# sepsamavi/safe-interactive-crowdnav

Hardware: AMD Instinct MI355X
Metric: sampled trajectories/sec (N x K, 50 denoise steps) (higher is better)
Workload: dtype fp16 activations x split-fp16 weights (weight-lo term as one bf8 MFMA per k64), fp32 accumulate; 1 GPU; cfg3: 256 episodes/GPU x N=5 x K=20 x H=12, 50 DDIM steps, JMID; episodes_per_gpu=256, total_episodes=256, humans=5, samples=20, horizon=12, denoise_steps=50, net=jmid, precision=f16mx, class_default_precision=f16mx, lanes=2

## Files before the change

### include/jmid_hip.h

```cpp
#ifndef JMID_HIP_H
#define JMID_HIP_H

#include <stddef.h>
#include <stdint.h>

#ifdef __cplusplus
extern "C" {
#endif
typedef struct jmid_ctx* jmid_handle_t;

#pragma GCC visibility push(default)

enum { JMID_NET_IMID = 0, JMID_NET_JMID = 1 };
enum { JMID_MEM_HOST = 0, JMID_MEM_DEVICE = 1 };
enum { JMID_PREC_F32 = 0, JMID_PREC_F16X3 = 1, JMID_PREC_F16 = 2, JMID_PREC_F16X2 = 3, JMID_PREC_F16MX = 4 };

enum {
    JMID_OK = 0,
    JMID_EINVAL = -1,
    JMID_ENOWEIGHT = -2,
    JMID_EHIP = -3,
    JMID_ENOMEM = -4,
    JMID_ERANGE = -5,
    JMID_ETIMEOUT = -6,
// ... 47 lines not shown

int jmid_wall_statistics(jmid_handle_t h, int E, int A, int K, int T, const float* pos, const float* p0, int L, const double* walls,
                         double radius, float* dist_out, uint8_t* agent_out, float* sample_out, float* scene_out, int mem);

int jmid_topk(jmid_handle_t h, int E, int A, int K, int T, int k, const float* pos, const float* bw, float* sel, float* logw,
              int mem);

int jmid_predict(jmid_handle_t h, int E, int A, int K, int T, int k, const float* x_st, const float* nbr_sum, const float* edge_mask,
                 const float* x_T, const float* p0, float dt, int precision, const float* bw, float* sel, float* logw, float* pos_out);

int jmid_net_eval_padded(jmid_handle_t h, int E, int A, int K, int T, const int32_t* n_agents, int step_idx, const float* x, const float* ctx,
                         int precision, float* e_out, int mem);
int jmid_denoise_padded(jmid_handle_t h, int E, int A, int K, int T, const int32_t* n_agents, const float* x_T, const float* ctx, const float* p0,
                        float dt, int precision, float* vel_out, float* pos_out, int mem);
int jmid_topk_padded(jmid_handle_t h, int E, int A, int K, int T, int k, const int32_t* n_agents, const float* pos, const float* bw, float* sel,
                     float* logw, int mem);
int jmid_predict_padded(jmid_handle_t h, int E, int A, int K, int T, int k, const int32_t* n_agents, const float* x_st, const float* nbr_sum,
                        const float* edge_mask, const float* x_T, const float* p0, float dt, int precision, const float* bw, float* sel,
                        float* logw, float* pos_out);

int jmid_collision_statistics_padded(jmid_handle_t h, int E, int A, int K, int T, const int32_t* n_agents, const float* pos, double threshold,
                                     float* pair_out, uint8_t* agent_out, float* sample_out, float* scene_out, int mem);
int jmid_wall_statistics_padded(jmid_handle_t h, int E, int A, int K, int T, const int32_t* n_agents, const float* pos, const float* p0, int L,
                                const double* walls, double radius, float* dist_out, uint8_t* agent_out, float* sample_out, float* scene_out,
                                int mem);

int jmid_build_scene(jmid_handle_t h, int E, int N, int F, const double* human_xy, const double* robot_xy, double time_step, int horizon,
                     int force_all_in_cluster, uint8_t* in_cluster_out, uint8_t* robot_in_cluster_out, int* n_in_out, double* cv_out, int mem);

int jmid_scene_get(jmid_handle_t h, float* x, float* x_st, float* nbr_sum, float* edge_mask, float* p0, int mem);

int jmid_build_scene_var(jmid_handle_t h, int E, int N, int F, const double* human_xy, const double* robot_xy, const int32_t* first_frame,
                         double time_step, int horizon, int force_all_in_cluster, uint8_t* in_cluster_out, uint8_t* robot_in_cluster_out,
                         int* n_in_out, double* cv_out, int mem);

int jmid_build_scene_absent(jmid_handle_t h, int E, int N, int F, const double* human_xy, const double* robot_xy, const int32_t* first_frame,
                            double time_step, int horizon, int force_all_in_cluster, uint8_t* in_cluster_out, uint8_t* robot_in_cluster_out,
                            int* n_in_out, double* cv_out, int mem);

int jmid_scene_get_first_index(jmid_handle_t h, int32_t* out, int mem);

int jmid_predict_scene(jmid_handle_t h, int E, int A, int K, int T, int k, const float* x_T, float dt, int precision, const float* bw,
                       float* sel, float* logw, float* pos_out);

int jmid_build_scene_stamped(jmid_handle_t h, int E, int N, int R, const double* stamps, const double* human_xy, const double* robot_xy,
                             const int* n_frames, double time_step, int horizon, int force_all_in_cluster, uint8_t* in_cluster_out,
                             uint8_t* robot_in_cluster_out, int* n_in_out, int* n_grid_out, double* cv_out, int mem);

int jmid_build_scene_stamped_var(jmid_handle_t h, int E, int N, int R, const double* stamps, const double* human_xy, const double* robot_xy,
                                 const int* n_frames, double time_step, int horizon, int force_all_in_cluster, uint8_t* in_cluster_out,
                                 uint8_t* robot_in_cluster_out, int* n_in_out, int* n_grid_out, double* cv_out, int32_t* first_frame_out,
                                 int mem);

int jmid_build_scene_stamped_coast(jmid_handle_t h, int E, int N, int R, const double* stamps, const double* human_xy, const double* robot_xy,
                                   const int* n_frames, double time_step, int horizon, int force_all_in_cluster, uint8_t* in_cluster_out,
                                   uint8_t* robot_in_cluster_out, int* n_in_out, int* n_grid_out, double* cv_out, int32_t* first_frame_out,
                                   int max_coast, int32_t* coast_out, int mem);

int jmid_scene_get_frames(jmid_handle_t h, double* human_xy_out, double* robot_xy_out, double* pose_now_out, int mem);

int jmid_forecast_scene(jmid_handle_t h, int E, int A, int K, int T, int k, const float* x_T, float dt, int precision, const float* bw,
                        double* forecasts_out, double* logw_out);

int jmid_noise_fill(jmid_handle_t h, uint64_t seed, int E, int rows, int T, const uint32_t* episode_ids, int draw, float* out, int mem);

int jmid_denoise_seeded(jmid_handle_t h, int E, int A, int K, int T, uint64_t seed, const uint32_t* episode_ids, const float* ctx,
                        const float* p0, float dt, int precision, float* vel_out, float* pos_out, int mem);

int jmid_denoise_reject_seeded(jmid_handle_t h, int E, int A, int K, int T, uint64_t seed, const uint32_t* episode_ids, int draw0,
                               const float* ctx, const float* p0, float dt, int precision, double threshold, int max_rounds,
                               float* vel_out, float* pos_out, int32_t* slot_out, int32_t* episode_out, int mem);

int jmid_denoise_reject_walls_seeded(jmid_handle_t h, int E, int A, int K, int T, uint64_t seed, const uint32_t* episode_ids, int draw0,
                                     const float* ctx, const float* p0, float dt, int precision, double threshold, int max_rounds, int L,
                                     const double* walls, double radius, float* vel_out, float* pos_out, int32_t* slot_out,
                                     int32_t* episode_out, int32_t* cause_out, int mem);

int jmid_predict_scene_seeded(jmid_handle_t h, int E, int A, int K, int T, int k, uint64_t seed, const uint32_t* episode_ids, float dt,
                              int precision, const float* bw, float* sel, float* logw, float* pos_out);
int jmid_forecast_scene_seeded(jmid_handle_t h, int E, int A, int K, int T, int k, uint64_t seed, const uint32_t* episode_ids, float dt,
                               int precision, const float* bw, double* forecasts_out, double* logw_out);

int jmid_noise_fill_padded(jmid_handle_t h, uint64_t seed, int E, int A, int K, int T, const int32_t* n_agents, const uint32_t* episode_ids,
                           int draw, float* out, int mem);
int jmid_denoise_padded_seeded(jmid_handle_t h, int E, int A, int K, int T, const int32_t* n_agents, uint64_t seed, const uint32_t* episode_ids,
                               const float* ctx, const float* p0, float dt, int precision, float* vel_out, float* pos_out, int mem);

int jmid_denoise_reject_padded_seeded(jmid_handle_t h, int E, int A, int K, int T, const int32_t* n_agents, uint64_t seed,
                                      const uint32_t* episode_ids, int draw0, const float* ctx, const float* p0, float dt, int precision,
                                      double threshold, int max_rounds, int L, const double* walls, double radius, float* vel_out,
                                      float* pos_out, int32_t* slot_out, int32_t* episode_out, int32_t* cause_out, int mem);

int jmid_repair_collisions(jmid_handle_t h, int E, int A, int K, int T, const int32_t* n_agents, const float* pos, const float* p0, float dt,
                           double threshold, double margin, double tau, double step, int max_iter, float* pos_out, float* vel_out,
                           float* sample_out, int32_t* episode_out, int mem);

int jmid_predict_scene_padded(jmid_handle_t h, int E, int A, int K, int T, int k, const float* x_T, float dt, int precision, const float* bw,
                              float* sel, float* logw, float* pos_out);
int jmid_forecast_scene_padded(jmid_handle_t h, int E, int A, int K, int T, int k, const float* x_T, float dt, int precision, const float* bw,
                               double* forecasts_out, double* logw_out);
int jmid_predict_scene_padded_seeded(jmid_handle_t h, int E, int A, int K, int T, int k, uint64_t seed, const uint32_t* episode_ids, float dt,
                                     int precision, const float* bw, float* sel, float* logw, float* pos_out);
int jmid_forecast_scene_padded_seeded(jmid_handle_t h, int E, int A, int K, int T, int k, uint64_t seed, const uint32_t* episode_ids, float dt,
                                      int precision, const float* bw, double* forecasts_out, double* logw_out);

int jmid_set_loss_schedule(jmid_handle_t h, int n_t, const float* beta, const float* c0, const float* c1);
int jmid_loss(jmid_handle_t h, int E, int A, int T, const int32_t* n_agents, const int32_t* t, const float* x0, const float* e, const float* ctx,
              int precision, double* loss_out, double* row_out, float* e_theta_out, int mem);
int jmid_loss_seeded(jmid_handle_t h, int E, int A, int T, const int32_t* n_agents, const int32_t* t, const float* x0, uint64_t seed,
                     const uint32_t* episode_ids, const float* ctx, int precision, double* loss_out, double* row_out, float* e_theta_out, int mem);

int jmid_set_caller_stream(jmid_handle_t h, void* stream);

int64_t jmid_graph_replays(jmid_handle_t h);

int64_t jmid_erange_count(jmid_handle_t h);
int64_t jmid_timeout_count(jmid_handle_t h);

int jmid_set_chunk_episodes(jmid_handle_t h, int episodes);
int jmid_set_tuning(jmid_handle_t h, const char* key, int value);
int jmid_profile_enable(jmid_handle_t h, uint32_t class_mask);
int jmid_profile_reset(jmid_handle_t h);
int jmid_profile_get(jmid_handle_t h, int cls, int64_t* n_launches, double* total_ms);
int jmid_kernel_class_count(void);
const char* jmid_kernel_class_name(int cls);
int jmid_synchronize(jmid_handle_t h);

#ifdef JMID_DIAGNOSTICS
int jmid_dbg_gemm(jmid_handle_t h, int M, int N, int K, const float* A, const float* Wt, const float* bias, int relu,
                  int precision, float* C);
int jmid_dbg_attention(jmid_handle_t h, int nseq, int S, const float* QKV, int precision, float* OUT);
int jmid_dbg_gemm_ln_mx(jmid_handle_t h, int M, int K, const float* A, const float* Wt, const float* bias, const float* gamma,
                        const float* beta, float* X, int fused);
int jmid_dbg_add_layernorm(jmid_handle_t h, int M, int d, float* X, const float* Y, const float* gamma,
                           const float* beta);
int jmid_dbg_plan_chunks(int net_kind, int nhead, int lanes, int chunk_episodes, int E, int tokens_per_episode, int* sizes, int cap);
int jmid_dbg_plan_chunks_mode(int net_kind, int nhead, int lanes, int chunk_episodes, int E, int tokens_per_episode, int precision, int* sizes, int cap);
#define JMID_DBG_GEMM_PLAN_KNOBS 13
int jmid_dbg_gemm_plan(int mode, int epi, int out, int M, int N, int K, int small_now, int one_chunk, const int* knobs, int* plan);
#define JMID_DBG_LAYOUT_SCENE 1
#define JMID_DBG_LAYOUT_FORECAST 2
#define JMID_DBG_LAYOUT_SEEDED 4
#define JMID_DBG_LAYOUT_PADDED 8
#define JMID_DBG_LAYOUT_FIRST_INDEX 16
#define JMID_DBG_LAYOUT_BW 32
#define JMID_DBG_LAYOUT_POS 64
#define JMID_DBG_LAYOUT_CV 128
#define JMID_DBG_CHAIN_WORDS (2 * 14 + 5)
#define JMID_DBG_SCENE_WORDS (2 * 13 + 4)
int jmid_dbg_chain_layout(int hist_len, int ctx_dim, int E, int A, int K, int T, int k, int N, int flags, int64_t* chain_dev, int64_t* chain_pin,
                          int64_t* scene);
int jmid_dbg_qkv0(jmid_handle_t h, int E, int A, int K, int T, const float* x, const float* hyp, int hyp_width, int step, int precision,
                  float* qkv, float* thyp_row);
int jmid_dbg_tail(jmid_handle_t h, int E, int A, int K, int T, const float* X, const float* hyp, int hyp_width, int step, int precision,
                  float* e, float* thyp_row);
#define JMID_DBG_LAYER_WIDTH(d_model, d_ff) (7 * (d_model) + (d_ff))
#define JMID_DBG_LAYER_PLAN_WORDS 25
int jmid_dbg_layer(jmid_handle_t h, int E, int A, int K, int T, int layer, int precision, const float* X, const int32_t* n_agents, int last,
                   float* hi, float* lo, int* plan);
int jmid_dbg_noise_words(jmid_handle_t h, uint64_t seed, int E, int rows, int T, const uint32_t* episode_ids, int draw, uint32_t* out, int mem);
#endif

#pragma GCC visibility pop
#ifdef __cplusplus
}
#endif
#endif
```

### safe-interactive-crowdnav_amd/_lib.py

```python
from __future__ import annotations

import ctypes as C
import os

from .build import library_path

c_float_p = C.POINTER(C.c_float)
Handle = C.c_void_p

NET_IMID, NET_JMID = 0, 1
MEM_HOST, MEM_DEVICE = 0, 1
PREC_F32, PREC_F16X3, PREC_F16, PREC_F16X2, PREC_F16MX = 0, 1, 2, 3, 4
PRECISIONS = {"f32": PREC_F32, "f16x3": PREC_F16X3, "f16": PREC_F16, "f16x2": PREC_F16X2, "f16mx": PREC_F16MX}

EINVAL, ENOWEIGHT, EHIP, ENOMEM, ERANGE, ETIMEOUT, EHISTORY = -1, -2, -3, -4, -5, -6, -7
ERR_NAMES = {EINVAL: "JMID_EINVAL", ENOWEIGHT: "JMID_ENOWEIGHT", EHIP: "JMID_EHIP", ENOMEM: "JMID_ENOMEM", ERANGE: "JMID_ERANGE",
             ETIMEOUT: "JMID_ETIMEOUT", EHISTORY: "JMID_EHISTORY"}

SIGNATURES = {
    "jmid_version": (C.c_char_p, []),
    "jmid_device_count": (C.c_int, []),
    "jmid_create": (C.c_int, [C.POINTER(Handle), C.c_int, C.c_int, C.c_int, C.c_int, C.c_int, C.c_int]),
    "jmid_destroy": (C.c_int, [Handle]),
    "jmid_last_error": (C.c_char_p, [Handle]),
    "jmid_load_weight": (C.c_int, [Handle, C.c_char_p, C.c_void_p, C.c_size_t]),
    "jmid_finalize_weights": (C.c_int, [Handle]),
    "jmid_set_ddim_table": (C.c_int, [Handle, C.c_int, C.c_void_p, C.c_void_p, C.c_void_p, C.c_void_p, C.c_void_p]),
    "jmid_set_ddpm_table": (C.c_int, [Handle, C.c_int, C.c_void_p, C.c_void_p, C.c_void_p, C.c_void_p, C.c_void_p]),
    "jmid_denoise_ddpm": (C.c_int, [Handle, C.c_int, C.c_int, C.c_int, C.c_int, C.c_void_p, C.c_void_p, C.c_void_p,
                                    C.c_void_p, C.c_float, C.c_int, C.c_void_p, C.c_void_p, C.c_int]),
    "jmid_encode": (C.c_int, [Handle, C.c_int, C.c_void_p, C.c_void_p, C.c_void_p, C.c_void_p, C.c_int]),
    "jmid_encode_var": (C.c_int, [Handle, C.c_int, C.c_void_p, C.c_void_p, C.c_void_p, C.c_void_p, C.c_void_p, C.c_int]),
    "jmid_denoise": (C.c_int, [Handle, C.c_int, C.c_int, C.c_int, C.c_int, C.c_void_p, C.c_void_p, C.c_void_p,
                               C.c_float, C.c_int, C.c_void_p, C.c_void_p, C.c_int]),
    "jmid_net_eval": (C.c_int, [Handle, C.c_int, C.c_int, C.c_int, C.c_int, C.c_int, C.c_void_p, C.c_void_p,
                                C.c_int, C.c_void_p, C.c_int]),
    "jmid_episode_metrics": (C.c_int, [Handle, C.c_int, C.c_int, C.c_int, C.c_int, C.c_void_p, C.c_void_p,
                                       C.c_void_p, C.c_int]),
    "jmid_eval_statistics": (C.c_int, [Handle, C.c_int, C.c_int, C.c_int, C.c_int, C.c_void_p, C.c_void_p, C.c_void_p,
                                       C.c_void_p, C.c_int]),
    "jmid_eval_statistics_masked": (C.c_int, [Handle, C.c_int, C.c_int, C.c_int, C.c_int, C.c_void_p, C.c_void_p, C.c_void_p,
                                              C.c_void_p, C.c_int, C.POINTER(C.c_int), C.c_void_p, C.c_void_p, C.c_void_p, C.c_int]),
    "jmid_collision_statistics": (C.c_int, [Handle, C.c_int, C.c_int, C.c_int, C.c_int, C.c_void_p, C.c_double, C.c_void_p,
                                            C.c_void_p, C.c_void_p, C.c_void_p, C.c_int]),
    "jmid_wall_statistics": (C.c_int, [Handle, C.c_int, C.c_int, C.c_int, C.c_int, C.c_void_p, C.c_void_p, C.c_int, C.c_void_p, C.c_double,
                                       C.c_void_p, C.c_void_p, C.c_void_p, C.c_void_p, C.c_int]),
    "jmid_collision_statistics_padded": (C.c_int, [Handle, C.c_int, C.c_int, C.c_int, C.c_int, C.c_void_p, C.c_void_p, C.c_double, C.c_void_p,
                                                   C.c_void_p, C.c_void_p, C.c_void_p, C.c_int]),
    "jmid_wall_statistics_padded": (C.c_int, [Handle, C.c_int, C.c_int, C.c_int, C.c_int, C.c_void_p, C.c_void_p, C.c_void_p, C.c_int, C.c_void_p,
                                              C.c_double, C.c_void_p, C.c_void_p, C.c_void_p, C.c_void_p, C.c_int]),
    "jmid_topk": (C.c_int, [Handle, C.c_int, C.c_int, C.c_int, C.c_int, C.c_int, C.c_void_p, C.c_void_p, C.c_void_p,
                            C.c_void_p, C.c_int]),
    "jmid_predict": (C.c_int, [Handle, C.c_int, C.c_int, C.c_int, C.c_int, C.c_int, C.c_void_p, C.c_void_p, C.c_void_p, C.c_void_p,
                               C.c_void_p, C.c_float, C.c_int, C.c_void_p, C.c_void_p, C.c_void_p, C.c_void_p]),
    "jmid_net_eval_padded": (C.c_int, [Handle, C.c_int, C.c_int, C.c_int, C.c_int, C.c_void_p, C.c_int, C.c_void_p, C.c_void_p,
                                       C.c_int, C.c_void_p, C.c_int]),
    "jmid_denoise_padded": (C.c_int, [Handle, C.c_int, C.c_int, C.c_int, C.c_int, C.c_void_p, C.c_void_p, C.c_void_p, C.c_void_p,
                                      C.c_float, C.c_int, C.c_void_p, C.c_void_p, C.c_int]),
    "jmid_topk_padded": (C.c_int, [Handle, C.c_int, C.c_int, C.c_int, C.c_int, C.c_int, C.c_void_p, C.c_void_p, C.c_void_p, C.c_void_p,
                                   C.c_void_p, C.c_int]),
    "jmid_predict_padded": (C.c_int, [Handle, C.c_int, C.c_int, C.c_int, C.c_int, C.c_int, C.c_void_p, C.c_void_p, C.c_void_p, C.c_void_p,
                                      C.c_void_p, C.c_void_p, C.c_float, C.c_int, C.c_void_p, C.c_void_p, C.c_void_p, C.c_void_p]),
    "jmid_build_scene": (C.c_int, [Handle, C.c_int, C.c_int, C.c_int, C.c_void_p, C.c_void_p, C.c_double, C.c_int, C.c_int, C.c_void_p,
                                   C.c_void_p, C.c_void_p, C.c_void_p, C.c_int]),
    "jmid_scene_get": (C.c_int, [Handle, C.c_void_p, C.c_void_p, C.c_void_p, C.c_void_p, C.c_void_p, C.c_int]),
    "jmid_build_scene_var": (C.c_int, [Handle, C.c_int, C.c_int, C.c_int, C.c_void_p, C.c_void_p, C.c_void_p, C.c_double, C.c_int, C.c_int,
                                       C.c_void_p, C.c_void_p, C.c_void_p, C.c_void_p, C.c_int]),
    "jmid_build_scene_absent": (C.c_int, [Handle, C.c_int, C.c_int, C.c_int, C.c_void_p, C.c_void_p, C.c_void_p, C.c_double, C.c_int, C.c_int,
                                          C.c_void_p, C.c_void_p, C.c_void_p, C.c_void_p, C.c_int]),
    "jmid_scene_get_first_index": (C.c_int, [Handle, C.c_void_p, C.c_int]),
    "jmid_predict_scene": (C.c_int, [Handle, C.c_int, C.c_int, C.c_int, C.c_int, C.c_int, C.c_void_p, C.c_float, C.c_int, C.c_void_p,
                                     C.c_void_p, C.c_void_p, C.c_void_p]),
    "jmid_build_scene_stamped": (C.c_int, [Handle, C.c_int, C.c_int, C.c_int, C.c_void_p, C.c_void_p, C.c_void_p, C.c_void_p, C.c_double,
                                           C.c_int, C.c_int, C.c_void_p, C.c_void_p, C.c_void_p, C.c_void_p, C.c_void_p, C.c_int]),
    "jmid_build_scene_stamped_var": (C.c_int, [Handle, C.c_int, C.c_int, C.c_int, C.c_void_p, C.c_void_p, C.c_void_p, C.c_void_p, C.c_double,
                                               C.c_int, C.c_int, C.c_void_p, C.c_void_p, C.c_void_p, C.c_void_p, C.c_void_p, C.c_void_p, C.c_int]),
    "jmid_build_scene_stamped_coast": (C.c_int, [Handle, C.c_int, C.c_int, C.c_int, C.c_void_p, C.c_void_p, C.c_void_p, C.c_void_p, C.c_double,
                                                 C.c_int, C.c_int, C.c_void_p, C.c_void_p, C.c_void_p, C.c_void_p, C.c_void_p, C.c_void_p, C.c_int,
                                                 C.c_void_p, C.c_int]),
    "jmid_scene_get_frames": (C.c_int, [Handle, C.c_void_p, C.c_void_p, C.c_void_p, C.c_int]),
    "jmid_forecast_scene": (C.c_int, [Handle, C.c_int, C.c_int, C.c_int, C.c_int, C.c_int, C.c_void_p, C.c_float, C.c_int, C.c_void_p,
                                      C.c_void_p, C.c_void_p]),
    "jmid_noise_fill": (C.c_int, [Handle, C.c_uint64, C.c_int, C.c_int, C.c_int, C.c_void_p, C.c_int, C.c_void_p, C.c_int]),
    "jmid_denoise_seeded": (C.c_int, [Handle, C.c_int, C.c_int, C.c_int, C.c_int, C.c_uint64, C.c_void_p, C.c_void_p, C.c_void_p,
                                      C.c_float, C.c_int, C.c_void_p, C.c_void_p, C.c_int]),
    "jmid_denoise_reject_seeded": (C.c_int, [Handle, C.c_int, C.c_int, C.c_int, C.c_int, C.c_uint64, C.c_void_p, C.c_int, C.c_void_p, C.c_void_p,
                                             C.c_float, C.c_int, C.c_double, C.c_int, C.c_void_p, C.c_void_p, C.c_void_p, C.c_void_p, C.c_int]),
    "jmid_denoise_reject_walls_seeded": (C.c_int, [Handle, C.c_int, C.c_int, C.c_int, C.c_int, C.c_uint64, C.c_void_p, C.c_int, C.c_void_p,
                                                   C.c_void_p, C.c_float, C.c_int, C.c_double, C.c_int, C.c_int, C.c_void_p, C.c_double,
                                                   C.c_void_p, C.c_void_p, C.c_void_p, C.c_void_p, C.c_void_p, C.c_int]),
    "jmid_predict_scene_seeded": (C.c_int, [Handle, C.c_int, C.c_int, C.c_int, C.c_int, C.c_int, C.c_uint64, C.c_void_p, C.c_float, C.c_int,
                                            C.c_void_p, C.c_void_p, C.c_void_p, C.c_void_p]),
    "jmid_forecast_scene_seeded": (C.c_int, [Handle, C.c_int, C.c_int, C.c_int, C.c_int, C.c_int, C.c_uint64, C.c_void_p, C.c_float, C.c_int,
                                             C.c_void_p, C.c_void_p, C.c_void_p]),
    "jmid_noise_fill_padded": (C.c_int, [Handle, C.c_uint64, C.c_int, C.c_int, C.c_int, C.c_int, C.c_void_p, C.c_void_p, C.c_int, C.c_void_p,
                                         C.c_int]),
    "jmid_denoise_padded_seeded": (C.c_int, [Handle, C.c_int, C.c_int, C.c_int, C.c_int, C.c_void_p, C.c_uint64, C.c_void_p, C.c_void_p,
                                             C.c_void_p, C.c_float, C.c_int, C.c_void_p, C.c_void_p, C.c_int]),
    "jmid_denoise_reject_padded_seeded": (C.c_int, [Handle, C.c_int, C.c_int, C.c_int, C.c_int, C.c_void_p, C.c_uint64, C.c_void_p, C.c_int,
                                                    C.c_void_p, C.c_void_p, C.c_float, C.c_int, C.c_double, C.c_int, C.c_int, C.c_void_p,
                                                    C.c_double, C.c_void_p, C.c_void_p, C.c_void_p, C.c_void_p, C.c_void_p, C.c_int]),
    "jmid_repair_collisions": (C.c_int, [Handle, C.c_int, C.c_int, C.c_int, C.c_int, C.c_void_p, C.c_void_p, C.c_void_p, C.c_float, C.c_double,
                                         C.c_double, C.c_double, C.c_double, C.c_int, C.c_void_p, C.c_void_p, C.c_void_p, C.c_void_p, C.c_int]),
    "jmid_predict_scene_padded": (C.c_int, [Handle, C.c_int, C.c_int, C.c_int, C.c_int, C.c_int, C.c_void_p, C.c_float, C.c_int, C.c_void_p,
                                            C.c_void_p, C.c_void_p, C.c_void_p]),
    "jmid_forecast_scene_padded": (C.c_int, [Handle, C.c_int, C.c_int, C.c_int, C.c_int, C.c_int, C.c_void_p, C.c_float, C.c_int, C.c_void_p,
                                             C.c_void_p, C.c_void_p]),
    "jmid_predict_scene_padded_seeded": (C.c_int, [Handle, C.c_int, C.c_int, C.c_int, C.c_int, C.c_int, C.c_uint64, C.c_void_p, C.c_float,
                                                   C.c_int, C.c_void_p, C.c_void_p, C.c_void_p, C.c_void_p]),
    "jmid_forecast_scene_padded_seeded": (C.c_int, [Handle, C.c_int, C.c_int, C.c_int, C.c_int, C.c_int, C.c_uint64, C.c_void_p, C.c_float,
                                                    C.c_int, C.c_void_p, C.c_void_p, C.c_void_p]),
    "jmid_set_loss_schedule": (C.c_int, [Handle, C.c_int, C.c_void_p, C.c_void_p, C.c_void_p]),
    "jmid_loss": (C.c_int, [Handle, C.c_int, C.c_int, C.c_int, C.c_void_p, C.c_void_p, C.c_void_p, C.c_void_p, C.c_void_p, C.c_int,
                            C.c_void_p, C.c_void_p, C.c_void_p, C.c_int]),
    "jmid_loss_seeded": (C.c_int, [Handle, C.c_int, C.c_int, C.c_int, C.c_void_p, C.c_void_p, C.c_void_p, C.c_uint64, C.c_void_p, C.c_void_p,
                                   C.c_int, C.c_void_p, C.c_void_p, C.c_void_p, C.c_int]),
    "jmid_set_chunk_episodes": (C.c_int, [Handle, C.c_int]),
    "jmid_set_tuning": (C.c_int, [Handle, C.c_char_p, C.c_int]),
    "jmid_set_caller_stream": (C.c_int, [Handle, C.c_void_p]),
    "jmid_graph_replays": (C.c_int64, [Handle]),
    "jmid_erange_count": (C.c_int64, [Handle]),
    "jmid_timeout_count": (C.c_int64, [Handle]),
    "jmid_profile_enable": (C.c_int, [Handle, C.c_uint32]),
    "jmid_profile_reset": (C.c_int, [Handle]),
    "jmid_profile_get": (C.c_int, [Handle, C.c_int, C.POINTER(C.c_int64), C.POINTER(C.c_double)]),
    "jmid_kernel_class_count": (C.c_int, []),
    "jmid_kernel_class_name": (C.c_char_p, [C.c_int]),
    "jmid_synchronize": (C.c_int, [Handle]),
}

DIAG_SIGNATURES = {
    "jmid_dbg_gemm": (C.c_int, [Handle, C.c_int, C.c_int, C.c_int, C.c_void_p, C.c_void_p, C.c_void_p, C.c_int,
                                C.c_int, C.c_void_p]),
    "jmid_dbg_attention": (C.c_int, [Handle, C.c_int, C.c_int, C.c_void_p, C.c_int, C.c_void_p]),
    "jmid_dbg_gemm_ln_mx": (C.c_int, [Handle, C.c_int, C.c_int, C.c_void_p, C.c_void_p, C.c_void_p, C.c_void_p, C.c_void_p,
                                      C.c_void_p, C.c_int]),
    "jmid_dbg_add_layernorm": (C.c_int, [Handle, C.c_int, C.c_int, C.c_void_p, C.c_void_p, C.c_void_p, C.c_void_p]),
    "jmid_dbg_plan_chunks": (C.c_int, [C.c_int, C.c_int, C.c_int, C.c_int, C.c_int, C.c_int, C.POINTER(C.c_int), C.c_int]),
    "jmid_dbg_plan_chunks_mode": (C.c_int, [C.c_int, C.c_int, C.c_int, C.c_int, C.c_int, C.c_int, C.c_int, C.POINTER(C.c_int), C.c_int]),
    "jmid_dbg_gemm_plan": (C.c_int, [C.c_int] * 8 + [C.POINTER(C.c_int), C.POINTER(C.c_int)]),
    "jmid_dbg_chain_layout": (C.c_int, [C.c_int] * 9 + [C.POINTER(C.c_int64)] * 3),
    "jmid_dbg_qkv0": (C.c_int, [Handle, C.c_int, C.c_int, C.c_int, C.c_int, C.c_void_p, C.c_void_p, C.c_int, C.c_int, C.c_int, C.c_void_p, C.c_void_p]),
    "jmid_dbg_tail": (C.c_int, [Handle, C.c_int, C.c_int, C.c_int, C.c_int, C.c_void_p, C.c_void_p, C.c_int, C.c_int, C.c_int, C.c_void_p, C.c_void_p]),
    "jmid_dbg_layer": (C.c_int, [Handle, C.c_int, C.c_int, C.c_int, C.c_int, C.c_int, C.c_int, C.c_void_p, C.c_void_p, C.c_int,
                                 C.c_void_p, C.c_void_p, C.POINTER(C.c_int)]),
    "jmid_dbg_noise_words": (C.c_int, [Handle, C.c_uint64, C.c_int, C.c_int, C.c_int, C.c_void_p, C.c_int, C.c_void_p, C.c_int]),
}


class JmidError(RuntimeError):
    def __init__(self, code: int, message: str):
        super().__init__(f"{ERR_NAMES.get(code, code)}: {message}")
        self.code = code


_LIBS = {}


def load_library(path: str = None) -> C.CDLL:
    key = os.path.abspath(path or library_path())
    if key in _LIBS:
        return _LIBS[key]
    import torch

    path = key
    if not os.path.exists(path):
        raise ImportError(
            f"{path} is missing: build it with `python -c 'import __graft_entry__ as g; g.build()'` "
            "(hipcc --offload-arch=gfx950).  The predictor has no CPU fallback.")
    lib = C.CDLL(path)
    for name, (res, args) in SIGNATURES.items():
        fn = getattr(lib, name)
        fn.restype = res
        fn.argtypes = args
    lib.has_diagnostics = b"diagnostics" in lib.jmid_version()
    if lib.has_diagnostics:
        for name, (res, args) in DIAG_SIGNATURES.items():
            fn = getattr(lib, name)
            fn.restype = res
            fn.argtypes = args
    _LIBS[key] = lib
    return lib
```

### safe-interactive-crowdnav_amd/csrc/common.hpp

```cpp
#pragma once
#include <hip/hip_runtime.h>
#include <hip/hip_fp16.h>
#include <stdint.h>

#include <atomic>
#include <mutex>

namespace jmid {

typedef float f32x4 __attribute__((ext_vector_type(4)));
typedef float f32x16 __attribute__((ext_vector_type(16)));
typedef _Float16 f16x8 __attribute__((ext_vector_type(8)));
typedef _Float16 f16x4 __attribute__((ext_vector_type(4)));
typedef _Float16 f16x2 __attribute__((ext_vector_type(2)));

constexpr int kWave = 64;
constexpr int kPeMaxLen = 24;

struct HyperLayout {
    int g1, b1, g3, b3, g4, b4, go, bo, total;
};
__host__ __device__ inline HyperLayout make_hyper_layout(int d_model, int d_mid, int d_low) {
    HyperLayout L;
    L.g1 = 0;
// ... 13 lines not shown
}
inline unsigned fast_div_magic(int d, unsigned long long x_max) {
    return d > 1 && x_max * (unsigned long long)d < (1ull << 32) ? (unsigned)((1ull << 32) / (unsigned)d + 1) : 0u;
}

struct RowMap {
    int T, A, KA;
    unsigned mT = 0, mKA = 0, mA = 0;
    __device__ __forceinline__ int ea(int m) const {
        const int r = fast_div(m, T, mT);
        const int e = fast_div(r, KA, mKA);
        const int a = r - fast_div(r, A, mA) * A;
        return e * A + a;
    }
    __device__ __forceinline__ int t_of(int m) const { return m - fast_div(m, T, mT) * T; }
};
inline RowMap make_rowmap(int T, int A, int KA, unsigned long long M) {
    RowMap r{T, A, KA};
    r.mT = fast_div_magic(T, M);
    r.mKA = fast_div_magic(KA, M);
    r.mA = fast_div_magic(A, M);
    return r;
}

__host__ __device__ __forceinline__ size_t blk_index(int row, int k, int K) {
    const int rb = row >> 7, r = row & 127, kb = k >> 5, kk = k & 31;
    return ((size_t)rb * (K >> 5) + kb) * 4096 + (size_t)(r * 32 + ((((kk >> 3) ^ ((r >> 2) & 3)) << 3) | (kk & 7)));
}
__host__ __device__ __forceinline__ size_t blk_plane_elems(size_t rows, int K) {
    return ((rows + 127) / 128) * 128 * (size_t)K;
}

__host__ __device__ __forceinline__ int vt_key_pos(int key) {
    const int g = (key >> 2) & 3;
    return (key & ~15) | ((((g & 1) << 1) | (g >> 1)) << 2) | (key & 3);
}
__host__ __device__ __forceinline__ int vt_spad(int S) { return (S + 15) / 16 * 16; }

template <typename T>
__device__ __forceinline__ void args_now(const T& a) {
    static_assert(sizeof(T) % 4 == 0, "argument block of whole dwords");
    struct Words { unsigned w[sizeof(T) / 4]; };
    const Words w = __builtin_bit_cast(Words, a);
#pragma unroll
    for (unsigned i = 0; i < sizeof(T) / 4; ++i) asm volatile("" ::"s"(w.w[i]));
}
template <typename... T>
__device__ __forceinline__ void args_now_each(const T&... t) { (args_now(t), ...); }

__device__ __forceinline__ unsigned long long pin_uniform(unsigned long long v) {
    asm volatile("" : "+s"(v));
    return v;
}
__device__ __forceinline__ unsigned long long pin_uniform_rfl(unsigned long long v) {
    const unsigned lo = __builtin_amdgcn_readfirstlane((unsigned)v), hi = __builtin_amdgcn_readfirstlane((unsigned)(v >> 32));
    unsigned long long u = ((unsigned long long)hi << 32) | lo;
    asm volatile("" : "+s"(u));
    return u;
}

struct Tuning {
    int fuse_embed = 1;
    int ln_fuse = 0;
    int ln_rows = 0;
    int bystander_lds = 0;
    int gemm_h_variant = 0;
    int gemm_ng = 0;
    int no_vt_direct = 0;
    int attn_h_variant = 0;
    int attn_pack = 1;
    int vt_stage = 0;
    int graph = 0;
    int attn_nsplit = 0;
    int csl_swap = 0;
    int attn_sm = 0;
    int attn_prio = 0;
    int attn_one_wg = 0;
    int h1_stage = 0;
    int out_traj = 0;
    int attn_mx = 0;
    int mx_ln = 0;
    int attn_pf = 0;
    int gemm_small = 0;
    int small_cmb = 0;
    int small_lnx = 0;
    int cus = 256;
    int lnx_polls = 0;
    int lnx_withhold = 0;
    int small_lnx2 = 0;
    int gemm_pn = 0;
    int small_lanes = 0;
    int small_qk = 0;
    int small_pn = 0;
    int qkv0 = 0;
    int tail_fold = 0;
    int attn_abl = 0;
    int gemm_abl = 0;
};
#ifdef JMID_ABLATIONS
inline int attn_abl_bits(const Tuning& t) { return t.attn_abl; }
inline int gemm_abl_bits(const Tuning& t) { return t.gemm_abl; }
#else
inline int attn_abl_bits(const Tuning&) { return 0; }
inline int gemm_abl_bits(const Tuning&) { return 0; }
#endif

struct DevSeen {
    std::atomic<bool> v[64];
    DevSeen() { for (auto& b : v) b.store(false, std::memory_order_relaxed); }
};
struct DeviceOnce {
    std::unique_lock<std::mutex> lk;
    std::atomic<bool>* slot = nullptr;
    explicit operator bool() const { return slot != nullptr; }
    DeviceOnce() = default;
    DeviceOnce(DeviceOnce&& o) noexcept : lk(std::move(o.lk)), slot(o.slot) { o.slot = nullptr; }
    ~DeviceOnce() { if (slot) slot->store(true, std::memory_order_release); }
};
inline std::mutex& device_once_mutex() {
    static std::mutex m;
    return m;
}
inline DeviceOnce first_use_on_device(DevSeen& seen) {
    int dev = 0;
    (void)hipGetDevice(&dev);
    dev &= 63;
    DeviceOnce o;
    if (seen.v[dev].load(std::memory_order_acquire)) return o;
    o.lk = std::unique_lock<std::mutex>(device_once_mutex());
    if (seen.v[dev].load(std::memory_order_acquire)) {
        o.lk.unlock();
        return o;
    }
    o.slot = &seen.v[dev];
    return o;
}

template <auto Kernel, size_t MaxLds = 0, typename... Args>
inline hipError_t launch_with_lds(dim3 grid, dim3 block, size_t lds_bytes, hipStream_t st, Args... args) {
    static DevSeen seen;
    if (auto once_ = first_use_on_device(seen))
        (void)hipFuncSetAttribute(reinterpret_cast<const void*>(Kernel), hipFuncAttributeMaxDynamicSharedMemorySize,
                                  (int)(MaxLds ? MaxLds : lds_bytes));
    hipLaunchKernelGGL(Kernel, grid, block, lds_bytes, st, args...);
    return hipGetLastError();
}

template <typename F>
static inline int bystander_lds(int n, F* fn) {
    if (n > 0) (void)hipFuncSetAttribute((const void*)fn, hipFuncAttributeMaxDynamicSharedMemorySize, n);
    return n;
}

__device__ __forceinline__ float sigmoidf_(float x) { return 1.0f / (1.0f + expf(-x)); }

__device__ __forceinline__ float wave_sum(float v) {
#pragma unroll
    for (int o = 32; o > 0; o >>= 1) v += __shfl_xor(v, o, 64);
    return v;
}

__device__ __forceinline__ void half_swap(float x, float& lo_half, float& hi_half) {
#ifdef JMID_ATT_SHFL
    lo_half = x;
    hi_half = __shfl_xor(x, 32, 64);
#else
    float a = x, b = x;
    asm volatile("s_nop 1\n\tv_permlane32_swap_b32 %0, %1" : "+v"(a), "+v"(b));
    lo_half = a;
    hi_half = b;
#endif
}

__device__ __forceinline__ int frag_row(int reg, int hi) { return (reg & 3) + 8 * (reg >> 2) + 4 * hi; }

}
```

### safe-interactive-crowdnav_amd/csrc/jmid_abi.hip

```cpp
#include "jmid_ctx.hpp"
#include "collision_stats.hpp"
#include "wall_stats.hpp"
#include "repair.hpp"

namespace jmid_host {

int upload_walls(jmid_ctx* h, int L, const double* walls, const double** dev, const std::string& who) {
    *dev = nullptr;
    if (L < 0 || L > WLS_MAX_L) return fail(h, JMID_EINVAL, who + " supports 0 <= L <= 64 walls");
    if (L == 0) return 0;
    if (!walls) return fail(h, JMID_EINVAL, who + ": null walls with L > 0");
    for (int i = 0; i < L * 4; ++i)
        if (!std::isfinite(walls[i])) return fail(h, JMID_EINVAL, who + ": a wall has a non-finite coordinate");
    if (int rc = h->wall_seg.upload(h, walls, L * 8, who.c_str())) return rc;
    *dev = h->wall_seg.get<double>();
    return 0;
}

std::string& thread_error() {
    static thread_local std::string e;
    return e;
}

int fail(jmid_ctx* h, int code, const std::string& msg) {
// ... 1294 lines not shown
}

int jmid_predict_scene_padded_seeded(jmid_handle_t h, int E, int A, int K, int T, int k, uint64_t seed, const uint32_t* episode_ids, float dt,
                                     int precision, const float* bw, float* sel, float* logw, float* pos_out) {
    const SeedArgs sa{seed, episode_ids};
    ChainCall c = chain_call("jmid_predict_scene_padded_seeded", E, A, K, T, k, dt, precision);
    c.padded = true; c.seeded = &sa; c.bw = bw; c.sel = sel; c.logw = logw; c.pos_out = pos_out;
    return predict_scene_entry(h, c);
}

int jmid_forecast_scene_padded_seeded(jmid_handle_t h, int E, int A, int K, int T, int k, uint64_t seed, const uint32_t* episode_ids, float dt,
                                      int precision, const float* bw, double* forecasts_out, double* logw_out) {
    const SeedArgs sa{seed, episode_ids};
    ChainCall c = chain_call("jmid_forecast_scene_padded_seeded", E, A, K, T, k, dt, precision);
    c.forecast = c.padded = true; c.seeded = &sa; c.bw = bw; c.forecasts_out = forecasts_out; c.logw_out = logw_out;
    return predict_scene_entry(h, c);
}

int jmid_denoise_padded_seeded(jmid_handle_t h, int E, int A, int K, int T, const int32_t* n_agents, uint64_t seed, const uint32_t* episode_ids,
                               const float* ctx, const float* p0, float dt, int precision, float* vel_out, float* pos_out, int mem) {
    if (!h) return JMID_EINVAL;
    if (!n_agents) return fail(h, JMID_EINVAL, "jmid_denoise_padded_seeded: null n_agents");
    if (!episode_ids) return fail(h, JMID_EINVAL, "jmid_denoise_padded_seeded: null episode_ids");
    const SeedArgs sa{seed, episode_ids};
    DenoiseCall c{E, A, K, T, precision, mem};
    c.ctx = ctx; c.p0 = p0; c.dt = dt; c.vel_out = vel_out; c.pos_out = pos_out; c.n_agents = n_agents; c.seeded = &sa;
    c.who = "jmid_denoise_padded_seeded";
    return run_network(h, c);
}

int jmid_noise_fill_padded(jmid_handle_t h, uint64_t seed, int E, int A, int K, int T, const int32_t* n_agents, const uint32_t* episode_ids, int draw,
                           float* out, int mem) {
    return noise_padded_entry(h, seed, E, A, K, T, n_agents, episode_ids, draw, out, mem);
}

int jmid_denoise_seeded(jmid_handle_t h, int E, int A, int K, int T, uint64_t seed, const uint32_t* episode_ids, const float* ctx, const float* p0,
                        float dt, int precision, float* vel_out, float* pos_out, int mem) {
    if (!h) return JMID_EINVAL;
    if (!episode_ids) return fail(h, JMID_EINVAL, "jmid_denoise_seeded: null episode_ids");
    const SeedArgs sa{seed, episode_ids};
    DenoiseCall c{E, A, K, T, precision, mem};
    c.ctx = ctx; c.p0 = p0; c.dt = dt; c.vel_out = vel_out; c.pos_out = pos_out; c.seeded = &sa; c.who = "jmid_denoise_seeded";
    return run_network(h, c);
}

static int reject_entry(jmid_handle_t h, const char* who, int E, int A, int K, int T, bool padded, const int32_t* n_agents, uint64_t seed, const uint32_t* episode_ids, int draw0,
                        const float* ctx, const float* p0, float dt, int precision, double threshold, int max_rounds, int L, const double* walls,
                        double radius, float* vel_out, float* pos_out, int32_t* slot_out, int32_t* episode_out, int32_t* cause_out, int mem) {
    if (!h) return JMID_EINVAL;
    const std::string w(who);
    if (int rc = check_ready(h)) return rc;
    if (h->ddpm) return fail(h, JMID_EINVAL, w + " samples with DDIM: under a DDPM table the draws 1.. are the steps' z");
    if (E < 1 || K < 1 || K > REJ_MAX_K || T < 2 || T > CLS_MAX_T || A < 1 || A > CLS_MAX_A)
        return fail(h, JMID_EINVAL, w + " supports E >= 1, 1 <= K <= 1024, 2 <= T <= 24, 1 <= A <= 64");
    if ((size_t)E * K > (size_t)0x7fffffff) return fail(h, JMID_EINVAL, w + ": E * K exceeds the launch grid");
    if (!episode_ids || !ctx) return fail(h, JMID_EINVAL, w + ": null episode_ids or ctx");
    if (!p0) return fail(h, JMID_EINVAL, w + ": null p0 (the predicate is defined on positions)");
    if (!(threshold >= 0.0) || !std::isfinite(threshold)) return fail(h, JMID_EINVAL, w + ": the threshold must be finite and >= 0");
    if (max_rounds < 0 || max_rounds > 64) return fail(h, JMID_EINVAL, w + ": max_rounds must be in 0..64");
    if (draw0 < 0 || draw0 > 0x7fffffff - 64) return fail(h, JMID_EINVAL, w + ": draw0 must be at least 0 (and draw0 + max_rounds must fit an int)");
    CallMode mode;
    if (!call_mode(precision, &mode)) return fail(h, JMID_EINVAL, w + ": precision must be JMID_PREC_F32, JMID_PREC_F16X3, JMID_PREC_F16X2 or JMID_PREC_F16MX");
    if (mem != JMID_MEM_HOST && mem != JMID_MEM_DEVICE) return fail(h, JMID_EINVAL, w + ": bad mem");
    if (!(radius >= 0.0) || !std::isfinite(radius)) return fail(h, JMID_EINVAL, w + ": the radius must be finite and >= 0");
    if (padded) {
        if (int rc = check_n_agents(h, who, n_agents, E, A)) return rc;
        if (h->net_kind == JMID_NET_JMID && mode.split && !attn_masked_built(plan_attn(h->d / h->nhead, h->tune), mode.x2 != 0))
            return fail(h, JMID_EINVAL, w + ": a padded call needs the default attention kernel (the attention A/B knobs have no masked form)");
    }
    HIPCHK(h, hipSetDevice(h->device));
    RejectWalls rw;
    rw.L = L; rw.radius = radius;
    if (int rc = upload_walls(h, L, walls, &rw.dev, w)) return rc;
    return reject_loop(h, who, E, A, K, T, n_agents, seed, episode_ids, draw0, ctx, p0, dt, precision, threshold, max_rounds, rw, vel_out, pos_out, slot_out,
                       episode_out, cause_out, mem);
}

int jmid_denoise_reject_seeded(jmid_handle_t h, int E, int A, int K, int T, uint64_t seed, const uint32_t* episode_ids, int draw0, const float* ctx,
                               const float* p0, float dt, int precision, double threshold, int max_rounds, float* vel_out, float* pos_out,
                               int32_t* slot_out, int32_t* episode_out, int mem) {
    return reject_entry(h, "jmid_denoise_reject_seeded", E, A, K, T, false, nullptr, seed, episode_ids, draw0, ctx, p0, dt, precision, threshold, max_rounds, 0,
                        nullptr, 0.0, vel_out, pos_out, slot_out, episode_out, nullptr, mem);
}

int jmid_denoise_reject_walls_seeded(jmid_handle_t h, int E, int A, int K, int T, uint64_t seed, const uint32_t* episode_ids, int draw0,
                                     const float* ctx, const float* p0, float dt, int precision, double threshold, int max_rounds, int L,
                                     const double* walls, double radius, float* vel_out, float* pos_out, int32_t* slot_out, int32_t* episode_out,
                                     int32_t* cause_out, int mem) {
    return reject_entry(h, "jmid_denoise_reject_walls_seeded", E, A, K, T, false, nullptr, seed, episode_ids, draw0, ctx, p0, dt, precision, threshold,
                        max_rounds, L, walls, radius, vel_out, pos_out, slot_out, episode_out, cause_out, mem);
}

int jmid_denoise_reject_padded_seeded(jmid_handle_t h, int E, int A, int K, int T, const int32_t* n_agents, uint64_t seed, const uint32_t* episode_ids,
                                      int draw0, const float* ctx, const float* p0, float dt, int precision, double threshold, int max_rounds, int L,
                                      const double* walls, double radius, float* vel_out, float* pos_out, int32_t* slot_out, int32_t* episode_out,
                                      int32_t* cause_out, int mem) {
    return reject_entry(h, "jmid_denoise_reject_padded_seeded", E, A, K, T, true, n_agents, seed, episode_ids, draw0, ctx, p0, dt, precision,
                        threshold, max_rounds, L, walls, radius, vel_out, pos_out, slot_out, episode_out, cause_out, mem);
}

int jmid_noise_fill(jmid_handle_t h, uint64_t seed, int E, int rows, int T, const uint32_t* episode_ids, int draw, float* out, int mem) {
    return noise_entry(h, "jmid_noise_fill", seed, E, rows, T, episode_ids, draw, out, nullptr, mem);
}

int jmid_set_chunk_episodes(jmid_handle_t h, int episodes) {
    if (!h || episodes < 0) return JMID_EINVAL;
    h->chunk_eps = episodes;
    drop_graphs(h);
    return JMID_OK;
}

int jmid_set_tuning(jmid_handle_t h, const char* key, int value) {
    if (!h || !key) return JMID_EINVAL;
    const std::string k(key);
    struct Knob {
        const char* name;
        int Tuning::*field;
        int lo, hi;
    };
#ifdef JMID_DIAGNOSTICS
    static const Knob knobs[] = {
        {"gemm_h_variant", &Tuning::gemm_h_variant, 0, 8},
        {"attn_pack", &Tuning::attn_pack, 0, 1},
        {"fuse_embed", &Tuning::fuse_embed, 0, 1},
        {"bystander_lds", &Tuning::bystander_lds, 0, 160 * 1024},
        {"ln_rows", &Tuning::ln_rows, 0, 128},
        {"ln_fuse", &Tuning::ln_fuse, 0, 2},
        {"no_vt_direct", &Tuning::no_vt_direct, 0, 1},
        {"gemm_ng", &Tuning::gemm_ng, 0, 64},
        {"attn_h_variant", &Tuning::attn_h_variant, 0, 2},
        {"vt_stage", &Tuning::vt_stage, 0, 3},
        {"graph", &Tuning::graph, 0, 2},
        {"attn_nsplit", &Tuning::attn_nsplit, 0, 16},
        {"attn_mx", &Tuning::attn_mx, 0, 3},
        {"out_traj", &Tuning::out_traj, 0, 2},
        {"attn_pf", &Tuning::attn_pf, 0, 2},
        {"attn_one_wg", &Tuning::attn_one_wg, 0, 1},
        {"attn_sm", &Tuning::attn_sm, 0, 2},
        {"attn_prio", &Tuning::attn_prio, 0, 2},
        {"mx_ln", &Tuning::mx_ln, 0, 2},
        {"csl_swap", &Tuning::csl_swap, 0, 3},
        {"h1_stage", &Tuning::h1_stage, 0, 2},
        {"gemm_small", &Tuning::gemm_small, 0, 2},
        {"gemm_pn", &Tuning::gemm_pn, 0, 8},
        {"small_lanes", &Tuning::small_lanes, 0, 2},
        {"small_cmb", &Tuning::small_cmb, 0, 2},
        {"small_lnx", &Tuning::small_lnx, 0, 2},
        {"cus", &Tuning::cus, 0, 4096},
        {"lnx_polls", &Tuning::lnx_polls, 0, 1 << 20},
        {"lnx_withhold", &Tuning::lnx_withhold, 0, 1},
        {"small_lnx2", &Tuning::small_lnx2, 0, 2},
        {"small_qk", &Tuning::small_qk, 0, 2},
        {"small_pn", &Tuning::small_pn, 0, 8},
        {"qkv0", &Tuning::qkv0, 0, 2},
        {"tail_fold", &Tuning::tail_fold, 0, 2},
#ifdef JMID_ABLATIONS
        {"attn_abl", &Tuning::attn_abl, 0, 1 << 30},
        {"gemm_abl", &Tuning::gemm_abl, 0, 1 << 30},
#endif
    };
#endif
    if (k == "lanes") {
        if (value < 1 || value > jmid_ctx::kMaxLanes) return fail(h, JMID_EINVAL, "lanes must be 1..4");
        h->lanes = value;
        return JMID_OK;
    }
#ifdef JMID_DIAGNOSTICS
    for (const Knob& kn : knobs)
        if (k == kn.name) {
            if (value < kn.lo || value > kn.hi || (k == "ln_rows" && value != 0 && value != 64 && value != 128))
                return fail(h, JMID_EINVAL, k + " out of range");
            h->tune.*(kn.field) = value;
            if (k == "cus" && value == 0) {
                int cus = 0;
                h->tune.cus = hipDeviceGetAttribute(&cus, hipDeviceAttributeMultiprocessorCount, h->device) == hipSuccess && cus > 0 ? cus : 256;
            }
            drop_graphs(h);
            return JMID_OK;
        }
#endif
    return fail(h, JMID_EINVAL, "unknown tuning key " + k);
}

int64_t jmid_graph_replays(jmid_handle_t h) { return h ? h->graph_replays : -1; }

int64_t jmid_erange_count(jmid_handle_t h) { return h ? h->erange_calls : -1; }
int64_t jmid_timeout_count(jmid_handle_t h) { return h ? h->lnx_timeouts : -1; }

int jmid_set_caller_stream(jmid_handle_t h, void* stream) {
    if (!h) return JMID_EINVAL;
    h->caller_stream = reinterpret_cast<hipStream_t>(stream);
    return JMID_OK;
}

int jmid_synchronize(jmid_handle_t h) {
    if (!h) return JMID_EINVAL;
    HIPCHK(h, hipSetDevice(h->device));
    HIPCHK(h, hipStreamSynchronize(h->stream));
    return JMID_OK;
}

}
```

### safe-interactive-crowdnav_amd/csrc/jmid_ctx.hpp

```cpp
#pragma once
#include "../../include/jmid_hip.h"

#include <hip/hip_runtime.h>

#include <algorithm>
#include <cmath>
#include <cstdio>
#include <cstring>
#include <limits>
#include <map>
#include <string>
#include <vector>

#include "attn_f16x3.hpp"
#include "attn_f32.hpp"
#include "common.hpp"
#include "elementwise.hpp"
#include "encoder.hpp"
#include "eval_stats.hpp"
#include "gemm_f16x3.hpp"
#include "gemm_ln_f16x3.hpp"
#include "gemm_ln2_mx.hpp"
#include "gemm_small.hpp"
#include "gemm_f32.hpp"
// ... 186 lines not shown
    std::string err;
    jmid_ctx() = default;
    jmid_ctx(const jmid_ctx&) = delete;
    ~jmid_ctx();
};

constexpr size_t kLnxWords = 2 * jmid::SM_LNX_GRANULES;

namespace jmid_host {

inline hipStream_t stream_of(jmid_ctx* h) { return h->stream; }
inline int reserve_block(jmid_ctx* h, Block& b, size_t need, const char* who) {
    return &b == &h->arena ? ensure_arena(h, need, who) : b.reserve(h, need, who);
}

struct CallMode {
    int precision = JMID_PREC_F32;
    bool split = false;
    int x2 = 0;
    int mx = 0;
    GemmMode gemm = GM_X3;
};
inline bool call_mode(int precision, CallMode* m) {
    if (precision != JMID_PREC_F32 && precision != JMID_PREC_F16X3 && precision != JMID_PREC_F16X2 && precision != JMID_PREC_F16MX) return false;
    const int mx = precision == JMID_PREC_F16MX, x2 = precision == JMID_PREC_F16X2 || mx;
    *m = CallMode{precision, precision != JMID_PREC_F32, x2, mx, !x2 ? GM_X3 : mx ? GM_MX : GM_X2};
    return true;
}

struct ProfScope {
    jmid_ctx* h;
    int cls;
    hipStream_t stream;
    bool on;
    EvPair ev;
    ProfScope(jmid_ctx* h_, int cls_, hipStream_t s) : h(h_), cls(cls_), stream(s), on((h_->prof_mask >> cls_) & 1u) {
        if (on) {
            if (!h->ev_pool.empty()) {
                ev = h->ev_pool.back();
                h->ev_pool.pop_back();
            } else {
                hipEventCreate(&ev.a);
                hipEventCreate(&ev.b);
            }
            hipEventRecord(ev.a, stream);
        }
    }
    ~ProfScope() {
        if (on) {
            hipEventRecord(ev.b, stream);
            h->prof_ev[cls].push_back(ev);
        }
    }
};

inline size_t numel(const std::vector<size_t>& s) {
    size_t n = 1;
    for (size_t v : s) n *= v;
    return n;
}

void register_shapes(jmid_ctx* h);
int dev_alloc_copy(jmid_ctx* h, float** out, const std::vector<float>& host);
int fetch_host(jmid_ctx* h, const std::string& name, std::vector<float>& out);
std::vector<float> time_table(const jmid_ctx* h, const std::vector<float>& beta);
int upload_time_table(jmid_ctx* h);
int upload_loss_schedule(jmid_ctx* h);
int make_w8(jmid_ctx* h, const float* dW, int N, int K, jmid_ctx::W8Image* out);
int w8_image(jmid_ctx* h, const float* dW, int N, int K, unsigned char* out);
void free_planes(jmid_ctx* h);
void free_derived(jmid_ctx* h);
void free_weights(jmid_ctx* h);
void drop_graphs(jmid_ctx* h);
void sync_lanes(jmid_ctx* h);
std::vector<int> plan_chunks(const jmid_ctx* h, const CallMode& m, int E, int tokens_per_episode);
int check_ready(jmid_ctx* h);
struct SeedArgs {
    uint64_t seed;
    const uint32_t* ids;
    int draw = 0;
};
int fill_noise(jmid_ctx* h, uint64_t seed, const unsigned* ids_dev, int E, size_t n, int draw, float* out, unsigned* words, hipStream_t stream);
int fill_noise_padded(jmid_ctx* h, uint64_t seed, const unsigned* ids_dev, const int* n_agents_dev, int E, int A, int K, int T, int draw, float* out,
                      hipStream_t stream);
struct LossCall {
    const int32_t* t = nullptr;
    const float* e = nullptr;
    const SeedArgs* seeded = nullptr;
    double *loss_out = nullptr, *row_out = nullptr;
};
struct DenoiseCall {
    int E, A, K, T, precision, mem;
    const float *x_in = nullptr, *ctx = nullptr, *p0 = nullptr;
    float dt = 0.f;
    float *vel_out = nullptr, *pos_out = nullptr, *e_out = nullptr;
    int single_step = -1;
    const float* z = nullptr;
    const SeedArgs* seeded = nullptr;
    bool chained = false;
    const int32_t* n_agents = nullptr;
    const int* n_agents_dev = nullptr;
    const LossCall* loss = nullptr;
    const char* who = "jmid_denoise";
};
struct ChainCall {
    int E, A, K, T, k, precision;
    float dt = 0.f;
    const char* who = "jmid_predict";
    bool scene = false;
    bool forecast = false;
    bool padded = false;
    const float *x_st = nullptr, *nbr_sum = nullptr, *edge_mask = nullptr, *p0 = nullptr;
    const float* x_T = nullptr;
    const SeedArgs* seeded = nullptr;
    const float* bw = nullptr;
    float *sel = nullptr, *logw = nullptr, *pos_out = nullptr;
    double *forecasts_out = nullptr, *logw_out = nullptr;
    const int32_t* n_agents = nullptr;
    bool rank() const { return k < K; }
};
struct ChainIo {
    Arr<float> x_st, nbr_sum, edge_mask, x_T, p0, bw;
    size_t up_bytes = 0;
    Arr<float> ctx;
    Arr<int> flag;
    Arr<double> forecasts, logw_d;
    Arr<float> sel, logw, pos;
    size_t down_bytes = 0;
    Arr<int> first_index;
    size_t up_bytes_from(const Arr<float>& a) const { return up_bytes - (size_t)((const char*)a.p - (const char*)x_st.p); }
};
enum SceneSource {
    SCENE_HOST_ARRAYS,
    SCENE_DEVICE_ARRAYS,
    SCENE_DEVICE_GRID,
};
struct SceneBuild {
    const char* who;
    int E, N, F;
    SceneSource src;
    const double *human_xy, *robot_xy;
    const int32_t* first_frame = nullptr;
    bool allow_absent = false;
    double time_step = 0.0;
    int horizon = 0, force_all_in_cluster = 0;
    uint8_t *in_cluster_out = nullptr, *robot_in_cluster_out = nullptr;
    int* n_in_out = nullptr;
    double* cv_out = nullptr;
    int mem = JMID_MEM_HOST;
};
int check_n_agents(jmid_ctx* h, const char* who, const int32_t* n_agents, int E, int A);
int run_network(jmid_ctx* h, DenoiseCall a);
int dbg_step(jmid_ctx* h, bool tail, int E, int A, int K, int T, const float* in, const float* hyp, int hyp_width, int step, int precision,
             float* out, float* thyp_row);
int dbg_layer(jmid_ctx* h, int E, int A, int K, int T, int layer, int precision, const float* X, const int32_t* n_agents, int last,
              float* hi, float* lo, int* plan);
int flagged_call(jmid_ctx* h, int flag);
int launch_episode_metrics(jmid_ctx* h, const float* pos, const float* gt, float* out, int E, int K, int A, int T);
size_t chain_io(const jmid_ctx* h, const ChainCall& c, char* base, ChainIo* out, bool pinned);
size_t scene_arrays(int E, int N, int F, int horizon, bool has_first, char* base, SceneArrays* out);
int noise_entry(jmid_ctx* h, const char* who, uint64_t seed, int E, int rows, int T, const uint32_t* episode_ids, int draw, float* out,
                unsigned* words, int mem);
int prof_collect(jmid_ctx* h);

}
using namespace jmid_host;
```

### safe-interactive-crowdnav_amd/csrc/jmid_diag.hip

```cpp
#include "jmid_ctx.hpp"
#include "jmid_launch.hpp"

#include <deque>

#ifdef JMID_DIAGNOSTICS

static int dbg_open(jmid_ctx* h, int precision, CallMode* mode) {
    if (!call_mode(precision, mode)) return fail(h, JMID_EINVAL, "bad precision");
    HIPCHK(h, hipSetDevice(h->device));
    if (!h->range_flag) {
        HIPCHK(h, hipMalloc((void**)&h->range_flag, sizeof(int)));
        HIPCHK(h, hipMemsetAsync(h->range_flag, 0, sizeof(int), h->stream));
    }
    return 0;
}

struct DbgTemps {
    jmid_ctx* h;
    const char* who;
    std::deque<Block> blocks;
    int rc = 0;
    template <class T>
    T* take(size_t bytes, const void* host = nullptr) {
        if (rc) return nullptr;
// ... 122 lines not shown
        GemmArgs g{};
        g.A = dA; g.lda = K; g.W = dW; g.ldw = K; g.bias = dB; g.C = dC; g.ldc = N; g.M = M; g.N = N; g.K = K;
        rc = relu ? run_gemm<EPI_BIAS_RELU>(h, h->stream, KC_GEMM_QKV, g) : run_gemm<EPI_BIAS>(h, h->stream, KC_GEMM_QKV, g);
    } else {
        const size_t pa = blk_plane_elems(M, K) * 2, pw = blk_plane_elems(N, K) * 2;
        half_t *ah = t.zeros<half_t>(pa), *al = t.zeros<half_t>(pa), *wh = t.zeros<half_t>(pw), *wl = t.zeros<half_t>(pw);
        if (t.rc) return t.rc;
        hipLaunchKernelGGL(split_planes_blocked_kernel, dim3(512), dim3(256), 0, h->stream, dA, ah, al, M, K,
                           h->range_flag, 1.0f);
        hipLaunchKernelGGL(split_planes_blocked_kernel, dim3(512), dim3(256), 0, h->stream, dW, wh, wl, N, K,
                           h->range_flag, kWScale);
        GemmHArgs g{};
        g.Ahi = ah; g.Alo = al; g.Whi = wh; g.Wlo = wl; g.bias = dB; g.C = dC; g.ldc = N;
        g.M = M; g.N = N; g.K = K; g.x2 = mode.x2;
        if (mode.mx && N % 32 == 0 && K % 64 == 0)
            if (!(g.W8 = dbg_w8(t, dW, N, K))) return t.rc;
        const GemmPlan plan = plan_gemm(mode.gemm, relu ? EPI_BIAS_RELU : EPI_BIAS, OUT_F32, M, N, K, CallFacts{}, h->tune);
        rc = relu ? run_gemm_h<EPI_BIAS_RELU, OUT_F32>(h, h->stream, KC_GEMM_QKV, g, plan) : run_gemm_h<EPI_BIAS, OUT_F32>(h, h->stream, KC_GEMM_QKV, g, plan);
    }
    if (rc) return rc;
    HIPCHK(h, hipStreamSynchronize(h->stream));
    HIPCHK(h, hipMemcpy(C, dC, (size_t)M * N * 4, hipMemcpyDeviceToHost));
    return 0;
}

int jmid_dbg_attention(jmid_handle_t h, int nseq, int S, const float* QKV, int precision, float* OUT) {
    if (!h || !QKV || !OUT) return JMID_EINVAL;
    CallMode mode;
    if (int rc = dbg_open(h, precision, &mode)) return rc;
    const size_t Mt = (size_t)nseq * S;
    const int d = h->d, hd = h->d / h->nhead;
    DbgTemps t{h, "jmid_dbg_attention"};
    float* dQ = t.take<float>(Mt * 3 * d * 4, QKV);
    float* dO = t.take<float>(Mt * d * 4);
    if (t.rc) return t.rc;
    int rc = 0;
    if (precision == JMID_PREC_F32) {
        AttnArgs aa{dQ, dO, S, d, h->nhead, 1.0f / sqrtf((float)hd), nullptr, nullptr};
        ProfScope ps(h, KC_ATTN, h->stream);
        hipError_t e = launch_attn_f32(aa, nseq, hd, plan_attn(hd, h->tune).pack, h->stream);
        if (e != hipSuccess) rc = fail(h, JMID_EHIP, hipGetErrorString(e));
    } else {
        const int Spad = vt_spad(S);
        const size_t vt = (size_t)nseq * d * Spad;
        half_t* b[8];
        const size_t sz[8] = {Mt * d, Mt * d, Mt * d, Mt * d, vt, vt, blk_plane_elems(Mt, d), blk_plane_elems(Mt, d)};
        for (int i = 0; i < 8; ++i) b[i] = t.zeros<half_t>(sz[i] * sizeof(half_t));
        if (t.rc) return t.rc;
        hipLaunchKernelGGL(qkv_to_planes_kernel, dim3(512), dim3(256), 0, h->stream, dQ, b[0], b[1], b[2], b[3], b[4],
                           b[5], Mt, d, hd, S, Spad, 1.4426950408889634f / sqrtf((float)hd));
        int ns = 1;
        float *opart = nullptr, *mlpart = nullptr;
        if (hd == 128) ns = attn_pick_nsplit(((S + 127) / 128) * h->nhead * nseq, S);
        if (ns > 1) {
            opart = t.take<float>((size_t)ns * Mt * d * 4);
            mlpart = t.take<float>((size_t)ns * Mt * h->nhead * 2 * 4);
            if (t.rc) return t.rc;
        }
        AttnHArgs aa{b[0], b[1], b[2], b[3], b[4], b[5], b[6], b[7], S, Spad, d, h->nhead, 1.0f / sqrtf((float)hd),
                     h->range_flag, ns, opart, mlpart, mode.x2};
        {
            ProfScope ps(h, KC_ATTN, h->stream);
            hipError_t e = launch_attn_f16x3(aa, nseq, hd, plan_attn(hd, h->tune), h->stream);
            if (e != hipSuccess) rc = fail(h, JMID_EHIP, hipGetErrorString(e));
        }
        hipLaunchKernelGGL(merge_planes_kernel, dim3(512), dim3(256), 0, h->stream, b[6], b[7], dO, (int)Mt, d, (float*)nullptr);
    }
    if (rc) return rc;
    HIPCHK(h, hipStreamSynchronize(h->stream));
    HIPCHK(h, hipMemcpy(OUT, dO, Mt * d * 4, hipMemcpyDeviceToHost));
    return 0;
}

int jmid_dbg_gemm_ln_mx(jmid_handle_t h, int M, int K, const float* A, const float* Wt, const float* bias, const float* gamma,
                        const float* beta, float* X, int fused) {
    if (!h || !A || !Wt || !bias || !gamma || !beta || !X || M <= 0 || K % 64 != 0) return JMID_EINVAL;
    constexpr int N = GLN_BN;
    CallMode mode;
    if (int rc = dbg_open(h, JMID_PREC_F16MX, &mode)) return rc;
    DbgTemps t{h, "jmid_dbg_gemm_ln_mx"};
    float* dA = t.take<float>((size_t)M * K * 4, A);
    float* dW = t.take<float>((size_t)N * K * 4, Wt);
    float* dB = t.take<float>(N * 4, bias);
    float* dG = t.take<float>(N * 4, gamma);
    float* dT = t.take<float>(N * 4, beta);
    float* dX = t.take<float>((size_t)M * N * 4, X);
    float* dY = t.zeros<float>((size_t)(M + 63) / 64 * 64 * N * 4);
    const size_t pa = blk_plane_elems(M, K) * 2, pw = blk_plane_elems(N, K) * 2, px = blk_plane_elems(M, N) * 2;
    half_t *ah = t.zeros<half_t>(pa), *al = t.zeros<half_t>(pa), *wh = t.zeros<half_t>(pw), *wl = t.zeros<half_t>(pw);
    half_t *w16h = t.zeros<half_t>((size_t)N * K * 2), *w16l = t.zeros<half_t>((size_t)N * K * 2);
    half_t* xh = t.zeros<half_t>(px);
    unsigned char* xl8 = t.zeros<unsigned char>(px);
    if (t.rc) return t.rc;
    hipLaunchKernelGGL(split_planes_blocked_kernel, dim3(512), dim3(256), 0, h->stream, dA, ah, al, M, K, h->range_flag, 1.0f);
    hipLaunchKernelGGL(split_planes_blocked_kernel, dim3(512), dim3(256), 0, h->stream, dW, wh, wl, N, K, h->range_flag, kWScale);
    hipLaunchKernelGGL(split_planes_k16_kernel, dim3(256), dim3(256), 0, h->stream, dW, w16h, w16l, N, K);
    hipLaunchKernelGGL(split_planes_lo8_kernel, dim3(512), dim3(256), 0, h->stream, dX, xh, xl8, M);
    unsigned char* w8 = dbg_w8(t, dW, N, K);
    if (!w8) return t.rc;
    int rc = 0;
    if (fused == 1) {
        GemmLn2Args g2{ah, w16h, w8, dB, dG, dT, xh, xl8, M, K, 1e-5f, h->range_flag, 0};
        hipError_t e = launch_gemm_ln2_mx(g2, plan_ln_rows(true, M, h->tune), h->stream);
        if (e != hipSuccess) rc = fail(h, JMID_EHIP, hipGetErrorString(e));
    } else {
        GemmHArgs g{};
        g.Ahi = ah; g.Alo = al; g.Whi = wh; g.Wlo = wl; g.W8 = w8; g.bias = dB; g.C = dY; g.ldc = N; g.M = M; g.N = N; g.K = K; g.x2 = mode.x2;
        if (fused == 3) {
            unsigned long long* xs = t.zeros<unsigned long long>(kLnxWords * sizeof(unsigned));
            const GemmPlan lnx = plan_gemm(GM_MX, EPI_BIAS, OUT_LNX, M, N, K, CallFacts{}, h->tune);
            if (!xs || lnx.shape == GS_NONE) return fail(h, JMID_EINVAL, "jmid_dbg_gemm_ln_mx: shape does not take the small kernel with the statistics exchange");
            g.ln_gamma = dG; g.ln_beta = dT; g.ln_xh = xh; g.ln_xl = nullptr; g.ln_xl8 = xl8; g.ln_xchg = xs; g.ln_eps = 1e-5f; g.ln_no_lo = 0;
            (void)hipMemsetAsync(h->range_flag, 0, sizeof(int), h->stream);
            rc = run_gemm_lnx_small(h, h->stream, KC_GEMM_OUT, g, lnx);
            if (!rc) {
                int flag = 0;
                (void)hipMemcpyAsync(&flag, h->range_flag, sizeof(int), hipMemcpyDeviceToHost, h->stream);
                (void)hipStreamSynchronize(h->stream);
                if (flag & 2) rc = fail(h, JMID_EHIP, "jmid_dbg_gemm_ln_mx: a workgroup gave up waiting for its row tile's statistics");
            }
        } else {
            rc = run_gemm_h<EPI_BIAS, OUT_F32>(h, h->stream, KC_GEMM_OUT, g, plan_gemm(GM_MX, EPI_BIAS, OUT_F32, M, N, K, CallFacts{}, h->tune));
            if (!rc) rc = run_add_ln(h, h->stream, nullptr, dY, dG, dT, M, N, xh, reinterpret_cast<half_t*>(xl8), true, 0);
        }
    }
    if (rc) return rc;
    hipLaunchKernelGGL(merge_planes_lo8_kernel, dim3(512), dim3(256), 0, h->stream, xh, xl8, dX, M, (float*)nullptr);
    HIPCHK(h, hipStreamSynchronize(h->stream));
    HIPCHK(h, hipMemcpy(X, dX, (size_t)M * N * 4, hipMemcpyDeviceToHost));
    return 0;
}

int jmid_dbg_add_layernorm(jmid_handle_t h, int M, int d, float* X, const float* Y, const float* gamma,
                           const float* beta) {
    if (!h || !X || !Y || !gamma || !beta) return JMID_EINVAL;
    HIPCHK(h, hipSetDevice(h->device));
    DbgTemps t{h, "jmid_dbg_add_layernorm"};
    float* dX = t.take<float>((size_t)M * d * 4, X);
    float* dY = t.take<float>((size_t)M * d * 4, Y);
    float* dG = t.take<float>((size_t)d * 4, gamma);
    float* dB = t.take<float>((size_t)d * 4, beta);
    if (t.rc) return t.rc;
    if (int rc = run_add_ln(h, h->stream, dX, dY, dG, dB, M, d)) return rc;
    HIPCHK(h, hipStreamSynchronize(h->stream));
    HIPCHK(h, hipMemcpy(X, dX, (size_t)M * d * 4, hipMemcpyDeviceToHost));
    return 0;
}

int jmid_dbg_qkv0(jmid_handle_t h, int E, int A, int K, int T, const float* x, const float* hyp, int hyp_width, int step, int precision,
                  float* qkv, float* thyp_row) {
    return h ? dbg_step(h, false, E, A, K, T, x, hyp, hyp_width, step, precision, qkv, thyp_row) : JMID_EINVAL;
}

int jmid_dbg_tail(jmid_handle_t h, int E, int A, int K, int T, const float* X, const float* hyp, int hyp_width, int step, int precision,
                  float* e, float* thyp_row) {
    return h ? dbg_step(h, true, E, A, K, T, X, hyp, hyp_width, step, precision, e, thyp_row) : JMID_EINVAL;
}

int jmid_dbg_layer(jmid_handle_t h, int E, int A, int K, int T, int layer, int precision, const float* X, const int32_t* n_agents, int last,
                   float* hi, float* lo, int* plan) {
    return h ? dbg_layer(h, E, A, K, T, layer, precision, X, n_agents, last, hi, lo, plan) : JMID_EINVAL;
}

int jmid_dbg_noise_words(jmid_handle_t h, uint64_t seed, int E, int rows, int T, const uint32_t* episode_ids, int draw, uint32_t* out, int mem) {
    return noise_entry(h, "jmid_dbg_noise_words", seed, E, rows, T, episode_ids, draw, nullptr, out, mem);
}

}
#endif
```

### safe-interactive-crowdnav_amd/csrc/jmid_planner.hip

```cpp
#include "jmid_ctx.hpp"
#include "jmid_launch.hpp"

namespace jmid_host {

void drop_graphs(jmid_ctx* h) {
    for (auto& kv : h->graphs)
        if (kv.second.exec) hipGraphExecDestroy(kv.second.exec);
    h->graphs.clear();
}

void sync_lanes(jmid_ctx* h) {
    for (int l = 0; l + 1 < jmid_ctx::kMaxLanes; ++l)
        if (h->lane_stream[l]) (void)hipStreamSynchronize(h->lane_stream[l]);
    if (h->stream) (void)hipStreamSynchronize(h->stream);
}

int ensure_arena(jmid_ctx* h, size_t bytes, const char* who) {
    if (bytes <= h->arena.bytes) return 0;
    drop_graphs(h);
    h->last_pos = nullptr;
    sync_lanes(h);
    return h->arena.reserve(h, bytes, who);
}

// ... 23 lines not shown
    g.S = h->net_kind == JMID_NET_JMID ? K * A * T : T;
    g.Spad = vt_spad(g.S);
    return g;
}

size_t step_ws_floats(const jmid_ctx* h, size_t Mc, const CallMode& m, const SeqGeom& sg, int nsplit, StepBuffers* sb,
                      char* base, size_t qkv0_rows, size_t tail_rows) {
    Carver c(base);
    StepBuffers s{};
    s.X = c.take(Mc * h->d);
    s.Y = c.take((Mc + 63) / 64 * 64 * h->d);
    s.ln_xchg = reinterpret_cast<unsigned long long*>(c.take(kLnxWords));
    if (!tail_rows) s.Y4 = c.take(Mc * h->dlow);
    if (!m.split) {
        s.QKV = c.take(Mc * 3 * h->d);
        s.ATT = c.take(Mc * h->d);
        s.H1 = c.take(Mc * h->ff);
        s.Y3 = c.take(Mc * h->dmid);
    } else {
        s.Xh = take_half(c, blk_plane_elems(Mc, h->d));
        s.Xl = take_half(c, blk_plane_elems(Mc, h->d));
        if (h->net_kind == JMID_NET_JMID) {
            s.Qh = take_half(c, Mc * h->d);
            s.Ql = take_half(c, Mc * h->d);
            s.Kh = take_half(c, Mc * h->d);
            s.Kl = take_half(c, Mc * h->d);
            s.Vh = take_half(c, Mc * h->d);
            s.Vl = take_half(c, Mc * h->d);
            s.vt_elems = (size_t)sg.nseq * h->d * sg.Spad;
            s.Vth = take_half(c, s.vt_elems);
            s.Vtl = take_half(c, s.vt_elems);
            if (nsplit > 1) {
                s.Opart = c.take((size_t)nsplit * Mc * h->d);
                s.MLpart = c.take((size_t)nsplit * Mc * h->nhead * 2);
            }
            if (qkv0_rows) {
                s.coef = c.take(qkv0_rows * h->d);
                s.uvc = c.take(qkv0_rows * 3 * h->d);
            }
        } else {
            s.QKV = c.take(Mc * 3 * h->d);
        }
        s.Ah = take_half(c, blk_plane_elems(Mc, h->d));
        s.Al = take_half(c, blk_plane_elems(Mc, h->d));
        s.H1h = take_half(c, blk_plane_elems(Mc, h->ff));
        s.H1l = take_half(c, blk_plane_elems(Mc, h->ff));
        if (tail_rows) {
            s.weff = c.take(tail_rows * 2 * h->d);
            s.beff = c.take(tail_rows * 2);
        } else {
            s.Y3h = take_half(c, blk_plane_elems(Mc, h->dmid));
            s.Y3l = take_half(c, blk_plane_elems(Mc, h->dmid));
        }
    }
    if (sb) *sb = s;
    return c.off;
}

bool byte_lo_plane(const jmid_ctx* h, const CallMode& m) { return m.mx && h->d == GLN_BN && h->tune.mx_ln != 2; }

enum ResidualPath {
    RB_GEMM_LN2,
    RB_GEMM_LN,
    RB_LNX_SMALL,
    RB_GEMM_ADD_LN,
};
struct ResidualPlan {
    ResidualPath path;
    int ln_rows;
    GemmPlan gemm;
    bool merge;
};

ResidualPlan residual_path(const jmid_ctx* h, const CallMode& m, int M, int K, const CallFacts& cf) {
    const Tuning& t = h->tune;
    if (h->d == GLN_BN && t.ln_fuse != 2 && (t.ln_fuse == 1 || M >= 7168))
        return {byte_lo_plane(h, m) ? RB_GEMM_LN2 : RB_GEMM_LN, plan_ln_rows(byte_lo_plane(h, m), M, t), {}, false};
    if (byte_lo_plane(h, m) && !h->lnx_off) {
        const GemmPlan lnx = plan_gemm(GM_MX, EPI_BIAS, OUT_LNX, M, h->d, K, cf, t);
        if (lnx.shape != GS_NONE) return {RB_LNX_SMALL, 0, lnx, false};
    }
    return {RB_GEMM_ADD_LN, 0, plan_gemm(m.gemm, EPI_BIAS, OUT_F32, M, h->d, K, cf, t), false};
}

bool one_launch_shape(const jmid_ctx* h, const CallMode& m, long tokens) { return m.mx && h->d == GLN_BN && tokens <= 2560; }

struct StepPlan {
    int Ec, M, T;
    int R;
    bool qkv0;
    bool tail_fold;
    CallMode mode;
    bool mxv2, joint;
    RowMap rm;
    SeqGeom sg;
    int hd;
    float att_scale;
    bool vt_direct;
    bool k8, q8l;
    CallFacts cf;
    GemmPlan in_proj, linear1, concat3, concat4;
    ResidualPlan out_proj, linear2;
    AttnPlan attn;
    int out_tpw;
    const float* thyp_base;
    size_t thyp_stride;
    const float* thyp(int step) const { return thyp_base + (size_t)step * thyp_stride; }
    const float *loss_hyp, *loss_tbo;
    const float* tbo(const float* hyp_chunk) const { return loss_tbo ? loss_tbo + (size_t)(hyp_chunk - loss_hyp) / thyp_ld * 2 : nullptr; }
    size_t thyp_ld;
};

StepPlan plan_step(const jmid_ctx* h, int Ec, int A, int K, int T, const CallMode& mode, const CallFacts& cf, bool masked = false) {
    StepPlan p{};
    const int d = h->d;
    p.Ec = Ec;
    p.M = Ec * K * A * T;
    p.T = T;
    p.R = Ec * A;
    p.mode = mode;
    const bool split = mode.split;
    p.mxv2 = split && byte_lo_plane(h, mode);
    p.joint = h->net_kind == JMID_NET_JMID;
    p.rm = make_rowmap(T, A, K * A, (unsigned long long)p.M);
    p.sg = seq_geom(h, Ec, A, K, T);
    p.hd = d / h->nhead;
    p.att_scale = 1.0f / sqrtf((float)p.hd);
    p.cf = cf;
    p.thyp_base = h->thyp;
    p.thyp_stride = p.thyp_ld = (size_t)h->hl.total;
    const Tuning& t = h->tune;
    p.attn = plan_attn(p.hd, t);
    p.attn.masked = masked && p.joint;
    p.qkv0 = split && p.joint && t.qkv0 != 1 && d % 32 == 0;
    p.tail_fold = split && t.tail_fold != 1 && d % 8 == 0 && d <= kTailMaxD && h->dmid <= kTailMaxMid && h->dlow <= kTailMaxLow;
    if (split) {
        const auto gemm = [&](int epi, int out, int N, int K) { return plan_gemm(mode.gemm, epi, out, p.M, N, K, cf, t); };
        p.in_proj = gemm(EPI_BIAS, p.joint ? OUT_QKV : OUT_F32, 3 * d, d);
        p.linear1 = gemm(EPI_BIAS_RELU, OUT_SPLIT, h->ff, d);
        p.concat3 = gemm(EPI_CSL, OUT_SPLIT, h->dmid, d);
        p.concat4 = gemm(EPI_CSL, OUT_F32, h->dlow, h->dmid);
        p.out_proj = residual_path(h, mode, p.M, d, cf);
        p.linear2 = residual_path(h, mode, p.M, h->ff, cf);
    }
    if (split && p.joint) {
        p.vt_direct = (p.sg.S % 4 == 0) && !t.no_vt_direct;
        p.k8 = p.in_proj.mode == GM_MX && p.hd == 128 && t.attn_h_variant == 0 && t.attn_mx != 2;
        p.q8l = p.k8 && t.attn_mx != 3;
        p.out_proj.merge = p.out_proj.path == RB_LNX_SMALL && small_cmb_fits(p.attn, p.cf.attn_nsplit, mode.x2, t);
    }
    if (d <= 512 && p.M % T == 0 && t.out_traj != 2 && (t.out_traj == 1 || p.M >= 4096 * 4)) {
        p.out_tpw = T;
        while (p.out_tpw > 1 && (p.M / p.out_tpw < 4096 || T % p.out_tpw != 0)) --p.out_tpw;
        if (t.out_traj == 1) p.out_tpw = T;
    }
    return p;
}

int residual_block(jmid_ctx* h, const StepPlan& p, const ResidualPlan& rp, const Lane& ln, const half_t* Ahi, const half_t* Alo,
                   int K, const LinearW& lin, const NormW& nrm, int cls, bool no_lo_out) {
    const int M = p.M, d = h->d;
    unsigned char* Xl8 = p.mxv2 ? reinterpret_cast<unsigned char*>(ln.Xl) : nullptr;
    if (rp.path == RB_GEMM_LN2) {
        GemmLn2Args g2{Ahi, lin.k16.hi, lin.w8, lin.bias, nrm.gamma, nrm.beta, ln.Xh, Xl8, M, K, 1e-5f, h->range_flag, no_lo_out};
        ProfScope ps(h, cls, ln.stream);
        HIPCHK(h, launch_gemm_ln2_mx(g2, rp.ln_rows, ln.stream));
        return 0;
    }
    if (rp.path == RB_GEMM_LN) {
        GemmLnArgs gl{Ahi, Alo, lin.k16.hi, lin.k16.lo, lin.bias, nrm.gamma, nrm.beta, ln.Xh, ln.Xl, M, K, 1e-5f, h->range_flag, p.mode.x2};
        gl.W8 = p.mode.mx ? lin.w8 : nullptr;
        gl.no_lo_out = p.mode.x2 && no_lo_out;
        ProfScope ps(h, cls, ln.stream);
        HIPCHK(h, launch_gemm_ln(gl, rp.ln_rows, ln.stream));
        return 0;
    }
    GemmHArgs g = gemm_h_args(p.mode, p.rm, M, Ahi, Alo, lin, d, K);
    g.C = ln.Y; g.ldc = d;
    if (rp.path == RB_LNX_SMALL) {
        if (rp.merge) {
            g.cmb_O = ln.Opart; g.cmb_ML = ln.MLpart; g.cmb_ns = p.cf.attn_nsplit; g.cmb_nhead = h->nhead;
            g.cmb_Mtot = (unsigned)((size_t)p.sg.nseq * p.sg.S);
        }
        g.ln_gamma = nrm.gamma; g.ln_beta = nrm.beta; g.ln_xh = ln.Xh; g.ln_xl = nullptr;
        g.ln_xl8 = Xl8; g.ln_xchg = ln.ln_xchg; g.ln_eps = 1e-5f; g.ln_no_lo = no_lo_out;
        return run_gemm_lnx_small(h, ln.stream, cls, g, rp.gemm);
    }
    if (int rc = (run_gemm_h<EPI_BIAS, OUT_F32>(h, ln.stream, cls, g, rp.gemm))) return rc;
    return run_add_ln(h, ln.stream, ln.X, ln.Y, nrm.gamma, nrm.beta, M, d, ln.Xh, ln.Xl, p.mxv2, no_lo_out);
}

constexpr size_t kQkv0TableMaxBytes = size_t(512) << 20;
int qkv0_table_steps(int steps, int Ec, int A, int d) {
    const size_t bytes = (size_t)steps * Ec * A * 3 * 4 * d * sizeof(float);
    return bytes <= kQkv0TableMaxBytes ? steps : 1;
}

int qkv0_build_table(jmid_ctx* h, const StepPlan& p, const Lane& ln, const float* hyp_chunk, int step0, int nsteps) {
    const int d = h->d;
    ProfScope ps(h, KC_HYPER, ln.stream);
    Qkv0CoefArgs ca{h->wt.concat1.W, h->wt.concat1.bias, hyp_chunk, p.thyp(step0), ln.coef,
                    nsteps, p.R, d, h->hl.total, h->hl.g1, h->hl.b1, h->range_flag};
    const long total = (long)nsteps * p.R * (d / 4);
    hipLaunchKernelGGL(qkv0_coef_kernel, dim3((int)std::min<long>((total + 255) / 256, 256L * 16)), dim3(256), 0, ln.stream, ca);
    HIPCHK(h, hipGetLastError());
    GemmArgs g{};
    g.A = ln.coef; g.lda = d; g.W = h->wt.layers[0].in_proj.W; g.ldw = d; g.C = ln.uvc; g.ldc = 3 * d;
    g.M = nsteps * p.R * 3; g.N = 3 * d; g.K = d;
    if (h->tune.qkv0 == 2) HIPCHK(h, (launch_gemm_f32<EPI_BIAS, false>(g, ln.stream)));
    else HIPCHK(h, (launch_gemm_f32<EPI_BIAS, true>(g, ln.stream)));
    return 0;
}

constexpr size_t kTailTableMaxBytes = size_t(128) << 20;
int tail_table_steps(int steps, int Ec, int A, int d) {
    const size_t bytes = (size_t)steps * Ec * A * (2 * d + 2) * sizeof(float);
    return bytes <= kTailTableMaxBytes ? steps : 1;
}

int tail_build_table(jmid_ctx* h, const StepPlan& p, const Lane& ln, const float* hyp_chunk, int step0, int nsteps) {
    const WeightTable& wt = h->wt;
    ProfScope ps(h, KC_HYPER, ln.stream);
    TailTableArgs ta{wt.concat3.W, wt.concat3.bias, wt.concat4.W, wt.concat4.bias, wt.linear.W, wt.linear.bias,
                     hyp_chunk, p.thyp(step0), ln.weff, ln.beff,
                     nsteps, p.R, h->d, h->dmid, h->dlow, h->hl.total,
                     h->hl.g3, h->hl.b3, h->hl.g4, h->hl.b4, h->hl.go, h->hl.bo, h->range_flag};
    HIPCHK(h, launch_tail_fold_table(ta, ln.stream));
    return 0;
}

EmbedArgs embed_args(const jmid_ctx* h, const StepPlan& p, const StepBuffers& sb, const float* x_chunk, const float* hyp_chunk, const float* th) {
    unsigned char* Xl8 = p.mxv2 ? reinterpret_cast<unsigned char*>(sb.Xl) : nullptr;
    return EmbedArgs{x_chunk, h->wt.concat1.W, h->wt.concat1.bias, h->pe, hyp_chunk, th,
                     p.mode.split ? nullptr : sb.X, p.M, h->d, h->hl.total, h->hl.g1, h->hl.b1, p.rm, p.mode.split ? sb.Xh : nullptr,
                     p.mode.split && !p.mxv2 ? sb.Xl : nullptr, Xl8};
}

int run_embed(jmid_ctx* h, const StepPlan& p, const Lane& ln, const float* x_chunk, const float* hyp_chunk, const float* thyp) {
    ProfScope ps(h, KC_EMBED, ln.stream);
    EmbedArgs ea = embed_args(h, p, ln, x_chunk, hyp_chunk, thyp);
    const long total = (long)p.M * (h->d / 4);
    int blocks = (int)std::min<long>((total + 255) / 256, 256L * 16);
    hipLaunchKernelGGL(embed_kernel, dim3(blocks), dim3(256), bystander_lds(h->tune.bystander_lds, embed_kernel), ln.stream, ea);
    HIPCHK(h, hipGetLastError());
    return 0;
}

struct LoImages {
    unsigned char *k8h, *k8l, *q8l;
};
LoImages lo_images(const StepPlan& p, const StepBuffers& sb, int d) {
    LoImages im{};
    im.k8h = p.k8 ? reinterpret_cast<unsigned char*>(sb.Kl) : nullptr;
    im.k8l = p.k8 ? im.k8h + (size_t)p.M * d : nullptr;
    im.q8l = p.q8l ? reinterpret_cast<unsigned char*>(sb.Ql) : nullptr;
    return im;
}

int in_proj_planes(jmid_ctx* h, const StepPlan& p, const Lane& ln, int l) {
    const int M = p.M, d = h->d, hd = p.hd, S = p.sg.S;
    const LoImages im = lo_images(p, ln, d);
    const float qscale = p.att_scale * 1.4426950408889634f;
    GemmHArgs g = gemm_h_args(p.mode, p.rm, M, ln.Xh, ln.Xl, h->wt.layers[l].in_proj, 3 * d, d);
    g.Chi = ln.Qh; g.Clo = ln.Ql; g.Khi = ln.Kh; g.Klo = ln.Kl;
    g.Vthi = p.vt_direct ? ln.Vth : ln.Vh; g.Vtlo = p.vt_direct ? ln.Vtl : ln.Vl; g.vt_direct = p.vt_direct;
    g.d = d; g.hd = hd; g.S = S; g.Spad = p.sg.Spad; g.qscale = qscale;
    g.K8h = im.k8h; g.K8l = im.k8l; g.Q8l = im.q8l;
    if (int rc = (run_gemm_h<EPI_BIAS, OUT_QKV>(h, ln.stream, KC_GEMM_QKV, g, p.in_proj))) return rc;
    if (!p.vt_direct) {
        ProfScope ps(h, KC_VTRANS, ln.stream);
        hipLaunchKernelGGL(v_transpose_kernel, dim3((S + 63) / 64, d / 64, p.sg.nseq), dim3(256), 0, ln.stream,
                           ln.Vh, ln.Vl, ln.Vth, ln.Vtl, S, p.sg.Spad, d, hd);
        HIPCHK(h, hipGetLastError());
    }
    return 0;
}

int qkv_planes(jmid_ctx* h, const StepPlan& p, const Lane& ln, int l, int step_idx, const float* x_chunk, const float* hyp_chunk) {
    const int M = p.M, d = h->d, hd = p.hd, S = p.sg.S;
    const LoImages im = lo_images(p, ln, d);
    const float qscale = p.att_scale * 1.4426950408889634f;
    if (l == 0 && p.qkv0) {
        if (p.cf.qkv0_steps <= 1)
            if (int rc = qkv0_build_table(h, p, ln, hyp_chunk, step_idx, 1)) return rc;
        Qkv0Args qa{};
        qa.x = x_chunk;
        qa.uvc = ln.uvc + (p.cf.qkv0_steps <= 1 ? 0 : (size_t)step_idx * p.R * 9 * d);
        qa.ppe = h->ppe;
        qa.Qh = ln.Qh; qa.Ql = ln.Ql; qa.Kh = ln.Kh; qa.Kl = ln.Kl; qa.Vth = ln.Vth; qa.Vtl = ln.Vtl;
        qa.Q8l = im.q8l; qa.K8h = im.k8h; qa.K8l = im.k8l;
        qa.M = M; qa.d = d; qa.hd = hd; qa.S = S; qa.Spad = p.sg.Spad; qa.nseq = p.sg.nseq;
        qa.qscale = qscale; qa.rmap = p.rm; qa.range_flag = h->range_flag; qa.x2 = p.mode.x2;
        qkv0_plan(qa, p.T);
        ProfScope ps(h, KC_GEMM_QKV, ln.stream);
        HIPCHK(h, launch_qkv0_expand(qa, ln.stream));
        return 0;
    }
    return in_proj_planes(h, p, ln, l);
}

OutArgs sampler_args(const jmid_ctx* h, const StepPlan& p, const StepBuffers& sb, int step_idx, float* x_chunk, const float* hyp_chunk,
                     float* e_out, const float* z_chunk) {
    OutArgs oa{sb.Y4, h->wt.linear.W, h->wt.linear.bias, hyp_chunk, p.thyp(step_idx), x_chunk, e_out,
               p.M, h->dlow, h->hl.total, h->hl.go, h->hl.bo,
               h->c_e[step_idx], h->c_x[step_idx], h->n_x[step_idx], h->n_e[step_idx], p.rm,
               nullptr, 0, 0.f, 0.f, 0.f, p.tbo(hyp_chunk)};
    if (h->ddpm && !e_out) {
        oa.ddpm = 1;
        oa.z = h->p_noise[step_idx] ? z_chunk : nullptr;
        oa.c0 = h->p_c0[step_idx];
        oa.c1 = h->p_c1[step_idx];
        oa.sigma = h->p_sigma[step_idx];
    }
    return oa;
}

int folded_tail(jmid_ctx* h, const StepPlan& p, const Lane& ln, int step_idx, float* x_chunk, const float* hyp_chunk,
                float* e_out, const float* z_chunk, int next_step) {
    const int M = p.M, d = h->d;
    if (p.cf.tail_steps <= 1)
        if (int rc = tail_build_table(h, p, ln, hyp_chunk, step_idx, 1)) return rc;
    const size_t at = p.cf.tail_steps <= 1 ? 0 : (size_t)step_idx * p.R;
    const TailFoldArgs fa{ln.Xh, ln.Xl, ln.weff + at * 2 * d, ln.beff + at * 2, d};
    const OutArgs oa = sampler_args(h, p, ln, step_idx, x_chunk, hyp_chunk, e_out, z_chunk);
    const bool embed_next = next_step >= 0 && !e_out;
    const EmbedArgs en = embed_next ? embed_args(h, p, ln, x_chunk, hyp_chunk, p.thyp(next_step)) : EmbedArgs{};
    const bool lo = !p.mode.x2;
    ProfScope ps(h, KC_OUT_DDIM, ln.stream);
    const auto launch = [&](auto* kernel, int waves, auto... tpw) {
        hipLaunchKernelGGL(kernel, dim3((waves + 3) / 4), dim3(256), bystander_lds(h->tune.bystander_lds, kernel), ln.stream, fa, oa, en, tpw...);
    };
    const auto pick = [&](auto embed, auto with_lo) {
        constexpr bool EN = decltype(embed)::value, LO = decltype(with_lo)::value;
        if (p.out_tpw) launch(tail_fold_traj_kernel<EN, LO>, M / p.out_tpw, p.out_tpw);
        else launch(tail_fold_kernel<EN, LO>, M);
    };
    if (embed_next && lo) pick(std::true_type{}, std::true_type{});
    else if (embed_next) pick(std::true_type{}, std::false_type{});
    else if (lo) pick(std::false_type{}, std::true_type{});
    else pick(std::false_type{}, std::false_type{});
    HIPCHK(h, hipGetLastError());
    return 0;
}

int output_stage(jmid_ctx* h, const StepPlan& p, const Lane& ln, int step_idx, float* x_chunk, const float* hyp_chunk,
                 float* e_out, const float* z_chunk, int next_step) {
    const int M = p.M;
    ProfScope ps(h, KC_OUT_DDIM, ln.stream);
    const OutArgs oa = sampler_args(h, p, ln, step_idx, x_chunk, hyp_chunk, e_out, z_chunk);
    const bool embed_next = next_step >= 0 && !e_out;
    const EmbedArgs en = embed_next ? embed_args(h, p, ln, x_chunk, hyp_chunk, p.thyp(next_step)) : EmbedArgs{};
    const auto launch = [&](auto* kernel, int waves, auto... tpw) {
        hipLaunchKernelGGL(kernel, dim3((waves + 3) / 4), dim3(256), bystander_lds(h->tune.bystander_lds, kernel), ln.stream, oa, en, tpw...);
    };
    if (p.out_tpw && embed_next) launch(out_ddim_traj_kernel<true>, M / p.out_tpw, p.out_tpw);
    else if (p.out_tpw) launch(out_ddim_traj_kernel<false>, M / p.out_tpw, p.out_tpw);
    else if (embed_next) launch(out_ddim_kernel<true>, M);
    else launch(out_ddim_kernel<false>, M);
    HIPCHK(h, hipGetLastError());
    return 0;
}

int net_tail(jmid_ctx* h, const StepPlan& p, const Lane& ln, int step_idx, float* x_chunk, const float* hyp_chunk,
             float* e_out, const float* z_chunk, int next_step) {
    if (p.tail_fold) return folded_tail(h, p, ln, step_idx, x_chunk, hyp_chunk, e_out, z_chunk, next_step);
    const int M = p.M, d = h->d;
    const WeightTable& wt = h->wt;
    const float* thyp = p.thyp(step_idx);
    GemmHArgs g = gemm_h_args(p.mode, p.rm, M, ln.Xh, ln.Xl, wt.concat3, h->dmid, d);
    g.hyp = hyp_chunk; g.thyp = thyp; g.hyp_ld = h->hl.total;
    g.Chi = ln.Y3h; g.Clo = ln.Y3l; g.ldc = h->dmid; g.goff = h->hl.g3; g.boff = h->hl.b3;
    if (int rc = (run_gemm_h<EPI_CSL, OUT_SPLIT>(h, ln.stream, KC_GEMM_TAIL, g, p.concat3))) return rc;
    g = gemm_h_args(p.mode, p.rm, M, ln.Y3h, ln.Y3l, wt.concat4, h->dlow, h->dmid);
    g.hyp = hyp_chunk; g.thyp = thyp; g.hyp_ld = h->hl.total;
    g.C = ln.Y4; g.ldc = h->dlow; g.goff = h->hl.g4; g.boff = h->hl.b4;
    if (int rc = (run_gemm_h<EPI_CSL, OUT_F32>(h, ln.stream, KC_GEMM_TAIL, g, p.concat4))) return rc;
    return output_stage(h, p, ln, step_idx, x_chunk, hyp_chunk, e_out, z_chunk, next_step);
}

int net_step(jmid_ctx* h, const StepPlan& p, const Lane& ln, int step_idx, float* x_chunk, const float* hyp_chunk,
             float* e_out, const float* z_chunk = nullptr, bool embed_done = false, int next_step = -1, const unsigned* mask_chunk = nullptr) {
    const bool split = p.mode.split;
    const int M = p.M, d = h->d, ff = h->ff;
    const WeightTable& wt = h->wt;
    const float* thyp = p.thyp(step_idx);
    const RowMap& rm = p.rm;
    if (!embed_done)
        if (int rc = run_embed(h, p, ln, x_chunk, hyp_chunk, thyp)) return rc;
    const SeqGeom& sg = p.sg;
    const int nseq = sg.nseq, S = sg.S, hd = p.hd;
    if (!split) {
        for (const LayerW& w : wt.layers) {
            if (int rc = run_gemm<EPI_BIAS>(h, ln.stream, KC_GEMM_QKV, gemm_args(rm, M, ln.X, w.in_proj, ln.QKV, 3 * d, d))) return rc;
            {
                ProfScope ps(h, KC_ATTN, ln.stream);
                AttnArgs aa{ln.QKV, ln.ATT, S, d, h->nhead, p.att_scale, nullptr, nullptr};
                aa.mask = p.attn.masked ? mask_chunk : nullptr;
                HIPCHK(h, launch_attn_f32(aa, nseq, hd, p.attn.pack, ln.stream));
            }
            if (int rc = run_gemm<EPI_BIAS>(h, ln.stream, KC_GEMM_OUT, gemm_args(rm, M, ln.ATT, w.out_proj, ln.Y, d, d))) return rc;
            if (int rc = run_add_ln(h, ln.stream, ln.X, ln.Y, w.norm1.gamma, w.norm1.beta, M, d)) return rc;
            if (int rc = run_gemm<EPI_BIAS_RELU>(h, ln.stream, KC_GEMM_FF1, gemm_args(rm, M, ln.X, w.linear1, ln.H1, ff, d))) return rc;
            if (int rc = run_gemm<EPI_BIAS>(h, ln.stream, KC_GEMM_FF2, gemm_args(rm, M, ln.H1, w.linear2, ln.Y, d, ff))) return rc;
            if (int rc = run_add_ln(h, ln.stream, ln.X, ln.Y, w.norm2.gamma, w.norm2.beta, M, d)) return rc;
        }
        GemmArgs g = gemm_args(rm, M, ln.X, wt.concat3, ln.Y3, h->dmid, d);
        g.hyp = hyp_chunk; g.thyp = thyp; g.hyp_ld = h->hl.total; g.goff = h->hl.g3; g.boff = h->hl.b3;
        if (int rc = run_gemm<EPI_CSL>(h, ln.stream, KC_GEMM_TAIL, g)) return rc;
        g = gemm_args(rm, M, ln.Y3, wt.concat4, ln.Y4, h->dlow, h->dmid);
        g.hyp = hyp_chunk; g.thyp = thyp; g.hyp_ld = h->hl.total; g.goff = h->hl.g4; g.boff = h->hl.b4;
        if (int rc = run_gemm<EPI_CSL>(h, ln.stream, KC_GEMM_TAIL, g)) return rc;
    } else {
        for (int l = 0; l < h->tf_layer; ++l) {
            const LayerW& w = wt.layers[l];
            GemmHArgs g{};
            if (p.joint) {
                if (int rc = qkv_planes(h, p, ln, l, step_idx, x_chunk, hyp_chunk)) return rc;
                const LoImages im = lo_images(p, ln, d);
                ProfScope ps(h, KC_ATTN, ln.stream);
                AttnHArgs aa{ln.Qh, ln.Ql, ln.Kh, ln.Kl, ln.Vth, ln.Vtl, ln.Ah, ln.Al, S, sg.Spad, d, h->nhead,
                             p.att_scale, h->range_flag, p.cf.attn_nsplit, ln.Opart, ln.MLpart, p.mode.x2, im.k8h, im.k8l, im.q8l};
                aa.skip_combine = p.out_proj.merge;
                HIPCHK(h, launch_attn_f16x3(aa, nseq, hd, p.attn, ln.stream, p.attn.masked ? mask_chunk : nullptr));
            } else {
                g = gemm_h_args(p.mode, rm, M, ln.Xh, ln.Xl, w.in_proj, 3 * d, d);
                g.C = ln.QKV; g.ldc = 3 * d;
                if (int rc = (run_gemm_h<EPI_BIAS, OUT_F32>(h, ln.stream, KC_GEMM_QKV, g, p.in_proj))) return rc;
                ProfScope ps(h, KC_ATTN, ln.stream);
                AttnArgs aa{ln.QKV, nullptr, S, d, h->nhead, p.att_scale, ln.Ah, ln.Al};
                HIPCHK(h, launch_attn_f32(aa, nseq, hd, p.attn.pack, ln.stream));
            }
            if (int rc = residual_block(h, p, p.out_proj, ln, ln.Ah, ln.Al, d, w.out_proj, w.norm1, KC_GEMM_OUT, false)) return rc;
            g = gemm_h_args(p.mode, rm, M, ln.Xh, ln.Xl, w.linear1, ff, d);
            g.Chi = ln.H1h; g.Clo = ln.H1l; g.ldc = ff;
            if (int rc = (run_gemm_h<EPI_BIAS_RELU, OUT_SPLIT>(h, ln.stream, KC_GEMM_FF1, g, p.linear1))) return rc;
            if (int rc = residual_block(h, p, p.linear2, ln, ln.H1h, ln.H1l, ff, w.linear2, w.norm2, KC_GEMM_FF2, l + 1 == h->tf_layer)) return rc;
        }
        return net_tail(h, p, ln, step_idx, x_chunk, hyp_chunk, e_out, z_chunk, next_step);
    }
    return output_stage(h, p, ln, step_idx, x_chunk, hyp_chunk, e_out, z_chunk, next_step);
}

int auto_chunk(const jmid_ctx* h, int E, int tokens_per_episode) {
    const long max_tokens = 65536;
    if (h->net_kind == JMID_NET_JMID) {
        const long bpe = (long)h->nhead * ((tokens_per_episode + 127) / 128);
        for (int k = 4; k >= 1; --k) {
            const long c = (k * 512L) / bpe;
            if (c >= 1 && c * tokens_per_episode <= max_tokens) return (int)std::min<long>(c, E);
        }
    }
    long c = max_tokens / std::max(1, tokens_per_episode);
    if (c < 1) c = 1;
    return (int)std::min<long>(c, E);
}

std::vector<int> plan_chunks(const jmid_ctx* h, const CallMode& m, int E, int tokens_per_episode) {
    int c = h->chunk_eps > 0 ? std::min(E, h->chunk_eps) : auto_chunk(h, E, tokens_per_episode);
    if (h->chunk_eps <= 0 && h->lanes >= 2 && E >= 2 && h->tune.graph != 1) {
        if (E <= c) {
            const long tokens = (long)E * tokens_per_episode;
            const bool lnx_call = one_launch_shape(h, m, tokens) && residual_path(h, m, (int)tokens, h->d, CallFacts{}).path == RB_LNX_SMALL;
            c = lnx_call ? E : (E + 1) / 2;
        } else {
            int n = (E + c - 1) / c;
            if ((n & 1) && n < E) ++n;
            std::vector<int> sizes(n, E / n);
            for (int i = 0; i < E % n; ++i) sizes[i] += 1;
            return sizes;
        }
    }
    std::vector<int> sizes(E / c, c);
    const int tail = E % c;
    if (tail) {
        if (h->chunk_eps > 0 || sizes.empty() || tail * 4 >= c || (tail + sizes.size() - 1) / sizes.size() > (size_t)c / 8)
            sizes.push_back(tail);
        else
            for (int i = 0; i < tail; ++i) sizes[i % sizes.size()] += 1;
    }
    return sizes;
}

int order_in(jmid_ctx* h, int mem) {
    if (mem != JMID_MEM_DEVICE) return 0;
    HIPCHK(h, hipEventRecord(h->ev_in, h->caller_stream));
    HIPCHK(h, hipStreamWaitEvent(h->stream, h->ev_in, 0));
// ... 242 lines not shown
        HIPCHK(h, launch_loss_prepare(pa, h->stream));
    }
    if (cp.nlanes > 1) {
        HIPCHK(h, hipEventRecord(h->ev_fork, h->stream));
        for (int l = 1; l < cp.nlanes; ++l) HIPCHK(h, hipStreamWaitEvent(cp.lanes[l].stream, h->ev_fork, 0));
    }
    return 0;
}

int run_steps(jmid_ctx* h, const DenoiseCall& a, const CallPlan& cp, const CallIo& io) {
    const int E = a.E, A = a.A, K = a.K, T = a.T, lanes = cp.nlanes, nchunks = (int)cp.chunk_sizes.size(), n_steps = (int)h->beta.size();
    const size_t M = (size_t)E * K * A * T, tok = (size_t)K * A * T;
    const bool one = a.single_step >= 0;
    const int i0 = one ? a.single_step : 0, i1 = one ? i0 + 1 : n_steps;
    jmid_ctx::LoopGraph* lg = nullptr;
    bool capturing = false;
    if (a.single_step < 0 && lanes == 1 && nchunks == 1 && !h->prof_mask && !a.z && !h->ddpm && h->tune.graph == 1 &&
        h->tune.bystander_lds == 0) {
        const std::string key = std::to_string(E) + "," + std::to_string(A) + "," + std::to_string(K) + "," + std::to_string(T) +
                                "," + std::to_string(a.precision) + (cp.masked ? ",padded" : "");
        lg = &h->graphs[key];
        if (lg->exec && lg->arena != h->arena.p) {
            hipGraphExecDestroy(lg->exec);
            lg->exec = nullptr;
        }
        if (lg->exec) {
            HIPCHK(h, hipGraphLaunch(lg->exec, h->stream));
            ++h->graph_replays;
        } else if (lg->warm) {
            HIPCHK(h, hipStreamBeginCapture(h->stream, hipStreamCaptureModeThreadLocal));
            capturing = true;
        }
    }
    for (int c0 = 0; c0 < nchunks && !(lg && lg->exec); c0 += lanes) {
        for (int i = i0; i < i1; ++i) {
            for (int l = 0; l < lanes; ++l) {
                if (c0 + l >= nchunks) break;
                const Lane& ln = cp.lanes[l];
                const size_t el = cp.chunk_start[c0 + l];
                float* xc = io.x_cur + el * tok * 2;
                const float* hc = io.hyp + el * A * h->hl.total;
                const float* zc = a.z ? a.z + ((size_t)i * M + el * tok) * 2 : nullptr;
                int rc = 0;
                if (cp.z_fill && h->p_noise[i]) {
                    rc = fill_noise(h, a.seeded->seed, h->noise_ids.get<unsigned>() + el, cp.chunk_sizes[c0 + l], tok * 2, i + 1, ln.z, nullptr, ln.stream);
                    zc = ln.z;
                }
                const StepPlan& pl = cp.plans[cp.chunk_plan[c0 + l]];
                if (!rc && i == 0 && pl.qkv0 && pl.cf.qkv0_steps > 1) rc = qkv0_build_table(h, pl, ln, hc, 0, n_steps);
                if (!rc && i == 0 && pl.tail_fold && pl.cf.tail_steps > 1) rc = tail_build_table(h, pl, ln, hc, 0, n_steps);
                if (!rc) rc = net_step(h, pl, ln, i, xc, hc, one ? io.stage + el * tok * 2 : nullptr, zc, h->tune.fuse_embed && i > i0,
                                        h->tune.fuse_embed && i + 1 < i1 ? i + 1 : -1,
                                        io.mask ? io.mask + el * mask_words_per_seq((int)tok) : nullptr);
                if (rc) {
                    if (capturing) {
                        hipGraph_t dead = nullptr;
                        (void)hipStreamEndCapture(h->stream, &dead);
                        if (dead) hipGraphDestroy(dead);
                    }
                    sync_lanes(h);
                    return rc;
                }
            }
        }
    }
    if (capturing) {
        hipGraph_t graph = nullptr;
        HIPCHK(h, hipStreamEndCapture(h->stream, &graph));
        hipError_t ge = hipGraphInstantiate(&lg->exec, graph, nullptr, nullptr, 0);
        hipGraphDestroy(graph);
        if (ge != hipSuccess) {
            lg->exec = nullptr;
            return fail(h, JMID_EHIP, std::string("hipGraphInstantiate: ") + hipGetErrorString(ge));
        }
        lg->arena = h->arena.p;
        HIPCHK(h, hipGraphLaunch(lg->exec, h->stream));
        ++h->graph_replays;
    } else if (lg && !lg->exec) {
        lg->warm = true;
    }
    return 0;
}

int finish_call(jmid_ctx* h, const DenoiseCall& a, const CallPlan& cp, const CallIo& io) {
    const size_t R = (size_t)a.E * a.K * a.A, M = R * a.T;
    const hipMemcpyKind kout = a.mem == JMID_MEM_HOST ? hipMemcpyDeviceToHost : hipMemcpyDeviceToDevice;
    for (int l = 1; l < cp.nlanes; ++l) {
        HIPCHK(h, hipEventRecord(h->ev_join[l - 1], cp.lanes[l].stream));
        HIPCHK(h, hipStreamWaitEvent(h->stream, h->ev_join[l - 1], 0));
    }
    const float qnan = std::numeric_limits<float>::quiet_NaN();
    if (const LossCall* lc = a.loss) {
        const LossReduceArgs ra{io.stage, io.e_dev, io.nag, io.loss_rows, io.loss, (int)R, a.A, a.T * 2};
        {
            ProfScope ps(h, KC_LOSS_REDUCE, h->stream);
            HIPCHK(h, launch_loss_reduce(ra, h->stream));
        }
        HIPCHK(h, hipMemcpyAsync(lc->loss_out, io.loss, 2 * sizeof(double), kout, h->stream));
        if (lc->row_out) HIPCHK(h, hipMemcpyAsync(lc->row_out, io.loss_rows, R * sizeof(double), kout, h->stream));
    }
    if (cp.masked) HIPCHK(h, launch_pad_fill(a.single_step >= 0 ? io.stage : io.x_cur, io.nag, a.E, a.K, a.A, a.T * 2, qnan, h->stream));
    if (a.single_step >= 0) {
        if (a.e_out) HIPCHK(h, hipMemcpyAsync(a.e_out, io.stage, M * 2 * sizeof(float), kout, h->stream));
    } else {
        if (a.vel_out) HIPCHK(h, hipMemcpyAsync(a.vel_out, io.x_cur, M * 2 * sizeof(float), kout, h->stream));
        if (a.p0) {
            {
                ProfScope ps(h, KC_INTEGRATE, h->stream);
                const int n = (int)R * 2;
                hipLaunchKernelGGL(integrate_kernel, dim3((n + 255) / 256), dim3(256), 0, h->stream, io.x_cur, a.p0,
                                   io.stage, (int)R, a.T, a.A, a.K * a.A, a.dt);
                HIPCHK(h, hipGetLastError());
            }
            h->last_pos = io.stage;
            h->last_pos_dims[0] = a.E; h->last_pos_dims[1] = a.A; h->last_pos_dims[2] = a.K; h->last_pos_dims[3] = a.T;
            if (a.pos_out) HIPCHK(h, hipMemcpyAsync(a.pos_out, io.stage, M * 2 * sizeof(float), kout, h->stream));
        }
    }
    if (a.chained) return 0;
    if (int rc = order_out(h, a.mem)) return rc;
    int flag = 0;
    if (cp.mode.split) HIPCHK(h, hipMemcpyAsync(&flag, h->range_flag, sizeof(int), hipMemcpyDeviceToHost, h->stream));
    if (cp.mode.split || a.mem == JMID_MEM_HOST) HIPCHK(h, hipStreamSynchronize(h->stream));
    return flag ? flagged_call(h, flag) : 0;
}

int run_network(jmid_ctx* h, DenoiseCall a) {
    CallMode mode;
    if (int rc = check_call(h, a, &mode)) return rc;
    CallPlan cp = plan_call(h, a, mode);
    HIPCHK(h, hipSetDevice(h->device));
    if (!a.chained)
        if (int rc = order_in(h, a.mem)) return rc;
    CallIo io;
    if (int rc = fill_workspace(h, a, cp, io)) return rc;
    if (int rc = run_steps(h, a, cp, io)) return rc;
    return finish_call(h, a, cp, io);
}

int flagged_call(jmid_ctx* h, int flag) {
    h->last_pos = nullptr;
    if (flag & 2) {
        h->lnx_off = true;
        ++h->lnx_timeouts;
        return fail(h, JMID_ETIMEOUT, "a workgroup of a one-launch GEMM + LayerNorm gave up waiting for its partners (not all workgroups of the launch "
                                      "were resident): this handle now runs the unfused kernels - repeat the call in the same precision");
    }
    ++h->erange_calls;
    return fail(h, JMID_ERANGE, "an activation left the fp16 range in JMID_PREC_F16X3 / F16X2 / F16MX: rerun with JMID_PREC_F32");
}

#ifdef JMID_DIAGNOSTICS
int dbg_step(jmid_ctx* h, bool tail, int E, int A, int K, int T, const float* in, const float* hyp, int hyp_width, int step, int precision,
             float* out, float* thyp_row) {
    const std::string who = tail ? "jmid_dbg_tail" : "jmid_dbg_qkv0";
    CallMode mode;
    if (int rc = check_ready(h)) return rc;
    if (!in || !hyp || !out || E <= 0 || A <= 0 || K <= 0 || T <= 0 || T > kPeMaxLen) return fail(h, JMID_EINVAL, who + ": bad arguments");
    if (hyp_width != h->hl.total) return fail(h, JMID_EINVAL, who + ": hyp rows must be " + std::to_string(h->hl.total) + " wide");
    if (!call_mode(precision, &mode) || !mode.split || (!tail && h->net_kind != JMID_NET_JMID))
        return fail(h, JMID_EINVAL, who + (tail ? ": a split-fp16 mode only" : ": JMID in a split-fp16 mode only"));
    if (step < 0 || step >= (int)h->beta.size()) return fail(h, JMID_EINVAL, who + ": step outside the step table");
    HIPCHK(h, hipSetDevice(h->device));
    h->last_pos = nullptr;
    const size_t M = (size_t)E * K * A * T, EA = (size_t)E * A;
    const int d = h->d, in_w = tail ? d : 2, out_w = tail ? 2 : 3 * d;
    const StepPlan p = plan_step(h, E, A, K, T, mode, CallFacts{});
    const size_t qkv0_rows = !tail && p.qkv0 ? EA * 3 : 0, tail_rows = tail && p.tail_fold ? EA : 0;
    float *in_d, *hyp_d, *out_d;
    const auto io = [&](char* base) {
        Carver c(base);
        in_d = c.take(M * in_w);
        hyp_d = c.take(EA * h->hl.total);
        out_d = c.take(M * out_w);
        return c.off;
    };
    const size_t io_off = io(nullptr);
    if (int rc = ensure_arena(h, io_off + step_ws_floats(h, M, mode, p.sg, 1, nullptr, nullptr, qkv0_rows, tail_rows), who.c_str())) return rc;
    io(h->arena.p);
    Lane ln{};
    ln.stream = h->stream;
    step_ws_floats(h, M, mode, p.sg, 1, &ln, h->arena.p + io_off, qkv0_rows, tail_rows);
    HIPCHK(h, hipMemsetAsync(h->range_flag, 0, sizeof(int), h->stream));
    if (!tail) {
        HIPCHK(h, hipMemsetAsync(ln.Vth, 0, ln.vt_elems * sizeof(half_t), h->stream));
        HIPCHK(h, hipMemsetAsync(ln.Vtl, 0, ln.vt_elems * sizeof(half_t), h->stream));
    }
    HIPCHK(h, hipMemcpyAsync(in_d, in, M * in_w * sizeof(float), hipMemcpyHostToDevice, h->stream));
    HIPCHK(h, hipMemcpyAsync(hyp_d, hyp, EA * h->hl.total * sizeof(float), hipMemcpyHostToDevice, h->stream));
    if (tail) {
        HIPCHK(h, hipMemsetAsync(ln.Xh, 0, blk_plane_elems(M, d) * sizeof(half_t), h->stream));
        HIPCHK(h, hipMemsetAsync(ln.Xl, 0, blk_plane_elems(M, d) * sizeof(half_t), h->stream));
        hipLaunchKernelGGL(tail_split_rows_kernel, dim3(512), dim3(256), 0, h->stream, in_d, ln.Xh, mode.x2 ? nullptr : ln.Xl, (int)M, d);
        HIPCHK(h, hipGetLastError());
        if (int rc = net_tail(h, p, ln, step, nullptr, hyp_d, out_d, nullptr, -1)) return rc;
    } else {
        if (int rc = run_embed(h, p, ln, in_d, hyp_d, p.thyp(step))) return rc;
        if (int rc = qkv_planes(h, p, ln, 0, step, in_d, hyp_d)) return rc;
        const LoImages im = lo_images(p, ln, d);
        QkvReadArgs ra{ln.Qh, ln.Ql, ln.Kh, ln.Kl, ln.Vth, ln.Vtl, im.q8l, im.k8l, out_d, M, d, p.hd, p.sg.S, p.sg.Spad, mode.x2,
                       p.att_scale * 1.4426950408889634f};
        hipLaunchKernelGGL(qkv_planes_read_kernel, dim3(512), dim3(256), 0, h->stream, ra);
        HIPCHK(h, hipGetLastError());
    }
    int flag = 0;
    HIPCHK(h, hipMemcpyAsync(&flag, h->range_flag, sizeof(int), hipMemcpyDeviceToHost, h->stream));
    HIPCHK(h, hipMemcpyAsync(out, out_d, M * out_w * sizeof(float), hipMemcpyDeviceToHost, h->stream));
    if (thyp_row)
        HIPCHK(h, hipMemcpyAsync(thyp_row, p.thyp(step), h->hl.total * sizeof(float), hipMemcpyDeviceToHost, h->stream));
    HIPCHK(h, hipStreamSynchronize(h->stream));
    return flag ? flagged_call(h, flag) : 0;
}

int dbg_layer(jmid_ctx* h, int E, int A, int K, int T, int layer, int precision, const float* X, const int32_t* n_agents, int last,
              float* hi, float* lo, int* plan) {
    const std::string who = "jmid_dbg_layer";
    CallMode mode;
    if (int rc = check_ready(h)) return rc;
    if (!X || !hi || !lo || !plan || E <= 0 || A <= 0 || K <= 0 || T <= 0 || T > kPeMaxLen) return fail(h, JMID_EINVAL, who + ": bad arguments");
    if (!call_mode(precision, &mode)) return fail(h, JMID_EINVAL, who + ": bad precision");
    if (layer < 0 || layer >= h->tf_layer) return fail(h, JMID_EINVAL, who + ": layer outside the encoder");
    if (mode.split && !h->weights_in_half_range) return fail(h, JMID_ERANGE, who + ": a weight exceeds the fp16 range");
    if (n_agents) {
        if (int rc = check_n_agents(h, who.c_str(), n_agents, E, A)) return rc;
        if (h->net_kind == JMID_NET_JMID && mode.split && !attn_masked_built(plan_attn(h->d / h->nhead, h->tune), mode.x2 != 0))
            return fail(h, JMID_EINVAL, who + ": the attention kernel these knobs select has no masked form");
    }
    HIPCHK(h, hipSetDevice(h->device));
    h->last_pos = nullptr;
    DenoiseCall call{};
    call.E = E; call.A = A; call.K = K; call.T = T; call.precision = precision; call.mem = JMID_MEM_HOST;
    call.single_step = 0; call.n_agents = n_agents; call.who = "jmid_dbg_layer";
    CallFacts cf = plan_call(h, call, mode).facts;
    cf.small_now = 1;
    cf.one_chunk = h->tune.graph != 1;
    const StepPlan p = plan_step(h, E, A, K, T, mode, cf, n_agents != nullptr);
    const bool split = mode.split, joint = p.joint;
    const int M = p.M, d = h->d, ff = h->ff, S = p.sg.S, nseq = p.sg.nseq, hd = p.hd;
    const size_t Mz = (size_t)M, width = 7 * (size_t)d + ff;
    const size_t off[6] = {0, (size_t)d, 4 * (size_t)d, 5 * (size_t)d, 6 * (size_t)d, 6 * (size_t)d + ff};
    const bool mask_words = n_agents && joint;
    float *in_d, *hi_d, *lo_d;
    unsigned* mask_d;
    const auto io = [&](char* base) {
        Carver c(base);
        in_d = c.take(Mz * d);
        hi_d = c.take(Mz * width);
        lo_d = c.take(Mz * width);
        mask_d = mask_words ? reinterpret_cast<unsigned*>(c.take((size_t)E * mask_words_per_seq(S))) : nullptr;
        return c.off;
    };
    const size_t io_off = io(nullptr);
    if (int rc = ensure_arena(h, io_off + step_ws_floats(h, Mz, mode, p.sg, cf.attn_nsplit, nullptr, nullptr, 0, 0), who.c_str())) return rc;
    io(h->arena.p);
    Lane ln{};
    ln.stream = h->stream;
    step_ws_floats(h, Mz, mode, p.sg, cf.attn_nsplit, &ln, h->arena.p + io_off, 0, 0);
    hipStream_t st = h->stream;
    HIPCHK(h, hipMemsetAsync(lo_d, 0, Mz * width * sizeof(float), st));
    HIPCHK(h, hipMemcpyAsync(in_d, X, Mz * d * sizeof(float), hipMemcpyHostToDevice, st));
    if (mask_words) {
        if (int rc = h->nag.upload(h, n_agents, E, who.c_str())) return rc;
        HIPCHK(h, launch_mask_words(h->nag.get<int>(), mask_d, E, A, T, S, st));
    }
    unsigned char* Xl8 = p.mxv2 ? reinterpret_cast<unsigned char*>(ln.Xl) : nullptr;
    const auto out_hi = [&](int s) { return hi_d + Mz * off[s]; };
    const auto out_lo = [&](int s) { return lo_d + Mz * off[s]; };
    const auto copy_f32 = [&](int s, const float* src, size_t w) {
        return hipMemcpyAsync(out_hi(s), src, Mz * w * sizeof(float), hipMemcpyDeviceToDevice, st);
    };
    const auto read_x = [&](int s, bool lo_written) {
        if (!split) return copy_f32(s, ln.X, d);
        if (p.mxv2) hipLaunchKernelGGL(merge_planes_lo8_kernel, dim3(512), dim3(256), 0, st, ln.Xh, lo_written ? Xl8 : nullptr, out_hi(s), M, out_lo(s));
        else hipLaunchKernelGGL(merge_planes_kernel, dim3(512), dim3(256), 0, st, ln.Xh, lo_written ? ln.Xl : nullptr, out_hi(s), M, d, out_lo(s));
        return hipGetLastError();
    };
    const auto read_planes = [&](int s, const half_t* ph, const half_t* pl, int w) {
        hipLaunchKernelGGL(merge_planes_kernel, dim3(512), dim3(256), 0, st, ph, pl, out_hi(s), M, w, out_lo(s));
        return hipGetLastError();
    };
    int stages = 0;
    if (!split) {
        HIPCHK(h, hipMemcpyAsync(ln.X, in_d, Mz * d * sizeof(float), hipMemcpyDeviceToDevice, st));
    } else {
        HIPCHK(h, hipMemsetAsync(h->range_flag, 0, sizeof(int), st));
        HIPCHK(h, hipMemsetAsync(ln.ln_xchg, 0, kLnxWords * sizeof(unsigned), st));
        half_t* const planes[6] = {ln.Xh, ln.Xl, ln.Ah, ln.Al, ln.H1h, ln.H1l};
        const int plane_w[6] = {d, d, d, d, ff, ff};
        for (int i = 0; i < 6; ++i) HIPCHK(h, hipMemsetAsync(planes[i], 0, blk_plane_elems(Mz, plane_w[i]) * sizeof(half_t), st));
        if (ln.Vth) {
            HIPCHK(h, hipMemsetAsync(ln.Vth, 0, ln.vt_elems * sizeof(half_t), st));
            HIPCHK(h, hipMemsetAsync(ln.Vtl, 0, ln.vt_elems * sizeof(half_t), st));
        }
        if (p.mxv2) hipLaunchKernelGGL(split_planes_lo8_kernel, dim3(512), dim3(256), 0, st, in_d, ln.Xh, Xl8, M);
        else hipLaunchKernelGGL(split_planes_blocked_kernel, dim3(512), dim3(256), 0, st, in_d, ln.Xh, ln.Xl, M, d, h->range_flag, 1.0f);
        HIPCHK(h, hipGetLastError());
    }
    HIPCHK(h, read_x(0, true));
    stages |= 1;
    const LayerW& w = h->wt.layers[layer];
    const RowMap& rm = p.rm;
    if (!split) {
        if (int rc = run_gemm<EPI_BIAS>(h, st, KC_GEMM_QKV, gemm_args(rm, M, ln.X, w.in_proj, ln.QKV, 3 * d, d))) return rc;
        HIPCHK(h, copy_f32(1, ln.QKV, 3 * (size_t)d));
        AttnArgs aa{ln.QKV, ln.ATT, S, d, h->nhead, p.att_scale, nullptr, nullptr};
        aa.mask = p.attn.masked ? mask_d : nullptr;
        HIPCHK(h, launch_attn_f32(aa, nseq, hd, p.attn.pack, st));
        HIPCHK(h, copy_f32(2, ln.ATT, d));
        stages |= 6;
        if (int rc = run_gemm<EPI_BIAS>(h, st, KC_GEMM_OUT, gemm_args(rm, M, ln.ATT, w.out_proj, ln.Y, d, d))) return rc;
        if (int rc = run_add_ln(h, st, ln.X, ln.Y, w.norm1.gamma, w.norm1.beta, M, d)) return rc;
        HIPCHK(h, read_x(3, true));
        if (int rc = run_gemm<EPI_BIAS_RELU>(h, st, KC_GEMM_FF1, gemm_args(rm, M, ln.X, w.linear1, ln.H1, ff, d))) return rc;
        HIPCHK(h, copy_f32(4, ln.H1, ff));
        if (int rc = run_gemm<EPI_BIAS>(h, st, KC_GEMM_FF2, gemm_args(rm, M, ln.H1, w.linear2, ln.Y, d, ff))) return rc;
        if (int rc = run_add_ln(h, st, ln.X, ln.Y, w.norm2.gamma, w.norm2.beta, M, d)) return rc;
        HIPCHK(h, read_x(5, true));
        stages |= 56;
    } else {
        GemmHArgs g{};
        if (joint) {
            if (int rc = in_proj_planes(h, p, ln, layer)) return rc;
            const LoImages im = lo_images(p, ln, d);
            QkvReadArgs ra{ln.Qh, ln.Ql, ln.Kh, ln.Kl, ln.Vth, ln.Vtl, im.q8l, im.k8l, out_hi(1), Mz, d, hd, S, p.sg.Spad, mode.x2,
                           p.att_scale * 1.4426950408889634f, out_lo(1)};
            hipLaunchKernelGGL(qkv_planes_read_kernel, dim3(512), dim3(256), 0, st, ra);
            HIPCHK(h, hipGetLastError());
            AttnHArgs aa{ln.Qh, ln.Ql, ln.Kh, ln.Kl, ln.Vth, ln.Vtl, ln.Ah, ln.Al, S, p.sg.Spad, d, h->nhead,
                         p.att_scale, h->range_flag, p.cf.attn_nsplit, ln.Opart, ln.MLpart, p.mode.x2, im.k8h, im.k8l, im.q8l};
            aa.skip_combine = p.out_proj.merge;
            HIPCHK(h, launch_attn_f16x3(aa, nseq, hd, p.attn, st, p.attn.masked ? mask_d : nullptr));
            if (!p.out_proj.merge) {
                HIPCHK(h, read_planes(2, ln.Ah, mode.x2 ? nullptr : ln.Al, d));
                stages |= 4;
            }
        } else {
            g = gemm_h_args(p.mode, rm, M, ln.Xh, ln.Xl, w.in_proj, 3 * d, d);
            g.C = ln.QKV; g.ldc = 3 * d;
            if (int rc = (run_gemm_h<EPI_BIAS, OUT_F32>(h, st, KC_GEMM_QKV, g, p.in_proj))) return rc;
            HIPCHK(h, copy_f32(1, ln.QKV, 3 * (size_t)d));
            AttnArgs aa{ln.QKV, nullptr, S, d, h->nhead, p.att_scale, ln.Ah, ln.Al};
            HIPCHK(h, launch_attn_f32(aa, nseq, hd, p.attn.pack, st));
            HIPCHK(h, read_planes(2, ln.Ah, ln.Al, d));
            stages |= 4;
        }
        stages |= 2;
        if (int rc = residual_block(h, p, p.out_proj, ln, ln.Ah, ln.Al, d, w.out_proj, w.norm1, KC_GEMM_OUT, false)) return rc;
        HIPCHK(h, read_x(3, true));
        g = gemm_h_args(p.mode, rm, M, ln.Xh, ln.Xl, w.linear1, ff, d);
        g.Chi = ln.H1h; g.Clo = ln.H1l; g.ldc = ff;
        if (int rc = (run_gemm_h<EPI_BIAS_RELU, OUT_SPLIT>(h, st, KC_GEMM_FF1, g, p.linear1))) return rc;
        HIPCHK(h, read_planes(4, ln.H1h, mode.x2 ? nullptr : ln.H1l, ff));
        if (int rc = residual_block(h, p, p.linear2, ln, ln.H1h, ln.H1l, ff, w.linear2, w.norm2, KC_GEMM_FF2, last != 0)) return rc;
        HIPCHK(h, read_x(5, !(last && mode.x2)));
        stages |= 56;
    }
    const auto block_mode = [&](const ResidualPlan& rp, const LinearW& lin) {
        if (rp.path == RB_GEMM_LN2 || rp.path == RB_LNX_SMALL) return (int)GM_MX;
        if (rp.path == RB_GEMM_LN) return (int)(mode.mx && lin.w8 ? GM_MX : mode.x2 ? GM_X2 : GM_X3);
        return (int)rp.gemm.mode;
// ... 28 lines not shown
```

### safe-interactive-crowdnav_amd/csrc/qkv0.hpp

```cpp
#pragma once
#include "common.hpp"
#include "gemm_f16x3.hpp"

namespace jmid {

struct Qkv0CoefArgs {
    const float* W1;
    const float* b1;
    const float* hyp;
    const float* thyp;
    float* coef;
    int steps, R, d, hyp_ld, goff, boff;
    int* range_flag;
};

static __global__ __launch_bounds__(256) void qkv0_coef_kernel(Qkv0CoefArgs a) {
    const int d4 = a.d >> 2;
    const long total = (long)a.steps * a.R * d4;
    bool overflow = false;
    for (long idx = (long)blockIdx.x * blockDim.x + threadIdx.x; idx < total; idx += (long)gridDim.x * blockDim.x) {
        const int j = (int)(idx % d4) * 4;
        const long sr = idx / d4;
        const int r = (int)(sr % a.R), s = (int)(sr / a.R);
        const float* hrow = a.hyp + (size_t)r * a.hyp_ld;
        const float* th = a.thyp + (size_t)s * a.hyp_ld;
        f32x4 u, v, c;
#pragma unroll
        for (int e = 0; e < 4; ++e) {
            const int cc = j + e;
            const float gate = sigmoidf_(hrow[a.goff + cc] + th[a.goff + cc]);
            const float bias = hrow[a.boff + cc] + th[a.boff + cc];
            u[e] = a.W1[2 * cc] * gate;
            v[e] = a.W1[2 * cc + 1] * gate;
            c[e] = a.b1[cc] * gate + bias;
            overflow |= !(fabsf(u[e]) <= kHalfMax) || !(fabsf(v[e]) <= kHalfMax) || !(fabsf(c[e]) <= kHalfMax);
        }
        float* o = a.coef + (size_t)sr * 3 * a.d + j;
        *reinterpret_cast<f32x4*>(o) = u;
        *reinterpret_cast<f32x4*>(o + a.d) = v;
        *reinterpret_cast<f32x4*>(o + 2 * a.d) = c;
    }
    if (overflow) atomicOr(a.range_flag, 1);
}

struct Qkv0Args {
    const float* x;
    const float* uvc;
    const float* ppe;
    half_t *Qh, *Ql, *Kh, *Kl;
    half_t *Vth, *Vtl;
    unsigned char *Q8l, *K8h, *K8l;
    int M, d, hd, S, Spad, nseq;
    float qscale;
    RowMap rmap;
    int* range_flag;
    int x2;
    int tpw;
    int qk_slabs;
    int qk_blocks;
    int v_cpw;
    int v_kblocks;
    int v_same_row;
};

__device__ __forceinline__ float qkv0_value(float x0, float x1, float u, float v, float c, float p) {
    return fmaf(x0, u, fmaf(x1, v, c)) + p;
}

__device__ __forceinline__ void qkv0_expand_qk(const Qkv0Args& a, int wave, int lane) {
    const int piece = wave / a.qk_slabs, slab = wave - piece * a.qk_slabs;
    const int m0 = piece * a.tpw;
    const int j = slab * 256 + lane * 4;
    if (m0 >= a.M || j >= 2 * a.d) return;
    const int part = j >= a.d, nn = j - part * a.d, n3 = 3 * a.d;
    const int t0 = a.rmap.t_of(m0);
    const float* row = a.uvc + (size_t)a.rmap.ea(m0) * 3 * n3 + j;
    const f32x4 u = *reinterpret_cast<const f32x4*>(row);
    const f32x4 v = *reinterpret_cast<const f32x4*>(row + n3);
    const f32x4 c = *reinterpret_cast<const f32x4*>(row + 2 * n3);
    const float qs = part == 0 ? a.qscale : 1.0f;
    unsigned amax16 = 0;
    for (int i = 0; i < a.tpw; ++i) {
        const int m = m0 + i;
        const float x0 = a.x[2 * (size_t)m], x1 = a.x[2 * (size_t)m + 1];
        const f32x4 p = *reinterpret_cast<const f32x4*>(a.ppe + (size_t)(t0 + i) * n3 + j);
        float o[4];
#pragma unroll
        for (int e = 0; e < 4; ++e) {
            o[e] = qkv0_value(x0, x1, u[e], v[e], c[e], p[e]);
            if (part == 0) o[e] *= qs;
        }
        const Split4 sp = split_f32x4(o[0], o[1], o[2], o[3], amax16);
        const size_t at = (size_t)m * a.d + nn;
        if (part == 0) {
            store_stream(reinterpret_cast<i32x2_s*>(a.Qh + at), sp.hi);
            if (a.Q8l) store_stream(reinterpret_cast<int*>(a.Q8l + at), bf8_of_f16x4(sp.lo[0], sp.lo[1]));
            else store_stream(reinterpret_cast<i32x2_s*>(a.Ql + at), sp.lo);
        } else {
            store_stream(reinterpret_cast<i32x2_s*>(a.Kh + at), sp.hi);
            if (a.K8h) {
                store_stream(reinterpret_cast<int*>(a.K8h + at), bf8_of_f16x4(sp.hi[0], sp.hi[1]));
                store_stream(reinterpret_cast<int*>(a.K8l + at), bf8_of_f16x4(sp.lo[0], sp.lo[1]));
            } else {
                store_stream(reinterpret_cast<i32x2_s*>(a.Kl + at), sp.lo);
            }
        }
    }
    if (split_range_exceeded(amax16)) atomicOr(a.range_flag, 1);
}

__device__ __forceinline__ void qkv0_expand_v(const Qkv0Args& a, int wave, int lane) {
    const int slabs = a.d / a.v_cpw;
    const int per_seq = a.v_kblocks * slabs;
    const int seq = wave / per_seq, rest = wave - seq * per_seq;
    const int kb = rest / slabs, slab = rest - kb * slabs;
    const int k0 = (kb * 64 + lane) * 4;
    if (seq >= a.nseq || k0 >= a.S) return;
    const int n3 = 3 * a.d, nh = a.d / a.hd;
    float x0[4], x1[4];
    const float *rowp[4], *pep[4];
    bool live[4];
#pragma unroll
    for (int q = 0; q < 4; ++q) {
        live[q] = k0 + q < a.S;
        const int m = seq * a.S + (live[q] ? k0 + q : k0);
        x0[q] = a.x[2 * (size_t)m];
        x1[q] = a.x[2 * (size_t)m + 1];
        rowp[q] = a.uvc + (size_t)a.rmap.ea(m) * 3 * n3 + 2 * a.d;
        pep[q] = a.ppe + (size_t)a.rmap.t_of(m) * n3 + 2 * a.d;
    }
    const size_t pos = vt_key_pos(k0);
    unsigned amax16 = 0;
    for (int cc = slab * a.v_cpw; cc < (slab + 1) * a.v_cpw; cc += 4) {
        f32x4 u[4], v[4], c[4], p[4];
#pragma unroll
        for (int q = 0; q < 4; ++q) {
            if (q == 0 || !a.v_same_row) {
                u[q] = *reinterpret_cast<const f32x4*>(rowp[q] + cc);
                v[q] = *reinterpret_cast<const f32x4*>(rowp[q] + n3 + cc);
                c[q] = *reinterpret_cast<const f32x4*>(rowp[q] + 2 * n3 + cc);
            } else {
                u[q] = u[0];
                v[q] = v[0];
                c[q] = c[0];
            }
            p[q] = *reinterpret_cast<const f32x4*>(pep[q] + cc);
        }
#pragma unroll
        for (int e = 0; e < 4; ++e) {
            float o[4];
#pragma unroll
            for (int q = 0; q < 4; ++q) o[q] = live[q] ? qkv0_value(x0[q], x1[q], u[q][e], v[q][e], c[q][e], p[q][e]) : 0.f;
            const Split4 sp = split_f32x4(o[0], o[1], o[2], o[3], amax16);
            const int ch = cc + e, head = ch / a.hd, vc = ch - head * a.hd;
            const size_t at = (((size_t)seq * nh + head) * a.hd + vc) * a.Spad + pos;
            store_stream(reinterpret_cast<i32x2_s*>(a.Vth + at), sp.hi);
            if (!a.x2) store_stream(reinterpret_cast<i32x2_s*>(a.Vtl + at), sp.lo);
        }
    }
    if (split_range_exceeded(amax16)) atomicOr(a.range_flag, 1);
}

static __global__ __launch_bounds__(256) void qkv0_expand_kernel(Qkv0Args a) {
    args_now(a);
    const int lane = threadIdx.x & 63, w = threadIdx.x >> 6;
    if ((int)blockIdx.x < a.qk_blocks) qkv0_expand_qk(a, blockIdx.x * 4 + w, lane);
    else qkv0_expand_v(a, ((int)blockIdx.x - a.qk_blocks) * 4 + w, lane);
}

inline void qkv0_plan(Qkv0Args& a, int T) {
    a.qk_slabs = (2 * a.d + 255) / 256;
    a.tpw = T;
    while (a.tpw > 1 && ((long)(a.M / a.tpw) * a.qk_slabs < 4096 || T % a.tpw != 0)) --a.tpw;
    a.qk_blocks = (int)(((long)(a.M / a.tpw) * a.qk_slabs + 3) / 4);
    a.v_kblocks = (a.S + 255) / 256;
    a.v_cpw = a.d % 16 == 0 ? 16 : 4;
    while (a.v_cpw > 4 && (long)a.nseq * a.v_kblocks * (a.d / a.v_cpw) < 4096) a.v_cpw >>= 1;
    a.v_same_row = T % 4 == 0 && a.S % 4 == 0;
}
inline hipError_t launch_qkv0_expand(const Qkv0Args& a, hipStream_t st) {
    const long v_waves = (long)a.nseq * a.v_kblocks * (a.d / a.v_cpw);
    const int blocks = a.qk_blocks + (int)((v_waves + 3) / 4);
    hipLaunchKernelGGL(qkv0_expand_kernel, dim3(blocks), dim3(256), 0, st, a);
    return hipGetLastError();
}

#ifdef JMID_DIAGNOSTICS
struct QkvReadArgs {
    const half_t *Qh, *Ql, *Kh, *Kl, *Vth, *Vtl;
    const unsigned char *Q8l, *K8l;
    float* out;
    size_t M;
    int d, hd, S, Spad, x2;
    float qscale;
    float* out_lo = nullptr;
};
__device__ __forceinline__ float f32_of_bf8(unsigned char b) {
    return (float)__builtin_bit_cast(half_t, (unsigned short)((unsigned)b << 8));
}
static __global__ void qkv_planes_read_kernel(QkvReadArgs a) {
    const size_t n = a.M * a.d;
    for (size_t i = (size_t)blockIdx.x * blockDim.x + threadIdx.x; i < n; i += (size_t)gridDim.x * blockDim.x) {
        const size_t m = i / a.d;
        const int c = (int)(i % a.d);
        const size_t seq = m / a.S, key = m % a.S;
        const int head = c / a.hd, vc = c % a.hd;
        const size_t at = ((seq * (a.d / a.hd) + head) * a.hd + vc) * a.Spad + (size_t)vt_key_pos((int)key);
        const float qh = (float)a.Qh[i], ql = a.Q8l ? f32_of_bf8(a.Q8l[i]) : (float)a.Ql[i];
        const float kh = (float)a.Kh[i], kl = a.K8l ? f32_of_bf8(a.K8l[i]) : (float)a.Kl[i];
        const float vh = (float)a.Vth[at], vl = a.x2 ? 0.f : (float)a.Vtl[at];
        float* o = a.out + m * 3 * a.d;
        if (a.out_lo) {
            float* ol = a.out_lo + m * 3 * a.d;
            o[c] = qh / a.qscale;
            ol[c] = ql / a.qscale;
            o[a.d + c] = kh;
            ol[a.d + c] = kl;
            o[2 * a.d + c] = vh;
            ol[2 * a.d + c] = vl;
        } else {
            o[c] = (qh + ql) / a.qscale;
            o[a.d + c] = kh + kl;
            o[2 * a.d + c] = vh + vl;
        }
    }
}
#endif

}
```

### safe-interactive-crowdnav_amd/csrc/tail_fold.hpp

```cpp
#pragma once
#include <cfloat>

#include "common.hpp"
#include "elementwise.hpp"

namespace jmid {

constexpr int kTailG = 8;
constexpr int kTailMaxD = 512, kTailMaxMid = 256, kTailMaxLow = 128;

struct TailTableArgs {
    const float *W3, *b3;
    const float *W4, *b4;
    const float *Wo, *bo;
    const float* hyp;
    const float* thyp;
    float* weff;
    float* beff;
    int steps, R, d, dmid, dlow, hyp_ld;
    int g3, b3o, g4, b4o, go, boo;
    int* range_flag;
};

static __global__ __launch_bounds__(256) void tail_fold_table_kernel(TailTableArgs a) {
// ... 19 lines not shown
        for (int o = 0; o < 2; ++o) {
            const float go = sigmoidf_(hr[a.go + o] + th[a.go + o]);
            s_v[c][2 * g + o] = go * a.Wo[o * a.dlow + c] * g4;
        }
    }
    __syncthreads();

    for (int j = tid; j < a.dmid; j += 256) {
        float acc[G2];
#pragma unroll
        for (int k = 0; k < G2; ++k) acc[k] = 0.f;
        for (int c0 = 0; c0 < a.dlow; c0 += 32) {
            float part[G2];
#pragma unroll
            for (int k = 0; k < G2; ++k) part[k] = 0.f;
            const int c1 = c0 + 32 < a.dlow ? c0 + 32 : a.dlow;
#pragma unroll 8
            for (int c = c0; c < c1; ++c) {
                const float w = a.W4[(size_t)c * a.dmid + j];
#pragma unroll
                for (int k4 = 0; k4 < G2; k4 += 4) {
                    const f32x4 v = *reinterpret_cast<const f32x4*>(&s_v[c][k4]);
#pragma unroll
                    for (int e = 0; e < 4; ++e) part[k4 + e] = fmaf(v[e], w, part[k4 + e]);
                }
            }
#pragma unroll
            for (int k = 0; k < G2; ++k) acc[k] += part[k];
        }
        const float b3 = a.b3[j];
        float u[G2];
#pragma unroll
        for (int g = 0; g < kTailG; ++g) {
            const float *hr = hrow(g), *th = trow(g);
            const float g3 = sigmoidf_(hr[a.g3 + j] + th[a.g3 + j]);
            s_t3[g][j] = g3 * b3 + (hr[a.b3o + j] + th[a.b3o + j]);
            u[2 * g] = acc[2 * g] * g3;
            u[2 * g + 1] = acc[2 * g + 1] * g3;
        }
#pragma unroll
        for (int k4 = 0; k4 < G2; k4 += 4) {
            *reinterpret_cast<f32x4*>(&s_q[j][k4]) = f32x4{acc[k4], acc[k4 + 1], acc[k4 + 2], acc[k4 + 3]};
            *reinterpret_cast<f32x4*>(&s_u[j][k4]) = f32x4{u[k4], u[k4 + 1], u[k4 + 2], u[k4 + 3]};
        }
    }
    __syncthreads();

    if (tid < G2 && p0 + (tid >> 1) < pairs) {
        const int g = tid >> 1, o = tid & 1;
        float sj = 0.f;
        for (int j0 = 0; j0 < a.dmid; j0 += 32) {
            float part = 0.f;
            const int j1 = j0 + 32 < a.dmid ? j0 + 32 : a.dmid;
            for (int j = j0; j < j1; ++j) part = fmaf(s_q[j][tid], s_t3[g][j], part);
            sj += part;
        }
        float sc = 0.f;
        for (int c0 = 0; c0 < a.dlow; c0 += 32) {
            float part = 0.f;
            const int c1 = c0 + 32 < a.dlow ? c0 + 32 : a.dlow;
            for (int c = c0; c < c1; ++c) part = fmaf(a.Wo[o * a.dlow + c], s_t4[g][c], part);
            sc += part;
        }
        const float *hr = hrow(g), *th = trow(g);
        const float go = sigmoidf_(hr[a.go + o] + th[a.go + o]);
        const float be = sj + go * sc + go * a.bo[o] + (hr[a.boo + o] + th[a.boo + o]);
        a.beff[(size_t)(p0 + g) * 2 + o] = be;
        bad |= !(fabsf(be) <= FLT_MAX);
    }

    {
        const int i0 = tid, i1 = tid + 256;
        const bool on0 = i0 < a.d, on1 = i1 < a.d;
        const float* w0p = a.W3 + (on0 ? i0 : 0);
        const float* w1p = a.W3 + (on1 ? i1 : 0);
        float acc0[G2], acc1[G2];
#pragma unroll
        for (int k = 0; k < G2; ++k) acc0[k] = acc1[k] = 0.f;
        for (int j0 = 0; j0 < a.dmid; j0 += 32) {
            float part0[G2], part1[G2];
#pragma unroll
            for (int k = 0; k < G2; ++k) part0[k] = part1[k] = 0.f;
            const int j1 = j0 + 32 < a.dmid ? j0 + 32 : a.dmid;
#pragma unroll 4
            for (int j = j0; j < j1; ++j) {
                const float w0 = w0p[(size_t)j * a.d], w1 = w1p[(size_t)j * a.d];
#pragma unroll
                for (int k4 = 0; k4 < G2; k4 += 4) {
                    const f32x4 u = *reinterpret_cast<const f32x4*>(&s_u[j][k4]);
#pragma unroll
                    for (int e = 0; e < 4; ++e) {
                        part0[k4 + e] = fmaf(u[e], w0, part0[k4 + e]);
                        part1[k4 + e] = fmaf(u[e], w1, part1[k4 + e]);
                    }
                }
            }
#pragma unroll
            for (int k = 0; k < G2; ++k) {
                acc0[k] += part0[k];
                acc1[k] += part1[k];
            }
        }
#pragma unroll
        for (int k = 0; k < G2; ++k) {
            if (p0 + (k >> 1) >= pairs) break;
            float* row = a.weff + ((size_t)(p0 + (k >> 1)) * 2 + (k & 1)) * a.d;
            if (on0) {
                row[i0] = acc0[k];
                bad |= !(fabsf(acc0[k]) <= FLT_MAX);
            }
            if (on1) {
                row[i1] = acc1[k];
                bad |= !(fabsf(acc1[k]) <= FLT_MAX);
            }
        }
    }
    if (bad) atomicOr(a.range_flag, 1);
}

inline hipError_t launch_tail_fold_table(const TailTableArgs& a, hipStream_t st) {
    const long pairs = (long)a.steps * a.R;
    hipLaunchKernelGGL(tail_fold_table_kernel, dim3((unsigned)((pairs + kTailG - 1) / kTailG)), dim3(256), 0, st, a);
    return hipGetLastError();
}

struct TailFoldArgs {
    const half_t* Xh;
    const half_t* Xl;
    const float* weff;
    const float* beff;
    int d;
};

struct TailMap {
    f32x4 w[2][2];
    float b0, b1;
};
__device__ __forceinline__ void tail_fold_map(const TailFoldArgs& f, int ea, int lane, TailMap& t) {
    const bool on = lane * 8 < f.d;
#pragma unroll
    for (int o = 0; o < 2; ++o) {
        const float* row = f.weff + ((size_t)ea * 2 + o) * f.d + lane * 8;
        t.w[o][0] = on ? *reinterpret_cast<const f32x4*>(row) : f32x4{0.f, 0.f, 0.f, 0.f};
        t.w[o][1] = on ? *reinterpret_cast<const f32x4*>(row + 4) : f32x4{0.f, 0.f, 0.f, 0.f};
    }
    t.b0 = f.beff[(size_t)ea * 2];
    t.b1 = f.beff[(size_t)ea * 2 + 1];
}
__device__ __forceinline__ f16x8 tail_fold_load(const half_t* plane, int d, int m, int lane) {
    f16x8 x = {0, 0, 0, 0, 0, 0, 0, 0};
    if (lane * 8 < d) x = *reinterpret_cast<const f16x8*>(plane + blk_index(m, lane * 8, d));
    return x;
}
template <bool LO>
__device__ __forceinline__ void tail_fold_dot(f16x8 xh, f16x8 xl, const TailMap& t, float& e0, float& e1) {
    float s0 = 0.f, s1 = 0.f;
#pragma unroll
    for (int e = 0; e < 8; ++e) {
        const float v = LO ? (float)xh[e] + (float)xl[e] : (float)xh[e];
        s0 = fmaf(v, t.w[0][e >> 2][e & 3], s0);
        s1 = fmaf(v, t.w[1][e >> 2][e & 3], s1);
    }
    e0 = wave_sum(s0) + t.b0;
    e1 = wave_sum(s1) + t.b1;
}
__device__ __forceinline__ void tail_fold_update(const OutArgs& a, float e0, float e1, float x0, float x1, float z0, float z1,
                                                 float& xn0, float& xn1) {
    if (a.ddpm) {
        xn0 = a.c0 * (x0 - a.c1 * e0) + a.sigma * z0;
        xn1 = a.c0 * (x1 - a.c1 * e1) + a.sigma * z1;
    } else {
        const float p0 = (x0 - e0 * a.c_e) / a.c_x, p1 = (x1 - e1 * a.c_e) / a.c_x;
        xn0 = a.n_x * p0 + a.n_e * e0;
        xn1 = a.n_x * p1 + a.n_e * e1;
    }
}

template <bool EMBED_NEXT, bool LO>
__global__ __launch_bounds__(256) void tail_fold_kernel(TailFoldArgs f, OutArgs a, EmbedArgs nxt) {
    args_now_each(f, a, nxt);
    const int lane = threadIdx.x & 63;
    const int m = blockIdx.x * (blockDim.x >> 6) + (threadIdx.x >> 6);
    if (m >= a.M) return;
    const f16x8 xh = tail_fold_load(f.Xh, f.d, m, lane);
    const f16x8 xl = LO ? tail_fold_load(f.Xl, f.d, m, lane) : xh;
    TailMap t;
    tail_fold_map(f, a.rmap.ea(m), lane, t);
    const float x0 = a.e_out ? 0.f : a.x[2 * (size_t)m], x1 = a.e_out ? 0.f : a.x[2 * (size_t)m + 1];
    const float z0 = (a.ddpm && a.z) ? a.z[2 * (size_t)m] : 0.f, z1 = (a.ddpm && a.z) ? a.z[2 * (size_t)m + 1] : 0.f;
    float e0, e1;
    tail_fold_dot<LO>(xh, xl, t, e0, e1);
    float xn0 = 0.f, xn1 = 0.f;
    if (a.e_out) {
        if (lane == 0) {
            a.e_out[2 * (size_t)m] = e0;
            a.e_out[2 * (size_t)m + 1] = e1;
        }
    } else {
        tail_fold_update(a, e0, e1, x0, x1, z0, z1, xn0, xn1);
        if (lane == 0) {
            a.x[2 * (size_t)m] = xn0;
            a.x[2 * (size_t)m + 1] = xn1;
        }
    }
    if (EMBED_NEXT) embed_row(nxt, m, lane, xn0, xn1);
}

template <bool EMBED_NEXT, bool LO>
__global__ __launch_bounds__(256) void tail_fold_traj_kernel(TailFoldArgs f, OutArgs a, EmbedArgs nxt, int tpw) {
    args_now_each(f, a, nxt);
    const int lane = threadIdx.x & 63;
    const int piece = blockIdx.x * (blockDim.x >> 6) + (threadIdx.x >> 6);
    const int m0 = piece * tpw;
    if (m0 >= a.M) return;
    const int t0 = a.rmap.t_of(m0), ea = a.rmap.ea(m0);
    EmbedCols c[2];
    const int j0 = lane * 4, j1 = lane * 4 + 256;
    if (EMBED_NEXT) {
        const float* hrow = nxt.hyp + (size_t)ea * nxt.hyp_ld;
        if (j0 < nxt.d) embed_cols(nxt, j0, hrow, c[0]);
        if (j1 < nxt.d) embed_cols(nxt, j1, hrow, c[1]);
    }
    TailMap t;
    tail_fold_map(f, ea, lane, t);
    for (int tb = 0; tb < tpw; tb += 12) {
        const int nb = tpw - tb < 12 ? tpw - tb : 12;
        f16x8 xh[12], xl[LO ? 12 : 1];
#pragma unroll
        for (int u = 0; u < 12; ++u) {
            const int m = m0 + tb + (u < nb ? u : 0);
            xh[u] = tail_fold_load(f.Xh, f.d, m, lane);
            if (LO) xl[LO ? u : 0] = tail_fold_load(f.Xl, f.d, m, lane);
        }
        const int mu = m0 + tb + (lane < nb ? lane : 0);
        const float xl0 = a.e_out ? 0.f : a.x[2 * (size_t)mu], xl1 = a.e_out ? 0.f : a.x[2 * (size_t)mu + 1];
        const float zl0 = (a.ddpm && a.z) ? a.z[2 * (size_t)mu] : 0.f, zl1 = (a.ddpm && a.z) ? a.z[2 * (size_t)mu + 1] : 0.f;
#pragma unroll
        for (int u = 0; u < 12; ++u) {
            if (u >= nb) continue;
            const int m = m0 + tb + u;
            float e0, e1;
            tail_fold_dot<LO>(xh[u], LO ? xl[LO ? u : 0] : xh[u], t, e0, e1);
            float xn0 = 0.f, xn1 = 0.f;
            if (a.e_out) {
                if (lane == 0) {
                    a.e_out[2 * (size_t)m] = e0;
                    a.e_out[2 * (size_t)m + 1] = e1;
                }
            } else {
                tail_fold_update(a, e0, e1, __shfl(xl0, u, 64), __shfl(xl1, u, 64), __shfl(zl0, u, 64), __shfl(zl1, u, 64), xn0, xn1);
                if (lane == 0) {
                    a.x[2 * (size_t)m] = xn0;
                    a.x[2 * (size_t)m + 1] = xn1;
                }
            }
            if (EMBED_NEXT) {
                if (j0 < nxt.d) embed_store_cols(nxt, m, j0, t0 + tb + u, xn0, xn1, c[0]);
                if (j1 < nxt.d) embed_store_cols(nxt, m, j1, t0 + tb + u, xn0, xn1, c[1]);
            }
        }
    }
}

#ifdef JMID_DIAGNOSTICS
static __global__ void tail_split_rows_kernel(const float* in, half_t* hi, half_t* lo, int rows, int K) {
    const size_t n = (size_t)rows * K;
    for (size_t i = (size_t)blockIdx.x * blockDim.x + threadIdx.x; i < n; i += (size_t)gridDim.x * blockDim.x) {
        half_t h, l;
        split_f32(in[i], h, l);
        const size_t o = blk_index((int)(i / K), (int)(i % K), K);
        hi[o] = h;
        if (lo) lo[o] = l;
    }
}
#endif

}
```

### safe-interactive-crowdnav_amd/engine.py

```python
from __future__ import annotations

import ctypes as C
import math
from typing import Dict, Optional, Tuple, Union

import numpy as np

from . import _lib
from ._lib import JmidError
from .schedule import VarianceSchedule, ddim_steps, ddpm_steps, loss_tables
from .weights import JMIDWeights

try:
    import torch
except Exception:
    torch = None

ArrayLike = Union[np.ndarray, "torch.Tensor"]

ERANGE_EVENTS: list = []
TIMEOUT_EVENTS: list = []


def _is_cuda(t) -> bool:
# ... 670 lines not shown
            E, A, K, T = (int(v) for v in dims)
            dev, bp = False, None
        else:
            dev = _is_cuda(pos)
            E, K, A, T, _ = (int(v) for v in pos.shape)
            bp = _Buf(pos, dev)
        shapes = (((E, K, A * (A - 1) // 2), np.float32) if pairs else None, ((E, K, A), np.uint8) if agents else None,
                  ((E, K, 4), np.float32), ((E, 5), np.float32))
        outs = [_out(*s, pos.device if dev else None) if s else None for s in shapes]
        if n_agents is not None:
            na = agent_counts(n_agents, E)
            self._check(self._lib.jmid_collision_statistics_padded(self._h, E, A, K, T, _ptr(na), bp.ptr if bp is not None else None,
                                                                   float(threshold), *[_ptr(o) for o in outs], self._mem(dev)))
            return tuple(outs)
        self._check(self._lib.jmid_collision_statistics(self._h, E, A, K, T, bp.ptr if bp is not None else None, float(threshold),
                                                        *[_ptr(o) for o in outs], self._mem(dev)))
        return tuple(outs)

    def repair_collisions(self, pos: Optional[ArrayLike], threshold: float = 0.2, margin: float = 0.02, tau: float = 0.005, step: float = 0.02,
                          max_iter: int = 32, p0: Optional[ArrayLike] = None, dt: float = 0.25, vel: Optional[ArrayLike] = None,
                          dims: Optional[Tuple[int, int, int, int]] = None, n_agents=None, want_pos: Optional[bool] = None):
        if pos is None:
            if dims is None:
                raise ValueError("pos=None needs dims=(E, A, K, T) of the preceding denoise call")
            E, A, K, T = (int(v) for v in dims)
            like = vel if vel is not None else p0
            dev, bp = like is not None and _is_cuda(like), None
            want_pos = bool(want_pos)
        else:
            dev, like = _is_cuda(pos), pos
            E, K, A, T, _ = (int(v) for v in pos.shape)
            bp = _Buf(pos, dev)
            want_pos = True if want_pos is None else bool(want_pos)
        if vel is not None and p0 is None:
            raise ValueError("vel needs p0 (a velocity's first step starts at the present position)")
        if p0 is not None and tuple(p0.shape) != (E, A, 2):
            raise ValueError("p0 must be [E, A, 2]")
        if vel is not None and tuple(vel.shape) != (E, K, A, T, 2):
            raise ValueError("vel must be [E, K, A, T, 2]")
        b0 = _Buf(p0, dev) if p0 is not None else None
        where = like.device if dev else None
        vel_out = None
        if vel is not None:
            bv = _Buf(vel, dev)
            vel_out = bv.keep.clone() if dev else np.array(bv.keep, dtype=np.float32, copy=True)
        pos_out = _out((E, K, A, T, 2), device=where) if want_pos else None
        sample, episode = _out((E, K, 4), device=where), _out((E, 3), np.int32, where)
        na = agent_counts(n_agents, E) if n_agents is not None else None
        self._check(self._lib.jmid_repair_collisions(self._h, E, A, K, T, _ptr(na), bp.ptr if bp is not None else None,
                                                     b0.ptr if b0 is not None else None, float(dt), float(threshold), float(margin), float(tau),
                                                     float(step), int(max_iter), _ptr(pos_out), _ptr(vel_out), _ptr(sample), _ptr(episode),
                                                     self._mem(dev)))
        return pos_out, vel_out, sample, episode

    def wall_statistics(self, pos: Optional[ArrayLike], walls, radius: float, p0: Optional[ArrayLike] = None,
                        dims: Optional[Tuple[int, int, int, int]] = None, n_agents=None):
        w = wall_segments(walls)
        L = int(w.shape[0])
        if pos is None:
            if dims is None:
                raise ValueError("pos=None needs dims=(E, A, K, T) of the preceding denoise call")
            E, A, K, T = (int(v) for v in dims)
            dev, bp = p0 is not None and _is_cuda(p0), None
        else:
            dev = _is_cuda(pos)
            E, K, A, T, _ = (int(v) for v in pos.shape)
            bp = _Buf(pos, dev)
        if p0 is not None and tuple(p0.shape) != (E, A, 2):
            raise ValueError("p0 must be [E, A, 2]")
        b0 = _Buf(p0, dev) if p0 is not None else None
        where = (pos if pos is not None else p0).device if dev else None
        outs = [_out((E, K, A, L), np.float32, where), _out((E, K, A), np.uint8, where), _out((E, K, 3), np.float32, where),
                _out((E, 5), np.float32, where)]
        if n_agents is not None:
            na = agent_counts(n_agents, E)
            self._check(self._lib.jmid_wall_statistics_padded(self._h, E, A, K, T, _ptr(na), bp.ptr if bp is not None else None,
                                                              b0.ptr if b0 is not None else None, L, _ptr(w) if L else None, float(radius),
                                                              *[_ptr(o) for o in outs], self._mem(dev)))
            return tuple(outs)
        self._check(self._lib.jmid_wall_statistics(self._h, E, A, K, T, bp.ptr if bp is not None else None, b0.ptr if b0 is not None else None,
                                                   L, _ptr(w) if L else None, float(radius), *[_ptr(o) for o in outs], self._mem(dev)))
        return tuple(outs)

    def kernel_classes(self):
        return [self._lib.jmid_kernel_class_name(i).decode() for i in range(self._lib.jmid_kernel_class_count())]

    def profile_enable(self, classes=None) -> None:
        names = self.kernel_classes()
        mask = 0
        for i, n in enumerate(names):
            if classes is None or n in classes:
                mask |= 1 << i
        self._check(self._lib.jmid_profile_enable(self._h, mask))

    def profile_disable(self) -> None:
        self._check(self._lib.jmid_profile_enable(self._h, 0))

    def profile_reset(self) -> None:
        self._check(self._lib.jmid_profile_reset(self._h))

    def profile_get(self) -> Dict[str, Tuple[int, float]]:
        out = {}
        for i, n in enumerate(self.kernel_classes()):
            cnt, ms = C.c_int64(0), C.c_double(0.0)
            self._check(self._lib.jmid_profile_get(self._h, i, C.byref(cnt), C.byref(ms)))
            out[n] = (int(cnt.value), float(ms.value))
        return out

    def dbg_gemm(self, A: np.ndarray, Wt: np.ndarray, bias: Optional[np.ndarray], relu: bool = False,
                 precision: str = "f32") -> np.ndarray:
        A = np.ascontiguousarray(A, np.float32)
        Wt = np.ascontiguousarray(Wt, np.float32)
        M, K = A.shape
        N = Wt.shape[0]
        out = np.empty((M, N), np.float32)
        b = np.ascontiguousarray(bias, np.float32) if bias is not None else None
        self._check(self._lib.jmid_dbg_gemm(self._h, M, N, K, C.c_void_p(A.ctypes.data), C.c_void_p(Wt.ctypes.data),
                                            C.c_void_p(b.ctypes.data) if b is not None else None, int(relu),
                                            _lib.PRECISIONS[precision], C.c_void_p(out.ctypes.data)))
        return out

    def dbg_attention(self, qkv: np.ndarray, nseq: int, S: int, precision: str = "f32") -> np.ndarray:
        qkv = np.ascontiguousarray(qkv, np.float32)
        d = 2 * self.dims.ctx_dim
        assert qkv.shape == (nseq * S, 3 * d)
        out = np.empty((nseq * S, d), np.float32)
        self._check(self._lib.jmid_dbg_attention(self._h, nseq, S, C.c_void_p(qkv.ctypes.data),
                                                 _lib.PRECISIONS[precision], C.c_void_p(out.ctypes.data)))
        return out

    def dbg_gemm_ln_mx(self, A: np.ndarray, Wt: np.ndarray, bias, gamma, beta, X: np.ndarray, fused) -> np.ndarray:
        A = np.ascontiguousarray(A, np.float32)
        Wt = np.ascontiguousarray(Wt, np.float32)
        X = np.array(X, np.float32, order="C", copy=True)
        v = [np.ascontiguousarray(t, np.float32) for t in (bias, gamma, beta)]
        M, K = A.shape
        assert Wt.shape == (512, K) and X.shape == (M, 512)
        self._check(self._lib.jmid_dbg_gemm_ln_mx(self._h, M, K, C.c_void_p(A.ctypes.data), C.c_void_p(Wt.ctypes.data),
                                                  *[C.c_void_p(t.ctypes.data) for t in v], C.c_void_p(X.ctypes.data),
                                                  int(fused)))
        return X

    def dbg_add_layernorm(self, X: np.ndarray, Y: np.ndarray, gamma: np.ndarray, beta: np.ndarray) -> np.ndarray:
        X = np.array(X, np.float32, order="C", copy=True)
        Y = np.ascontiguousarray(Y, np.float32)
        g = np.ascontiguousarray(gamma, np.float32)
        b = np.ascontiguousarray(beta, np.float32)
        M, d = X.shape
        self._check(self._lib.jmid_dbg_add_layernorm(self._h, M, d, C.c_void_p(X.ctypes.data),
                                                     C.c_void_p(Y.ctypes.data), C.c_void_p(g.ctypes.data),
                                                     C.c_void_p(b.ctypes.data)))
        return X

    def dbg_qkv0(self, x: np.ndarray, hyp: np.ndarray, step: int, dims: Tuple[int, int, int, int], precision: str = "f16mx"):
        E, A, K, T = (int(v) for v in dims)
        x = np.ascontiguousarray(x, np.float32)
        hyp = np.ascontiguousarray(hyp, np.float32)
        M, d = E * K * A * T, 2 * self.dims.ctx_dim
        width = self.hyper_width()
        if x.shape != (M, 2) or hyp.shape != (E * A, width):
            raise ValueError(f"expected x [{M}, 2] and hyp [{E * A}, {width}]")
        out = np.empty((M, 3 * d), np.float32)
        thyp = np.empty((width,), np.float32)
        self._check(self._lib.jmid_dbg_qkv0(self._h, E, A, K, T, C.c_void_p(x.ctypes.data), C.c_void_p(hyp.ctypes.data), width, int(step),
                                            _lib.PRECISIONS[precision], C.c_void_p(out.ctypes.data), C.c_void_p(thyp.ctypes.data)))
        return out, thyp

    def dbg_tail(self, X: np.ndarray, hyp: np.ndarray, step: int, dims: Tuple[int, int, int, int], precision: str = "f16mx"):
        E, A, K, T = (int(v) for v in dims)
        X = np.ascontiguousarray(X, np.float32)
        hyp = np.ascontiguousarray(hyp, np.float32)
        M, d = E * K * A * T, 2 * self.dims.ctx_dim
        width = self.hyper_width()
        if X.shape != (M, d) or hyp.shape != (E * A, width):
            raise ValueError(f"expected X [{M}, {d}] and hyp [{E * A}, {width}]")
        out = np.empty((M, 2), np.float32)
        thyp = np.empty((width,), np.float32)
        self._check(self._lib.jmid_dbg_tail(self._h, E, A, K, T, C.c_void_p(X.ctypes.data), C.c_void_p(hyp.ctypes.data), width, int(step),
                                            _lib.PRECISIONS[precision], C.c_void_p(out.ctypes.data), C.c_void_p(thyp.ctypes.data)))
        return out, thyp

    LAYER_PLAN_FIELDS = ("stages", "in_proj_mode", "in_proj_shape", "in_proj_flags", "linear1_mode", "linear1_shape", "linear1_flags",
                         "out_proj_path", "out_proj_ln_rows", "out_proj_gemm_shape", "linear2_path", "linear2_ln_rows", "linear2_gemm_shape",
                         "vt_direct", "k8", "q8l", "attn_nsplit", "masked", "merge", "byte_lo", "attn_dma", "range_flag", "out_proj_mode", "linear2_mode", "attn_pack")

    def dbg_layer(self, X: np.ndarray, layer: int, dims: Tuple[int, int, int, int], precision: str = "f16mx", n_agents=None, last: bool = False):
        E, A, K, T = (int(v) for v in dims)
        X = np.ascontiguousarray(X, np.float32)
        M, d, ff = E * K * A * T, self.dims.d_model, self.dims.d_ff
        if X.shape != (M, d):
            raise ValueError(f"expected X [{M}, {d}]")
        nag = None
        if n_agents is not None:
            nag = np.ascontiguousarray(n_agents, np.int32)
            if nag.shape != (E,):
                raise ValueError(f"expected n_agents [{E}]")
        widths = (d, 3 * d, d, d, ff, d)
        total = sum(widths)
        hi, lo = np.empty((M * total,), np.float32), np.empty((M * total,), np.float32)
        plan = (C.c_int * len(self.LAYER_PLAN_FIELDS))()
        self._check(self._lib.jmid_dbg_layer(self._h, E, A, K, T, int(layer), _lib.PRECISIONS[precision], C.c_void_p(X.ctypes.data),
                                             C.c_void_p(nag.ctypes.data) if nag is not None else None, int(bool(last)),
                                             C.c_void_p(hi.ctypes.data), C.c_void_p(lo.ctypes.data), plan))
        plan = dict(zip(self.LAYER_PLAN_FIELDS, (int(v) for v in plan)))
        stages, at = [], 0
        for s, w in enumerate(widths):
            pair = (hi[M * at:M * (at + w)].reshape(M, w), lo[M * at:M * (at + w)].reshape(M, w))
            stages.append(pair if plan["stages"] >> s & 1 else None)
            at += w
        return stages, plan

    def hyper_width(self) -> int:
        return 2 * self.dims.d_model + 2 * self.dims.d_mid + 2 * self.dims.d_low + 4
```

Measured before the change: 51010 traj/s.

## Rework qkv0 expand and tail_fold seam kernels for wider lanes and occupancy-aware rows

The qkv0 Q/K expand now has each lane handle 8 columns (512-wide slabs) and batches 6 token rows per pass, using readlane to broadcast per-row inputs. A new seam_tokens_per_wave heuristic picks tokens-per-wave from resident-wave capacity instead of a fixed 4096-wave threshold, and it is applied to both qkv0 and tail_fold. The tail_fold kernels gain DPP/permlane wave reductions and waves_per_eu hints. The old versions are kept behind diagnostic tuning value 3. Fewer waves doing more rows each should cut per-wave overhead and redundant loads, at the risk of reduced parallelism and higher register pressure.

After: 51160 traj/s, median of 6. Within noise of the previous version (+0.3%).

```diff
diff --git a/include/jmid_hip.h b/include/jmid_hip.h
--- a/include/jmid_hip.h
+++ b/include/jmid_hip.h
@@ -223,6 +223,8 @@
                           int64_t* scene);
 int jmid_dbg_qkv0(jmid_handle_t h, int E, int A, int K, int T, const float* x, const float* hyp, int hyp_width, int step, int precision,
                   float* qkv, float* thyp_row);
+int jmid_dbg_qkv0_planes(jmid_handle_t h, int E, int A, int K, int T, const float* x, const float* hyp, int hyp_width, int step, int precision,
+                         float* hi, float* lo, float* thyp_row);
 int jmid_dbg_tail(jmid_handle_t h, int E, int A, int K, int T, const float* X, const float* hyp, int hyp_width, int step, int precision,
                   float* e, float* thyp_row);
 #define JMID_DBG_LAYER_WIDTH(d_model, d_ff) (7 * (d_model) + (d_ff))
diff --git a/safe-interactive-crowdnav_amd/_lib.py b/safe-interactive-crowdnav_amd/_lib.py
--- a/safe-interactive-crowdnav_amd/_lib.py
+++ b/safe-interactive-crowdnav_amd/_lib.py
@@ -141,6 +141,7 @@
     "jmid_dbg_gemm_plan": (C.c_int, [C.c_int] * 8 + [C.POINTER(C.c_int), C.POINTER(C.c_int)]),
     "jmid_dbg_chain_layout": (C.c_int, [C.c_int] * 9 + [C.POINTER(C.c_int64)] * 3),
     "jmid_dbg_qkv0": (C.c_int, [Handle, C.c_int, C.c_int, C.c_int, C.c_int, C.c_void_p, C.c_void_p, C.c_int, C.c_int, C.c_int, C.c_void_p, C.c_void_p]),
+    "jmid_dbg_qkv0_planes": (C.c_int, [Handle, C.c_int, C.c_int, C.c_int, C.c_int, C.c_void_p, C.c_void_p, C.c_int, C.c_int, C.c_int, C.c_void_p, C.c_void_p, C.c_void_p]),
     "jmid_dbg_tail": (C.c_int, [Handle, C.c_int, C.c_int, C.c_int, C.c_int, C.c_void_p, C.c_void_p, C.c_int, C.c_int, C.c_int, C.c_void_p, C.c_void_p]),
     "jmid_dbg_layer": (C.c_int, [Handle, C.c_int, C.c_int, C.c_int, C.c_int, C.c_int, C.c_int, C.c_void_p, C.c_void_p, C.c_int,
                                  C.c_void_p, C.c_void_p, C.POINTER(C.c_int)]),
diff --git a/safe-interactive-crowdnav_amd/csrc/common.hpp b/safe-interactive-crowdnav_amd/csrc/common.hpp
--- a/safe-interactive-crowdnav_amd/csrc/common.hpp
+++ b/safe-interactive-crowdnav_amd/csrc/common.hpp
@@ -189,6 +189,18 @@
     return n;
 }
 
+inline int seam_tokens_per_wave(int M, int T, int waves_per_piece) {
+    constexpr long kResident = 256 * 4 * 4;
+    int one_round = 0;
+    for (int c = T; c >= 1; --c) {
+        if (T % c != 0) continue;
+        const long waves = (long)(M / c) * waves_per_piece;
+        if (c >= 4 && waves >= 3 * kResident) return c;
+        if (!one_round && waves >= kResident) one_round = c;
+    }
+    return one_round ? one_round : 1;
+}
+
 __device__ __forceinline__ float sigmoidf_(float x) { return 1.0f / (1.0f + expf(-x)); }
 
 __device__ __forceinline__ float wave_sum(float v) {
diff --git a/safe-interactive-crowdnav_amd/csrc/jmid_abi.hip b/safe-interactive-crowdnav_amd/csrc/jmid_abi.hip
--- a/safe-interactive-crowdnav_amd/csrc/jmid_abi.hip
+++ b/safe-interactive-crowdnav_amd/csrc/jmid_abi.hip
@@ -1470,8 +1470,8 @@
         {"small_lnx2", &Tuning::small_lnx2, 0, 2},
         {"small_qk", &Tuning::small_qk, 0, 2},
         {"small_pn", &Tuning::small_pn, 0, 8},
-        {"qkv0", &Tuning::qkv0, 0, 2},
-        {"tail_fold", &Tuning::tail_fold, 0, 2},
+        {"qkv0", &Tuning::qkv0, 0, 3},
+        {"tail_fold", &Tuning::tail_fold, 0, 3},
 #ifdef JMID_ABLATIONS
         {"attn_abl", &Tuning::attn_abl, 0, 1 << 30},
         {"gemm_abl", &Tuning::gemm_abl, 0, 1 << 30},
diff --git a/safe-interactive-crowdnav_amd/csrc/jmid_ctx.hpp b/safe-interactive-crowdnav_amd/csrc/jmid_ctx.hpp
--- a/safe-interactive-crowdnav_amd/csrc/jmid_ctx.hpp
+++ b/safe-interactive-crowdnav_amd/csrc/jmid_ctx.hpp
@@ -362,7 +362,7 @@
 int check_n_agents(jmid_ctx* h, const char* who, const int32_t* n_agents, int E, int A);
 int run_network(jmid_ctx* h, DenoiseCall a);
 int dbg_step(jmid_ctx* h, bool tail, int E, int A, int K, int T, const float* in, const float* hyp, int hyp_width, int step, int precision,
-             float* out, float* thyp_row);
+             float* out, float* thyp_row, float* out_lo = nullptr);
 int dbg_layer(jmid_ctx* h, int E, int A, int K, int T, int layer, int precision, const float* X, const int32_t* n_agents, int last,
               float* hi, float* lo, int* plan);
 int flagged_call(jmid_ctx* h, int flag);
diff --git a/safe-interactive-crowdnav_amd/csrc/jmid_diag.hip b/safe-interactive-crowdnav_amd/csrc/jmid_diag.hip
--- a/safe-interactive-crowdnav_amd/csrc/jmid_diag.hip
+++ b/safe-interactive-crowdnav_amd/csrc/jmid_diag.hip
@@ -298,6 +298,11 @@
     return h ? dbg_step(h, false, E, A, K, T, x, hyp, hyp_width, step, precision, qkv, thyp_row) : JMID_EINVAL;
 }
 
+int jmid_dbg_qkv0_planes(jmid_handle_t h, int E, int A, int K, int T, const float* x, const float* hyp, int hyp_width, int step, int precision,
+                         float* hi, float* lo, float* thyp_row) {
+    return h && lo ? dbg_step(h, false, E, A, K, T, x, hyp, hyp_width, step, precision, hi, thyp_row, lo) : JMID_EINVAL;
+}
+
 int jmid_dbg_tail(jmid_handle_t h, int E, int A, int K, int T, const float* X, const float* hyp, int hyp_width, int step, int precision,
                   float* e, float* thyp_row) {
     return h ? dbg_step(h, true, E, A, K, T, X, hyp, hyp_width, step, precision, e, thyp_row) : JMID_EINVAL;
diff --git a/safe-interactive-crowdnav_amd/csrc/jmid_planner.hip b/safe-interactive-crowdnav_amd/csrc/jmid_planner.hip
--- a/safe-interactive-crowdnav_amd/csrc/jmid_planner.hip
+++ b/safe-interactive-crowdnav_amd/csrc/jmid_planner.hip
@@ -199,6 +199,7 @@
     if (d <= 512 && p.M % T == 0 && t.out_traj != 2 && (t.out_traj == 1 || p.M >= 4096 * 4)) {
         p.out_tpw = T;
         while (p.out_tpw > 1 && (p.M / p.out_tpw < 4096 || T % p.out_tpw != 0)) --p.out_tpw;
+        if (p.tail_fold && t.tail_fold != 3) p.out_tpw = seam_tokens_per_wave(p.M, T, 1);
         if (t.out_traj == 1) p.out_tpw = T;
     }
     return p;
@@ -338,9 +339,16 @@
         qa.Q8l = im.q8l; qa.K8h = im.k8h; qa.K8l = im.k8l;
         qa.M = M; qa.d = d; qa.hd = hd; qa.S = S; qa.Spad = p.sg.Spad; qa.nseq = p.sg.nseq;
         qa.qscale = qscale; qa.rmap = p.rm; qa.range_flag = h->range_flag; qa.x2 = p.mode.x2;
+        ProfScope ps(h, KC_GEMM_QKV, ln.stream);
+#ifdef JMID_DIAGNOSTICS
+        if (h->tune.qkv0 == 3) {
+            qkv0_plan_v0(qa, p.T);
+            HIPCHK(h, launch_qkv0_expand(qkv0_expand_v0_kernel, qa, ln.stream));
+            return 0;
+        }
+#endif
         qkv0_plan(qa, p.T);
-        ProfScope ps(h, KC_GEMM_QKV, ln.stream);
-        HIPCHK(h, launch_qkv0_expand(qa, ln.stream));
+        HIPCHK(h, launch_qkv0_expand(qkv0_expand_kernel, qa, ln.stream));
         return 0;
     }
     return in_proj_planes(h, p, ln, l);
@@ -379,6 +387,13 @@
     };
     const auto pick = [&](auto embed, auto with_lo) {
         constexpr bool EN = decltype(embed)::value, LO = decltype(with_lo)::value;
+#ifdef JMID_DIAGNOSTICS
+        if (h->tune.tail_fold == 3) {
+            if (p.out_tpw) launch(tail_fold_traj_v0_kernel<EN, LO>, M / p.out_tpw, p.out_tpw);
+            else launch(tail_fold_v0_kernel<EN, LO>, M);
+            return;
+        }
+#endif
         if (p.out_tpw) launch(tail_fold_traj_kernel<EN, LO>, M / p.out_tpw, p.out_tpw);
         else launch(tail_fold_kernel<EN, LO>, M);
     };
@@ -927,7 +942,7 @@
 
 #ifdef JMID_DIAGNOSTICS
 int dbg_step(jmid_ctx* h, bool tail, int E, int A, int K, int T, const float* in, const float* hyp, int hyp_width, int step, int precision,
-             float* out, float* thyp_row) {
+             float* out, float* thyp_row, float* out_lo) {
     const std::string who = tail ? "jmid_dbg_tail" : "jmid_dbg_qkv0";
     CallMode mode;
     if (int rc = check_ready(h)) return rc;
@@ -942,12 +957,13 @@
     const int d = h->d, in_w = tail ? d : 2, out_w = tail ? 2 : 3 * d;
     const StepPlan p = plan_step(h, E, A, K, T, mode, CallFacts{});
     const size_t qkv0_rows = !tail && p.qkv0 ? EA * 3 : 0, tail_rows = tail && p.tail_fold ? EA : 0;
-    float *in_d, *hyp_d, *out_d;
+    float *in_d, *hyp_d, *out_d, *lo_d = nullptr;
     const auto io = [&](char* base) {
         Carver c(base);
         in_d = c.take(M * in_w);
         hyp_d = c.take(EA * h->hl.total);
         out_d = c.take(M * out_w);
+        if (out_lo) lo_d = c.take(M * out_w);
         return c.off;
     };
     const size_t io_off = io(nullptr);
@@ -974,13 +990,14 @@
         if (int rc = qkv_planes(h, p, ln, 0, step, in_d, hyp_d)) return rc;
         const LoImages im = lo_images(p, ln, d);
         QkvReadArgs ra{ln.Qh, ln.Ql, ln.Kh, ln.Kl, ln.Vth, ln.Vtl, im.q8l, im.k8l, out_d, M, d, p.hd, p.sg.S, p.sg.Spad, mode.x2,
-                       p.att_scale * 1.4426950408889634f};
+                       p.att_scale * 1.4426950408889634f, out_lo ? lo_d : nullptr};
         hipLaunchKernelGGL(qkv_planes_read_kernel, dim3(512), dim3(256), 0, h->stream, ra);
         HIPCHK(h, hipGetLastError());
     }
     int flag = 0;
     HIPCHK(h, hipMemcpyAsync(&flag, h->range_flag, sizeof(int), hipMemcpyDeviceToHost, h->stream));
     HIPCHK(h, hipMemcpyAsync(out, out_d, M * out_w * sizeof(float), hipMemcpyDeviceToHost, h->stream));
+    if (out_lo && !tail) HIPCHK(h, hipMemcpyAsync(out_lo, lo_d, M * out_w * sizeof(float), hipMemcpyDeviceToHost, h->stream));
     if (thyp_row)
         HIPCHK(h, hipMemcpyAsync(thyp_row, p.thyp(step), h->hl.total * sizeof(float), hipMemcpyDeviceToHost, h->stream));
     HIPCHK(h, hipStreamSynchronize(h->stream));
diff --git a/safe-interactive-crowdnav_amd/csrc/qkv0.hpp b/safe-interactive-crowdnav_amd/csrc/qkv0.hpp
--- a/safe-interactive-crowdnav_amd/csrc/qkv0.hpp
+++ b/safe-interactive-crowdnav_amd/csrc/qkv0.hpp
@@ -67,7 +67,78 @@
     return fmaf(x0, u, fmaf(x1, v, c)) + p;
 }
 
+constexpr int kQkRows = 6;
 __device__ __forceinline__ void qkv0_expand_qk(const Qkv0Args& a, int wave, int lane) {
+    typedef int i32x4_t __attribute__((ext_vector_type(4)));
+    const int piece = wave / a.qk_slabs, slab = wave - piece * a.qk_slabs;
+    const int m0 = piece * a.tpw;
+    if (m0 >= a.M) return;
+    const bool on = slab * 512 + lane * 8 < 2 * a.d;
+    const int j = on ? slab * 512 + lane * 8 : 0;
+    const int part = j >= a.d, nn = j - part * a.d, n3 = 3 * a.d;
+    const int t0 = a.rmap.t_of(m0);
+    const float* row = a.uvc + (size_t)a.rmap.ea(m0) * 3 * n3 + j;
+    f32x4 u[2], v[2], c[2];
+#pragma unroll
+    for (int h = 0; h < 2; ++h) {
+        u[h] = *reinterpret_cast<const f32x4*>(row + 4 * h);
+        v[h] = *reinterpret_cast<const f32x4*>(row + n3 + 4 * h);
+        c[h] = *reinterpret_cast<const f32x4*>(row + 2 * n3 + 4 * h);
+    }
+    const float qs = part == 0 ? a.qscale : 1.0f;
+    const auto of_lane = [](float x, int l) { return __builtin_bit_cast(float, __builtin_amdgcn_readlane(__builtin_bit_cast(int, x), l)); };
+    unsigned amax16 = 0;
+    for (int tb = 0; tb < a.tpw; tb += kQkRows) {
+        const int nb = a.tpw - tb < kQkRows ? a.tpw - tb : kQkRows;
+        f32x4 p[kQkRows][2];
+#pragma unroll
+        for (int i = 0; i < kQkRows; ++i) {
+            if (i >= nb) break;
+            const float* pe = a.ppe + (size_t)(t0 + tb + i) * n3 + j;
+            p[i][0] = *reinterpret_cast<const f32x4*>(pe);
+            p[i][1] = *reinterpret_cast<const f32x4*>(pe + 4);
+        }
+        const int mu = m0 + tb + (lane < nb ? lane : 0);
+        const float xl0 = a.x[2 * (size_t)mu], xl1 = a.x[2 * (size_t)mu + 1];
+#pragma unroll
+        for (int i = 0; i < kQkRows; ++i) {
+            if (i >= nb) break;
+            const float x0 = of_lane(xl0, i), x1 = of_lane(xl1, i);
+            Split4 sp[2];
+#pragma unroll
+            for (int h = 0; h < 2; ++h) {
+                float o[4];
+#pragma unroll
+                for (int e = 0; e < 4; ++e) {
+                    o[e] = qkv0_value(x0, x1, u[h][e], v[h][e], c[h][e], p[i][h][e]);
+                    if (part == 0) o[e] *= qs;
+                }
+                sp[h] = split_f32x4(o[0], o[1], o[2], o[3], amax16);
+            }
+            if (!on) continue;
+            const size_t at = (size_t)(m0 + tb + i) * a.d + nn;
+            const i32x4_t hi = {sp[0].hi[0], sp[0].hi[1], sp[1].hi[0], sp[1].hi[1]}, lo = {sp[0].lo[0], sp[0].lo[1], sp[1].lo[0], sp[1].lo[1]};
+            const i32x2_s lo8 = {bf8_of_f16x4(sp[0].lo[0], sp[0].lo[1]), bf8_of_f16x4(sp[1].lo[0], sp[1].lo[1])};
+            if (part == 0) {
+                store_stream(reinterpret_cast<i32x4_t*>(a.Qh + at), hi);
+                if (a.Q8l) store_stream(reinterpret_cast<i32x2_s*>(a.Q8l + at), lo8);
+                else store_stream(reinterpret_cast<i32x4_t*>(a.Ql + at), lo);
+            } else {
+                store_stream(reinterpret_cast<i32x4_t*>(a.Kh + at), hi);
+                if (a.K8h) {
+                    store_stream(reinterpret_cast<i32x2_s*>(a.K8h + at), i32x2_s{bf8_of_f16x4(sp[0].hi[0], sp[0].hi[1]), bf8_of_f16x4(sp[1].hi[0], sp[1].hi[1])});
+                    store_stream(reinterpret_cast<i32x2_s*>(a.K8l + at), lo8);
+                } else {
+                    store_stream(reinterpret_cast<i32x4_t*>(a.Kl + at), lo);
+                }
+            }
+        }
+    }
+    if (split_range_exceeded(amax16)) atomicOr(a.range_flag, 1);
+}
+
+#ifdef JMID_DIAGNOSTICS
+__device__ __forceinline__ void qkv0_expand_qk_v0(const Qkv0Args& a, int wave, int lane) {
     const int piece = wave / a.qk_slabs, slab = wave - piece * a.qk_slabs;
     const int m0 = piece * a.tpw;
     const int j = slab * 256 + lane * 4;
@@ -108,6 +179,7 @@
     }
     if (split_range_exceeded(amax16)) atomicOr(a.range_flag, 1);
 }
+#endif
 
 __device__ __forceinline__ void qkv0_expand_v(const Qkv0Args& a, int wave, int lane) {
     const int slabs = a.d / a.v_cpw;
@@ -168,22 +240,41 @@
     else qkv0_expand_v(a, ((int)blockIdx.x - a.qk_blocks) * 4 + w, lane);
 }
 
+inline void qkv0_plan_v(Qkv0Args& a, int T) {
+    a.v_kblocks = (a.S + 255) / 256;
+    a.v_cpw = a.d % 16 == 0 ? 16 : 4;
+    while (a.v_cpw > 4 && (long)a.nseq * a.v_kblocks * (a.d / a.v_cpw) < 4096) a.v_cpw >>= 1;
+    a.v_same_row = T % 4 == 0 && a.S % 4 == 0;
+}
 inline void qkv0_plan(Qkv0Args& a, int T) {
+    a.qk_slabs = (2 * a.d + 511) / 512;
+    a.tpw = seam_tokens_per_wave(a.M, T, a.qk_slabs);
+    a.qk_blocks = (int)(((long)(a.M / a.tpw) * a.qk_slabs + 3) / 4);
+    qkv0_plan_v(a, T);
+}
+template <typename Kernel>
+inline hipError_t launch_qkv0_expand(Kernel* kernel, const Qkv0Args& a, hipStream_t st) {
+    const long v_waves = (long)a.nseq * a.v_kblocks * (a.d / a.v_cpw);
+    const int blocks = a.qk_blocks + (int)((v_waves + 3) / 4);
+    hipLaunchKernelGGL(kernel, dim3(blocks), dim3(256), 0, st, a);
+    return hipGetLastError();
+}
+
+#ifdef JMID_DIAGNOSTICS
+static __global__ __launch_bounds__(256) void qkv0_expand_v0_kernel(Qkv0Args a) {
+    args_now(a);
+    const int lane = threadIdx.x & 63, w = threadIdx.x >> 6;
+    if ((int)blockIdx.x < a.qk_blocks) qkv0_expand_qk_v0(a, blockIdx.x * 4 + w, lane);
+    else qkv0_expand_v(a, ((int)blockIdx.x - a.qk_blocks) * 4 + w, lane);
+}
+inline void qkv0_plan_v0(Qkv0Args& a, int T) {
     a.qk_slabs = (2 * a.d + 255) / 256;
     a.tpw = T;
     while (a.tpw > 1 && ((long)(a.M / a.tpw) * a.qk_slabs < 4096 || T % a.tpw != 0)) --a.tpw;
     a.qk_blocks = (int)(((long)(a.M / a.tpw) * a.qk_slabs + 3) / 4);
-    a.v_kblocks = (a.S + 255) / 256;
-    a.v_cpw = a.d % 16 == 0 ? 16 : 4;
-    while (a.v_cpw > 4 && (long)a.nseq * a.v_kblocks * (a.d / a.v_cpw) < 4096) a.v_cpw >>= 1;
-    a.v_same_row = T % 4 == 0 && a.S % 4 == 0;
-}
-inline hipError_t launch_qkv0_expand(const Qkv0Args& a, hipStream_t st) {
-    const long v_waves = (long)a.nseq * a.v_kblocks * (a.d / a.v_cpw);
-    const int blocks = a.qk_blocks + (int)((v_waves + 3) / 4);
-    hipLaunchKernelGGL(qkv0_expand_kernel, dim3(blocks), dim3(256), 0, st, a);
-    return hipGetLastError();
-}
+    qkv0_plan_v(a, T);
+}
+#endif
 
 #ifdef JMID_DIAGNOSTICS
 struct QkvReadArgs {
diff --git a/safe-interactive-crowdnav_amd/csrc/tail_fold.hpp b/safe-interactive-crowdnav_amd/csrc/tail_fold.hpp
--- a/safe-interactive-crowdnav_amd/csrc/tail_fold.hpp
+++ b/safe-interactive-crowdnav_amd/csrc/tail_fold.hpp
@@ -195,7 +195,31 @@
     if (lane * 8 < d) x = *reinterpret_cast<const f16x8*>(plane + blk_index(m, lane * 8, d));
     return x;
 }
-template <bool LO>
+__device__ __forceinline__ void row_swap(float x, float& even_rows, float& odd_rows) {
+    float a = x, b = x;
+    asm volatile("s_nop 1\n\tv_permlane16_swap_b32 %0, %1" : "+v"(a), "+v"(b));
+    even_rows = a;
+    odd_rows = b;
+}
+template <int CTRL>
+__device__ __forceinline__ float row_dpp(float v) {
+    const int i = __builtin_bit_cast(int, v);
+    return __builtin_bit_cast(float, __builtin_amdgcn_update_dpp(i, i, CTRL, 0xf, 0xf, false));
+}
+__device__ __forceinline__ float tail_wave_sum(float v) {
+    float a, b;
+    half_swap(v, a, b);
+    v = a + b;
+    row_swap(v, a, b);
+    v = a + b;
+    v += row_dpp<0x128>(v);
+    v += row_dpp<0x124>(v);
+    v += row_dpp<0x4E>(v);
+    v += row_dpp<0xB1>(v);
+    return v;
+}
+
+template <bool LO, bool SHFL = false>
 __device__ __forceinline__ void tail_fold_dot(f16x8 xh, f16x8 xl, const TailMap& t, float& e0, float& e1) {
     float s0 = 0.f, s1 = 0.f;
 #pragma unroll
@@ -204,8 +228,8 @@
         s0 = fmaf(v, t.w[0][e >> 2][e & 3], s0);
         s1 = fmaf(v, t.w[1][e >> 2][e & 3], s1);
     }
-    e0 = wave_sum(s0) + t.b0;
-    e1 = wave_sum(s1) + t.b1;
+    e0 = (SHFL ? wave_sum(s0) : tail_wave_sum(s0)) + t.b0;
+    e1 = (SHFL ? wave_sum(s1) : tail_wave_sum(s1)) + t.b1;
 }
 __device__ __forceinline__ void tail_fold_update(const OutArgs& a, float e0, float e1, float x0, float x1, float z0, float z1,
                                                  float& xn0, float& xn1) {
@@ -219,8 +243,135 @@
     }
 }
 
+__device__ __forceinline__ void embed_store_cols8(const EmbedArgs& a, int m, int j, int t, float x0, float x1, const EmbedCols (&c)[2]) {
+    const float* pe = a.pe + (size_t)t * a.d + j;
+    const f32x4 p[2] = {*reinterpret_cast<const f32x4*>(pe), *reinterpret_cast<const f32x4*>(pe + 4)};
+    f32x4 o[2];
+#pragma unroll
+    for (int h = 0; h < 2; ++h)
+#pragma unroll
+        for (int e = 0; e < 4; ++e) {
+            const float lin = c[h].w0[e] * x0 + c[h].w1[e] * x1 + c[h].b1[e];
+            o[h][e] = lin * c[h].gate[e] + c[h].bias[e] + p[h][e];
+        }
+    if (a.X) {
+        *reinterpret_cast<f32x4*>(a.X + (size_t)m * a.d + j) = o[0];
+        *reinterpret_cast<f32x4*>(a.X + (size_t)m * a.d + j + 4) = o[1];
+    }
+    if (a.Xh) {
+        typedef int i32x4_t __attribute__((ext_vector_type(4)));
+        unsigned unused = 0;
+        const Split4 s0 = split_f32x4(o[0][0], o[0][1], o[0][2], o[0][3], unused), s1 = split_f32x4(o[1][0], o[1][1], o[1][2], o[1][3], unused);
+        const size_t ob = blk_index(m, j, a.d);
+        *reinterpret_cast<i32x4_t*>(a.Xh + ob) = i32x4_t{s0.hi[0], s0.hi[1], s1.hi[0], s1.hi[1]};
+        if (a.Xl8)
+            *reinterpret_cast<i32x2_s*>(a.Xl8 + ((((size_t)(m >> 7) * (a.d >> 5) + (j >> 5)) * 128 + (m & 127)) * 32 + (j & 31))) =
+                i32x2_s{bf8_of_f16x4(s0.lo[0], s0.lo[1]), bf8_of_f16x4(s1.lo[0], s1.lo[1])};
+        else
+            *reinterpret_cast<i32x4_t*>(a.Xl + ob) = i32x4_t{s0.lo[0], s0.lo[1], s1.lo[0], s1.lo[1]};
+    }
+}
+
 template <bool EMBED_NEXT, bool LO>
 __global__ __launch_bounds__(256) void tail_fold_kernel(TailFoldArgs f, OutArgs a, EmbedArgs nxt) {
+    args_now_each(f, a, nxt);
+    const int lane = threadIdx.x & 63;
+    const int m = blockIdx.x * (blockDim.x >> 6) + (threadIdx.x >> 6);
+    if (m >= a.M) return;
+    const f16x8 xh = tail_fold_load(f.Xh, f.d, m, lane);
+    const f16x8 xl = LO ? tail_fold_load(f.Xl, f.d, m, lane) : xh;
+    const int ea = a.rmap.ea(m);
+    TailMap t;
+    tail_fold_map(f, ea, lane, t);
+    const float x0 = a.e_out ? 0.f : a.x[2 * (size_t)m], x1 = a.e_out ? 0.f : a.x[2 * (size_t)m + 1];
+    const float z0 = (a.ddpm && a.z) ? a.z[2 * (size_t)m] : 0.f, z1 = (a.ddpm && a.z) ? a.z[2 * (size_t)m + 1] : 0.f;
+    float e0, e1;
+    tail_fold_dot<LO>(xh, xl, t, e0, e1);
+    float xn0 = 0.f, xn1 = 0.f;
+    if (a.e_out) {
+        if (lane == 0) {
+            a.e_out[2 * (size_t)m] = e0;
+            a.e_out[2 * (size_t)m + 1] = e1;
+        }
+    } else {
+        tail_fold_update(a, e0, e1, x0, x1, z0, z1, xn0, xn1);
+        if (lane == 0) {
+            a.x[2 * (size_t)m] = xn0;
+            a.x[2 * (size_t)m + 1] = xn1;
+        }
+    }
+    if (EMBED_NEXT && lane * 8 < nxt.d) {
+        const float* hrow = nxt.hyp + (size_t)ea * nxt.hyp_ld;
+        EmbedCols c[2];
+        embed_cols(nxt, lane * 8, hrow, c[0]);
+        embed_cols(nxt, lane * 8 + 4, hrow, c[1]);
+        embed_store_cols8(nxt, m, lane * 8, nxt.rmap.t_of(m), xn0, xn1, c);
+    }
+}
+
+constexpr int kTailRows = 6, kTailRowsLo = 4;
+template <bool EMBED_NEXT, bool LO>
+__global__ __launch_bounds__(256) __attribute__((amdgpu_waves_per_eu(LO ? 3 : 4, 8))) void tail_fold_traj_kernel(TailFoldArgs f, OutArgs a, EmbedArgs nxt, int tpw) {
+    args_now_each(f, a, nxt);
+    const int lane = threadIdx.x & 63;
+    const int piece = blockIdx.x * (blockDim.x >> 6) + (threadIdx.x >> 6);
+    const int m0 = piece * tpw;
+    if (m0 >= a.M) return;
+    const int t0 = a.rmap.t_of(m0), ea = a.rmap.ea(m0);
+    const bool on = lane * 8 < f.d;
+    constexpr int ROWS = LO ? kTailRowsLo : kTailRows;
+    f16x8 xh[ROWS], xl[LO ? ROWS : 1];
+    const auto request = [&](int tb, int nb) {
+#pragma unroll
+        for (int u = 0; u < ROWS; ++u) {
+            if (u >= nb) break;
+            xh[u] = tail_fold_load(f.Xh, f.d, m0 + tb + u, lane);
+            if (LO) xl[LO ? u : 0] = tail_fold_load(f.Xl, f.d, m0 + tb + u, lane);
+        }
+    };
+    request(0, tpw < ROWS ? tpw : ROWS);
+    EmbedCols c[2];
+    if (EMBED_NEXT && on) {
+        const float* hrow = nxt.hyp + (size_t)ea * nxt.hyp_ld;
+        embed_cols(nxt, lane * 8, hrow, c[0]);
+        embed_cols(nxt, lane * 8 + 4, hrow, c[1]);
+    }
+    TailMap t;
+    tail_fold_map(f, ea, lane, t);
+    for (int tb = 0; tb < tpw; tb += ROWS) {
+        const int nb = tpw - tb < ROWS ? tpw - tb : ROWS;
+        if (tb) request(tb, nb);
+        const int mu = m0 + tb + (lane < nb ? lane : 0);
+        const float xl0 = a.e_out ? 0.f : a.x[2 * (size_t)mu], xl1 = a.e_out ? 0.f : a.x[2 * (size_t)mu + 1];
+        const float zl0 = (a.ddpm && a.z) ? a.z[2 * (size_t)mu] : 0.f, zl1 = (a.ddpm && a.z) ? a.z[2 * (size_t)mu + 1] : 0.f;
+        const auto of_lane = [](float v, int u) { return __builtin_bit_cast(float, __builtin_amdgcn_readlane(__builtin_bit_cast(int, v), u)); };
+#pragma unroll
+        for (int u = 0; u < ROWS; ++u) {
+            if (u >= nb) break;
+            const int m = m0 + tb + u;
+            float e0, e1;
+            tail_fold_dot<LO>(xh[u], LO ? xl[LO ? u : 0] : xh[u], t, e0, e1);
+            float xn0 = 0.f, xn1 = 0.f;
+            if (a.e_out) {
+                if (lane == 0) {
+                    a.e_out[2 * (size_t)m] = e0;
+                    a.e_out[2 * (size_t)m + 1] = e1;
+                }
+            } else {
+                tail_fold_update(a, e0, e1, of_lane(xl0, u), of_lane(xl1, u), of_lane(zl0, u), of_lane(zl1, u), xn0, xn1);
+                if (lane == 0) {
+                    a.x[2 * (size_t)m] = xn0;
+                    a.x[2 * (size_t)m + 1] = xn1;
+                }
+            }
+            if (EMBED_NEXT && on) embed_store_cols8(nxt, m, lane * 8, t0 + tb + u, xn0, xn1, c);
+        }
+    }
+}
+
+#ifdef JMID_DIAGNOSTICS
+template <bool EMBED_NEXT, bool LO>
+__global__ __launch_bounds__(256) void tail_fold_v0_kernel(TailFoldArgs f, OutArgs a, EmbedArgs nxt) {
     args_now_each(f, a, nxt);
     const int lane = threadIdx.x & 63;
     const int m = blockIdx.x * (blockDim.x >> 6) + (threadIdx.x >> 6);
@@ -232,7 +383,7 @@
     const float x0 = a.e_out ? 0.f : a.x[2 * (size_t)m], x1 = a.e_out ? 0.f : a.x[2 * (size_t)m + 1];
     const float z0 = (a.ddpm && a.z) ? a.z[2 * (size_t)m] : 0.f, z1 = (a.ddpm && a.z) ? a.z[2 * (size_t)m + 1] : 0.f;
     float e0, e1;
-    tail_fold_dot<LO>(xh, xl, t, e0, e1);
+    tail_fold_dot<LO, true>(xh, xl, t, e0, e1);
     float xn0 = 0.f, xn1 = 0.f;
     if (a.e_out) {
         if (lane == 0) {
@@ -250,7 +401,7 @@
 }
 
 template <bool EMBED_NEXT, bool LO>
-__global__ __launch_bounds__(256) void tail_fold_traj_kernel(TailFoldArgs f, OutArgs a, EmbedArgs nxt, int tpw) {
+__global__ __launch_bounds__(256) void tail_fold_traj_v0_kernel(TailFoldArgs f, OutArgs a, EmbedArgs nxt, int tpw) {
     args_now_each(f, a, nxt);
     const int lane = threadIdx.x & 63;
     const int piece = blockIdx.x * (blockDim.x >> 6) + (threadIdx.x >> 6);
@@ -283,7 +434,7 @@
             if (u >= nb) continue;
             const int m = m0 + tb + u;
             float e0, e1;
-            tail_fold_dot<LO>(xh[u], LO ? xl[LO ? u : 0] : xh[u], t, e0, e1);
+            tail_fold_dot<LO, true>(xh[u], LO ? xl[LO ? u : 0] : xh[u], t, e0, e1);
             float xn0 = 0.f, xn1 = 0.f;
             if (a.e_out) {
                 if (lane == 0) {
@@ -305,7 +456,6 @@
     }
 }
 
-#ifdef JMID_DIAGNOSTICS
 static __global__ void tail_split_rows_kernel(const float* in, half_t* hi, half_t* lo, int rows, int K) {
     const size_t n = (size_t)rows * K;
     for (size_t i = (size_t)blockIdx.x * blockDim.x + threadIdx.x; i < n; i += (size_t)gridDim.x * blockDim.x) {
diff --git a/safe-interactive-crowdnav_amd/engine.py b/safe-interactive-crowdnav_amd/engine.py
--- a/safe-interactive-crowdnav_amd/engine.py
+++ b/safe-interactive-crowdnav_amd/engine.py
@@ -846,7 +846,7 @@
                                                      C.c_void_p(b.ctypes.data)))
         return X
 
-    def dbg_qkv0(self, x: np.ndarray, hyp: np.ndarray, step: int, dims: Tuple[int, int, int, int], precision: str = "f16mx"):
+    def dbg_qkv0(self, x: np.ndarray, hyp: np.ndarray, step: int, dims: Tuple[int, int, int, int], precision: str = "f16mx", out_lo: bool = False):
         E, A, K, T = (int(v) for v in dims)
         x = np.ascontiguousarray(x, np.float32)
         hyp = np.ascontiguousarray(hyp, np.float32)
@@ -856,6 +856,12 @@
             raise ValueError(f"expected x [{M}, 2] and hyp [{E * A}, {width}]")
         out = np.empty((M, 3 * d), np.float32)
         thyp = np.empty((width,), np.float32)
+        if out_lo:
+            lo = np.empty((M, 3 * d), np.float32)
+            self._check(self._lib.jmid_dbg_qkv0_planes(self._h, E, A, K, T, C.c_void_p(x.ctypes.data), C.c_void_p(hyp.ctypes.data), width, int(step),
+                                                       _lib.PRECISIONS[precision], C.c_void_p(out.ctypes.data), C.c_void_p(lo.ctypes.data),
+                                                       C.c_void_p(thyp.ctypes.data)))
+            return out, lo, thyp
         self._check(self._lib.jmid_dbg_qkv0(self._h, E, A, K, T, C.c_void_p(x.ctypes.data), C.c_void_p(hyp.ctypes.data), width, int(step),
                                             _lib.PRECISIONS[precision], C.c_void_p(out.ctypes.data), C.c_void_p(thyp.ctypes.data)))
         return out, thyp
```
